# timbroed/HRFuser

Measured on AMD Instinct MI355X. Metric: train images/sec HRFuser-T r640 3-modal @1/2/4/8 MI355X; fwd ms/img, higher is better.
Workload: dtype f32; 1 GPU; t_nus_bn backbone train step (fwd+bwd+grad exchange+AdamW at lr 0), 2 img/GPU, 2x3x384x640 camera + 2 modalities, BN, single GPU; global_batch=2, parallelism=dp1, launch=hipGraph replay

## Files before the change

hrfuser_amd/_lib.py:

```python
import ctypes
import os
import re

import torch

_HERE = os.path.dirname(os.path.abspath(__file__))
HEADER = os.path.join(os.path.dirname(_HERE), 'include', 'hrfuser_hip.h')
DEBUG_HEADER = os.path.join(os.path.dirname(_HERE), 'include', 'hrfuser_hip_debug.h')
LIB_PATH = os.environ.get('HRF_LIB_PATH') or os.path.join(_HERE, 'libhrfuser_hip.so')

def _header_int(name, default):
    m = re.search(r'#define\s+' + name + r'\s+(\d+)', open(HEADER).read())
    return int(m.group(1)) if m else default


STAT_COPIES = _header_int('HRF_STAT_COPIES', 16)
FIN_MAXC = _header_int('HRF_FIN_MAXC', 576)
C3X_MAXC = _header_int('HRF_C3X_MAXC', 256)

def struct_from_header(tag, path=HEADER):
    src = re.sub(r'/\*.*?\*/', '', open(path).read(), flags=re.S)
    m = re.search(r'typedef\s+struct\s+' + tag + r'\s*\{(.*?)\}\s*' + tag + r'_t\s*;', src, flags=re.S)
    if not m:
        raise KeyError(tag)
    fields = []
    for decl in m.group(1).split(';'):
        decl = ' '.join(decl.split())
        if not decl:
            continue
        arr = re.search(r'(\w+)\[(\w+)\]$', decl)
        if arr:
            ext = int(arr.group(2)) if arr.group(2).isdigit() else _header_int(arr.group(2), 0)
            base = decl.split(' ', 1)[0]
            el = ctypes.c_void_p if '*' in decl else {'int': ctypes.c_int, 'long': ctypes.c_long, 'float': ctypes.c_float, 'double': ctypes.c_double}[base]
            fields.append((arr.group(1), el * ext))
            continue
        if '*' in decl:
            ct, names = ctypes.c_void_p, [re.findall(r'(\w+)$', decl)[0]]
        else:
            base, rest = decl.split(' ', 1)
            ct = {'int': ctypes.c_int, 'long': ctypes.c_long, 'float': ctypes.c_float, 'double': ctypes.c_double}[base]
            names = [n.strip() for n in rest.split(',')]
        fields += [(n, ct) for n in names]
    return type(tag, (ctypes.Structure,), {'_fields_': fields})


BnFin = struct_from_header('hrf_bn_fin')
BnBFin = struct_from_header('hrf_bn_bfin')
AttnBlock = struct_from_header('hrf_attn_block')
AttnProj = struct_from_header('hrf_attn_proj')
FfnEval = struct_from_header('hrf_ffn_eval')
BottleneckEval = struct_from_header('hrf_bottleneck_eval')
Conv3xPackJob = struct_from_header('hrf_conv3x_pack_job')
RoiLevels = struct_from_header('hrf_roi_levels')
P2p = struct_from_header('hrf_p2p')


def _ptr(t):
    return None if t is None else t.data_ptr()


_RAW_RETURN = ('hrf_conv3_wgrad_wide_scratch', 'hrf_conv_bwd_weight_scratch', 'hrf_conv3x_pack_size', 'hrf_conv3x_supported', 'hrf_conv_bwd_data_weight_supported', 'hrf_conv_fwd_split_scratch', 'hrf_wgrad_group_report', 'hrf_attn_block_supported', 'hrf_attn_block_bwd_supported', 'hrf_window_attn_proj_supported', 'hrf_group_count',
               'hrf_ffn_eval_supported', 'hrf_bottleneck_eval_supported', 'hrf_roi_align_supported', 'hrf_get_deterministic', 'hrf_det_bins_bytes', 'hrf_conv3_bf16x3_supported', 'hrf_grad_sumsq_parts')
_ERR = {1: 'HRF_ERR_ARG (bad argument)', 2: 'HRF_ERR_LAUNCH (kernel launch failed)'}


class HRFuserHipError(RuntimeError):
    pass


def parse_header(path=HEADER):
    src = open(path).read()
    src = re.sub(r'/\*.*?\*/', '', src, flags=re.S)
    protos = {}
    for m in re.finditer(r'\b(?:int|long)\s+(hrf_\w+)\s*\(([^)]*)\)\s*;', src):
        args = []
        for a in m.group(2).split(','):
            a = ' '.join(a.split())
            if not a or a == 'void':
                continue
            name = re.findall(r'(\w+)$', a)[0]
            if '*' in a:
                ct = ctypes.c_void_p
            elif a.startswith('float'):
                ct = ctypes.c_float
            elif a.startswith('double'):
                ct = ctypes.c_double
            elif a.startswith('long'):
                ct = ctypes.c_long
            else:
                ct = ctypes.c_int
            args.append((ct, name))
        protos[m.group(1)] = args
    return protos


class Lib:

    def __init__(self, path, require_cuda=True):
        if not os.path.exists(path):
            raise HRFuserHipError(
                f'{path} not found: the HRFuser HIP extension is not built. Run '
                '`python -m hrfuser_amd.build_ext` (needs hipcc). There is no CPU fallback.')
        self.path = path
        self.require_cuda = require_cuda
        self._dll = ctypes.CDLL(path)
        self.protos = parse_header()
        self.protos.update(parse_header(DEBUG_HEADER))
        self._fns = {}
        for name, args in self.protos.items():
            fn = getattr(self._dll, name)
            fn.restype = ctypes.c_long if name in ('hrf_conv3_wgrad_wide_scratch', 'hrf_conv_bwd_weight_scratch', 'hrf_conv3x_pack_size', 'hrf_conv_fwd_split_scratch', 'hrf_wgrad_group_report', 'hrf_group_count', 'hrf_det_bins_bytes', 'hrf_grad_sumsq_parts') else ctypes.c_int
            fn.argtypes = [ct for ct, _ in args]
            self._fns[name] = self._wrap(name, fn, args)
        if os.environ.get('HRF_DETERMINISTIC', '0') == '1':
            self.hrf_set_deterministic(1)

    def _wrap(self, name, fn, args):
        kinds = [ct for ct, _ in args]
        nargs = len(kinds)
        require_cuda = self.require_cuda

        def call(*a):
            if len(a) != nargs:
                raise TypeError(f'{name} expects {nargs} args, got {len(a)}')
            conv = []
            for v, ct in zip(a, kinds):
                if ct is ctypes.c_void_p:
                    if v is None:
                        conv.append(None)
                    elif isinstance(v, (ctypes.Structure, ctypes.Array)):
                        conv.append(ctypes.addressof(v))
                    elif isinstance(v, torch.Tensor):
                        if require_cuda and not v.is_cuda:
                            raise HRFuserHipError(f'{name}: tensor on {v.device}; the HIP path has no CPU fallback')
                        conv.append(v.data_ptr())
                    else:
                        conv.append(int(v))
                else:
                    conv.append(v)
            rc = fn(*conv)
            if name in _RAW_RETURN:
                return rc
            if rc != 0:
                raise HRFuserHipError(f'{name} failed: {_ERR.get(rc, rc)}')
# ... 35 lines not shown
```

hrfuser_amd/backbone.py:

```python
import os
import warnings

import torch
import torch.nn as nn

from . import _lib
from . import runtime as R
from .registry import BACKBONES

WIN = 7


def build_bn(norm_cfg, c):
    cfg = dict(norm_cfg or dict(type='BN'))
    kind = cfg.pop('type')
    if kind not in ('BN', 'SyncBN', 'GN'):
        raise KeyError(f'unsupported norm_cfg type {kind}')
    requires_grad = cfg.pop('requires_grad', True)
    if kind == 'GN':
        if 'num_groups' not in cfg:
            raise AssertionError('norm_cfg of type GN needs num_groups')
        bn = nn.GroupNorm(cfg['num_groups'], c, eps=cfg.get('eps', 1e-5))
    else:
        bn = nn.BatchNorm2d(c, eps=cfg.get('eps', 1e-5), momentum=cfg.get('momentum', 0.1))
# ... 425 lines not shown
        if eng is None:
            eng = Engine(self)
            self.__dict__['_hrf_engine'] = eng
        return eng

    def _lib_handle(self):
        return _lib.lib()

    def _bn_slot(self, bn):
        return self._engine().slots[id(bn)]

    def _bn_eval_affine(self, bn):
        return self._engine().bn_eval_affine(bn)

    use_lanes = True

    def _lane_pool(self, grow=False):
        pool = self.__dict__.setdefault('_hrf_lanes', [])
        if grow:
            lane = R.Lane(torch.cuda.Stream(priority=int(os.environ.get('HRF_LANE_PRIORITY', '0'))))
            pool.append(lane)
            return lane
        return pool

    def _lane_group(self, lane, base_group):
        groups = self.__dict__.setdefault('_hrf_lane_groups', {})
        g = groups.get(id(lane))
        if g is None:
            import torch.distributed as dist
            g = groups[id(lane)] = dist.new_group(ranks=dist.get_process_group_ranks(base_group))
        return g

    def _side_pool(self):
        pool = self.__dict__.get('_hrf_side')
        if pool is None:
            n = int(os.environ.get('HRF_SIDE_LANES', '6') or 6)
            try:
                low = max(torch.cuda.Stream.priority_range())
            except Exception:
                low = 0
            if os.environ.get('HRF_SIDE_PRIORITY', '1') == '0':
                low = 0
            pool = [R.Lane(torch.cuda.Stream(priority=low)) for _ in range(max(1, n))]
            self.__dict__['_hrf_side'] = pool
        return pool

    def set_sync_group(self, group, world):
        self.sync_group, self.sync_world = group, world
        if group is not None:
            R.check_sync_schedule(group, world)

    def set_deterministic(self, on=True):
        L = self._lib_handle()
        if bool(L.hrf_get_deterministic()) != bool(on):
            self._engine().det_epoch += 1
        L.hrf_set_deterministic(1 if on else 0)
        self._engine().det_sync()
        if hasattr(self, 'reset_graphs'):
            self.reset_graphs()

    def set_bottleneck_eval(self, on=True):
        self.__dict__['_hrf_bneck_eval'] = bool(on)
        if hasattr(self, 'reset_graphs'):
            self.reset_graphs()

    def params_updated(self):
        """Kept for callers that signal a weight update; nothing is cached across steps any more."""


class Bottleneck(nn.Module):
    expansion = 4

    def __init__(self, inplanes, planes, norm_cfg, downsample=None):
        super().__init__()
        self._nn = [norm_name(norm_cfg, k) for k in (1, 2, 3)]
        self.conv1 = nn.Conv2d(inplanes, planes, 1, bias=False)
        self.add_module(self._nn[0], build_bn(norm_cfg, planes))
        self.conv2 = nn.Conv2d(planes, planes, 3, 1, 1, bias=False)
        self.add_module(self._nn[1], build_bn(norm_cfg, planes))
        self.conv3 = nn.Conv2d(planes, planes * 4, 1, bias=False)
        self.add_module(self._nn[2], build_bn(norm_cfg, planes * 4))
        self.downsample = downsample

    def run(self, ctx, x):
        if R.bottleneck_eval_ok(ctx, self, x):
            return R.bottleneck_eval(ctx, x, self)
        n1, n2, n3 = (getattr(self, k) for k in self._nn)
        y = R.conv_bn(ctx, x, self.conv1, n1, R.TF_RELU)
        y = R.conv_bn(ctx, y, self.conv2, n2, R.TF_RELU)
        y = R.conv_bn(ctx, y, self.conv3, n3, R.TF_AFFINE)
        if self.downsample is not None:
            idt = R.conv_bn(ctx, x, self.downsample[0], self.downsample[1], R.TF_AFFINE)
            return R.materialize(ctx, y, R.ACT_RELU, lazy2=idt)
        return R.materialize(ctx, y, R.ACT_RELU, res=x)


class BasicBlock(nn.Module):
    expansion = 1

    def __init__(self, inplanes, planes, norm_cfg, downsample=None):
        super().__init__()
        if downsample is not None or inplanes != planes:
            raise NotImplementedError('BasicBlock with a downsample path is unused by the HRNet branches')
        self._nn = [norm_name(norm_cfg, k) for k in (1, 2)]
        self.conv1 = nn.Conv2d(inplanes, planes, 3, 1, 1, bias=False)
        self.add_module(self._nn[0], build_bn(norm_cfg, planes))
        self.conv2 = nn.Conv2d(planes, planes, 3, 1, 1, bias=False)
        self.add_module(self._nn[1], build_bn(norm_cfg, planes))
        self.downsample = None

    def run(self, ctx, x):
        y = R.conv_bn(ctx, x, self.conv1, getattr(self, self._nn[0]), R.TF_RELU)
        y = R.conv_bn(ctx, y, self.conv2, getattr(self, self._nn[1]), R.TF_AFFINE)
        return R.materialize(ctx, y, R.ACT_RELU, res=x)


class CrossFFN(nn.Module):

    def __init__(self, in_channels, hidden_channels=None, out_channels=None, norm_cfg=dict(type='SyncBN'), **kw):
        super().__init__()
        out_channels = out_channels or in_channels
        hidden_channels = hidden_channels or in_channels
        self.layers = nn.Sequential(
            nn.Conv2d(in_channels, hidden_channels, 1), build_bn(norm_cfg, hidden_channels), nn.GELU(),
            nn.Conv2d(hidden_channels, hidden_channels, 3, 1, 1, groups=hidden_channels),
            build_bn(norm_cfg, hidden_channels), nn.GELU(),
            nn.Conv2d(hidden_channels, out_channels, 1), build_bn(norm_cfg, out_channels), nn.GELU())

    def run(self, ctx, ln_in):
        l = self.layers
        return self.run_tail(ctx, R.conv_bn(ctx, ln_in, l[0], l[1], R.TF_GELU))

    def run_tail(self, ctx, h1):
        l = self.layers
        h = R.dwconv_bn(ctx, h1, l[3], l[4], R.TF_GELU)
        return R.conv_bn(ctx, h, l[6], l[7], R.TF_GELU)


class WindowMSA(nn.Module):
    def __init__(self, embed_dims, num_heads, window_size=(WIN, WIN), **kw):
        super().__init__()
        if tuple(window_size) != (WIN, WIN):
            raise NotImplementedError('the HIP attention core is specialised for 7x7 windows')
        self.embed_dims, self.num_heads = embed_dims, num_heads
        self.relative_position_bias_table = nn.Parameter(torch.zeros((2 * WIN - 1) ** 2, num_heads))
        self.register_buffer('relative_position_index', _rel_index())
        self.qkv = nn.Linear(embed_dims, embed_dims * 3)
        self.out_proj = nn.Linear(embed_dims, embed_dims)


class LocalWindowSelfAttention(nn.Module):

    def __init__(self, embed_dims, num_heads, window_size=WIN, with_pad_mask=False, **kw):
        super().__init__()
        if with_pad_mask:
            raise NotImplementedError('with_pad_mask=True is unused by every reference config')
        ws = (window_size, window_size) if isinstance(window_size, int) else tuple(window_size)
        self.attn = WindowMSA(embed_dims, num_heads, ws)

    def run(self, ctx, x, ln, cache=None, drop=None):
        a = self.attn
        B, H, W, C = x.t.shape
        lin = R.ln_input(ctx, x, ln, cache)
        if R.attn_proj_ok(ctx, C, a.num_heads):
            o = R.window_attention_proj(ctx, lin, lin, (a.qkv,), a.relative_position_bias_table, a.num_heads)
            return R.linear_residual(ctx, o, a.out_proj, x, drop=drop)
        qkv = R.Plain(R._new((B * H * W, 3 * C), x.t.device))
        R.linear_into(ctx, lin, a.qkv, qkv, 0)
        bq = a.qkv.bias
        o = R.window_attention(ctx, qkv, 0, qkv, C, qkv, 2 * C, bq[C:2 * C], bq[2 * C:], bq, C, bq, 2 * C,
                               a.relative_position_bias_table, a.num_heads, (B, H, W, C))
        return R.linear_residual(ctx, o, a.out_proj, x, drop=drop)


_DEBUG_PAD_CACHE = {}


# ... 310 lines not shown
                        row.append(nn.Sequential(nn.Conv2d(ch[j], ch[i], 1, bias=False), build_bn(norm_cfg, ch[i]),
                                                 nn.Upsample(scale_factor=2 ** (j - i), mode='nearest')))
                    elif j == i:
                        row.append(None)
                    else:
                        steps = []
                        for k in range(i - j):
                            last = k == i - j - 1
                            cout = ch[i] if last else ch[j]
                            mods = [nn.Conv2d(ch[j], cout, 3, 2, 1, bias=False), build_bn(norm_cfg, cout)]
                            if not last:
                                mods.append(nn.ReLU(inplace=False))
                            steps.append(nn.Sequential(*mods))
                        row.append(nn.Sequential(*steps))
                rows.append(nn.ModuleList(row))
            self.fuse_layers = nn.ModuleList(rows)

    def run(self, ctx, xs):
        nb = self.num_branches
        xs = list(xs)
        lanes = ctx.fork(nb, keep_first=ctx.keep_first)

        def branch(i):
            xs[i] = R.force(ctx, xs[i])
            for blk in self.branches[i]:
                xs[i] = blk.run(ctx, xs[i])
        ctx.parallel(lanes, [lambda i=i: branch(i) for i in range(nb)])
        ctx.join(lanes)
        if nb == 1:
            return [xs[0]]
        nrows = len(self.fuse_layers)
        terms = [[None] * nb for _ in range(nrows)]
        lanes = ctx.fork(nb, keep_first=ctx.keep_first)

        def source(j):
            for i, row in enumerate(self.fuse_layers):
                if j == i:
                    terms[i][j] = ('id', xs[j])
                elif j > i:
                    Hi, Wi, Hj, Wj = xs[i].t.shape[1], xs[i].t.shape[2], xs[j].t.shape[1], xs[j].t.shape[2]
                    if Hi != Hj << (j - i) or Wi != Wj << (j - i):
                        raise NotImplementedError('HRModule exchange on grids that do not nest (input not a multiple of 32)')
                    terms[i][j] = ('near', R.conv_bn(ctx, xs[j], row[j][0], row[j][1], R.TF_AFFINE))
                else:
                    cur = xs[j]
                    for step in row[j]:
                        cur = R.conv_bn(ctx, cur, step[0], step[1], R.TF_RELU if len(step) == 3 else R.TF_AFFINE)
                    terms[i][j] = ('same', cur)
        ctx.parallel(lanes, [lambda j=j: source(j) for j in range(nb)])
        ctx.join(lanes)
        return [R.fuse_sum(ctx, tuple(xs[i].t.shape), terms[i]) for i in range(nrows)]


def _make_transition(pre, cur, norm_cfg):
    layers = []
    for i, c in enumerate(cur):
        if i < len(pre):
            layers.append(_conv_bn_seq(pre[i], c, 3, 1, norm_cfg, relu=True) if c != pre[i] else None)
        else:
            steps = []
            for j in range(i + 1 - len(pre)):
                cout = c if j == i - len(pre) else pre[-1]
                steps.append(_conv_bn_seq(pre[-1], cout, 3, 2, norm_cfg, relu=True))
            layers.append(nn.Sequential(*steps))
    return nn.ModuleList(layers)


def _run_conv_chain(ctx, x, seqs):
    cur = x
    for seq in seqs:
        cur = R.conv_bn(ctx, cur, seq[0], seq[1], R.TF_RELU)
    return R.materialize(ctx, cur, R.ACT_RELU)


def _make_res_layer(inplanes, planes, blocks, norm_cfg):
    ds = None
    if inplanes != planes * 4:
        ds = nn.Sequential(nn.Conv2d(inplanes, planes * 4, 1, bias=False), build_bn(norm_cfg, planes * 4))
    layers = [Bottleneck(inplanes, planes, norm_cfg, ds)]
    layers += [Bottleneck(planes * 4, planes, norm_cfg) for _ in range(1, blocks)]
    return nn.Sequential(*layers)


def resolve_init_cfg(pretrained, init_cfg):
    assert not (init_cfg and pretrained), 'init_cfg and pretrained cannot be specified at the same time'
    if isinstance(pretrained, str):
        warnings.warn('DeprecationWarning: pretrained is deprecated, please use "init_cfg" instead')
        return dict(type='Pretrained', checkpoint=pretrained)
    if pretrained is not None:
        raise TypeError('pretrained must be a str or None')
    return init_cfg


def load_pretrained(module, init_cfg):
    path = init_cfg['checkpoint']
    if not os.path.isfile(path):
        raise FileNotFoundError(f'init_cfg Pretrained: {path} is not a local file (there is no downloader here)')
    ckpt = torch.load(path, map_location='cpu')
    sd = ckpt.get('state_dict', ckpt) if isinstance(ckpt, dict) else ckpt
    prefix = init_cfg.get('prefix')
    out = {}
    for k, v in sd.items():
        if k.startswith('module.'):
            k = k[7:]
        if prefix:
            p = prefix if prefix.endswith('.') else prefix + '.'
            if not k.startswith(p):
                continue
            k = k[len(p):]
        out[k] = v
    res = module.load_state_dict(out, strict=False)
    if res.missing_keys or res.unexpected_keys:
        warnings.warn(f'Pretrained init from {path}: {len(res.missing_keys)} missing, '
                      f'{len(res.unexpected_keys)} unexpected keys')
    return res


def default_or_pretrained_init(module):
    cfg = getattr(module, 'init_cfg', None)
    if cfg:
        if isinstance(cfg, dict) and cfg.get('type') == 'Pretrained':
            return load_pretrained(module, cfg)
        raise NotImplementedError(f'init_cfg {cfg!r}: only None (Kaiming / Constant default) and type=Pretrained are built')
    for m in module.modules():
        if isinstance(m, nn.Conv2d):
            nn.init.kaiming_normal_(m.weight, mode='fan_out', nonlinearity='relu')
            if m.bias is not None:
                nn.init.constant_(m.bias, 0)
        elif isinstance(m, (nn.modules.batchnorm._BatchNorm, nn.GroupNorm)):
            nn.init.constant_(m.weight, 1)
            nn.init.constant_(m.bias, 0)


class _BackboneFn(torch.autograd.Function):

    @staticmethod
    def forward(fctx, module, anchor, *inputs):
        record = anchor is not None
        ctx, outs, srcs = module._execute(inputs, record)
        fctx.hrf = (ctx, outs, srcs)
        fctx.set_materialize_grads(False)
        return tuple(o.t.permute(0, 3, 1, 2) for o in outs)

    @staticmethod
    def backward(fctx, *gouts):
        ctx, outs, srcs = fctx.hrf
        for o, g in zip(outs, gouts):
            if g is None:
                o.grad = torch.zeros_like(o.t)
            else:
                o.grad = g.permute(0, 2, 3, 1).contiguous()
                if o.grad.data_ptr() == g.data_ptr():
                    o.grad = o.grad.clone()
        ctx.run_backward()
        grads = tuple(fctx_module_input_grad(s) for s in srcs)
        fctx.hrf = None
        _poll_exchange(ctx.owner)
        return (None, None) + grads


def _poll_exchange(module):
    px = module._engine().__dict__.get('_p2p')
    if px is not None and px[2] is not None:
        px[2].poll()


# ... 314 lines not shown
            fcfg = extra['ModFusionD']
            self.fusion_d_cfg = fcfg
            ch = list(fcfg['num_channels'])
            self.transition_d = nn.ModuleList(_make_transition(sch, ch, ncfg) for _ in range(M))
            self.fusion_d = self._make_multimodal_fusion(fcfg, ch)
        self.init_weights()

    def _make_stage(self, cfg, in_channels, multiscale_output=True):
        block = self.blocks_dict[cfg['block']]
        if block is not HRFormerBlock:
            raise NotImplementedError('stages 2-4 / LidarStage B-C must use block HRFORMER')
        n = cfg['num_modules']
        nb0 = cfg['num_blocks'][0]
        dpr = cfg.get('drop_path_rates', [0.0] * (n * nb0))
        mods = []
        for i in range(n):
            ms = multiscale_output or i != n - 1
            mods.append(HRFomerModule(cfg['num_branches'], block, cfg['num_blocks'], in_channels,
                                      cfg['num_channels'], cfg['num_heads'], cfg['window_sizes'], cfg['mlp_ratios'],
                                      ms, drop_paths=dpr[nb0 * i:nb0 * (i + 1)],
                                      with_rpe=self.extra.get('with_rpe', True),
                                      with_pad_mask=self.extra.get('with_pad_mask', False),
                                      norm_cfg=self.norm_cfg, transformer_norm_cfg=self.transformer_norm_cfg,
                                      with_cp=self.with_cp))
            in_channels = mods[-1].in_channels
        return nn.Sequential(*mods), in_channels

    def _make_multimodal_fusion(self, cfg, num_inchannels):
        if cfg['block'] not in ('CA', 'MWCA'):
            raise Exception('Not valid fusion block')
        block = self.blocks_dict[cfg['block']]
        return nn.ModuleList(
            block(num_inchannels[i], cfg['num_channels'][i], num_heads=cfg['num_heads'][i],
                  window_size=cfg['window_sizes'][i], mlp_ratio=cfg['mlp_ratios'][i], drop_path=cfg['drop_path'],
                  norm_cfg=self.norm_cfg, transformer_norm_cfg=self.transformer_norm_cfg,
                  num_fused_modalities=self.num_fused_modalities, proj_drop_rate=cfg['proj_drop_rate'])
            for i in range(cfg['num_branches']))

    def init_weights(self):
        default_or_pretrained_init(self)

    def train(self, mode=True):
        super().train(mode)
        if mode and self.norm_eval:
            for m in self.modules():
                if isinstance(m, nn.modules.batchnorm._BatchNorm):
                    m.eval()
        return self

    def unused_parameter_names(self):
        return ('transition1.0.1.weight', 'transition1.0.1.bias')

    def forward(self, x, x_mod):
        if not self.num_fused_modalities == len(x_mod):
            raise Exception('num_fused_modalities does not fit the given input length')
        for m in x_mod:
            if m.shape[0] != x.shape[0] or m.shape[2:] != x.shape[2:]:
                raise AssertionError('camera and modality inputs must share batch and spatial size')
        return self._call_engine((x,) + tuple(x_mod))

    def refresh_inputs(self, inputs):
        bufs = self.__dict__.setdefault('_nhwc_in', {})
        for i, t in enumerate(inputs):
            Bn, C, H, W = t.shape
            if t.is_contiguous(memory_format=torch.channels_last) and not t.is_contiguous():
                bufs[i] = t.permute(0, 2, 3, 1)
                continue
            b = bufs.get(i)
            if b is None or b.shape != (Bn, H, W, C) or b.device != t.device or not b.is_contiguous():
                b = bufs[i] = torch.empty(Bn, H, W, C, device=t.device, dtype=torch.float32)
            b.copy_(t.permute(0, 2, 3, 1))
        return bufs

    def _wrap_inputs(self, inputs):
        bufs = {}
        if self.training and inputs[0].is_cuda:
            bufs = self.refresh_inputs(inputs)
        return [R.RawInput(t, bool(t.requires_grad), bufs.get(i)) for i, t in enumerate(inputs)]

    def _stem(self, ctx, src, c1, b1, c2, b2, layer):
        y = R.conv_bn(ctx, src, c1, b1, R.TF_RELU)
        y = R.conv_bn(ctx, y, c2, b2, R.TF_RELU)
        x = R.materialize(ctx, y, R.ACT_RELU)
        for blk in layer:
            x = blk.run(ctx, x)
        return x

    def _fuse_stage(self, ctx, cam_in, trans_cam, trans_mod, fusion, nb, mods, first, tag=''):
        M = self.num_fused_modalities
        cams = [None] * nb
        ms = [[None] * M for _ in range(nb)]
        lanes = ctx.bundle_lanes(1 + M, 'trans')

        def cam_trans():
            for i in range(nb):
                if first:
                    t0 = trans_cam[i][0]
                    cams[i] = self._bare_conv(ctx, cam_in, t0) if isinstance(t0, nn.Conv2d) \
                        else _run_conv_chain(ctx, cam_in, [t0])
                elif trans_cam[i] is not None:
                    tr = trans_cam[i]
                    same = isinstance(tr[0], nn.Conv2d)
                    cams[i] = _run_conv_chain(ctx, cam_in[i] if same else cam_in[-1], [tr] if same else list(tr))
                else:
                    cams[i] = cam_in[i]

        def mod_trans(k):
            for i in range(nb):
                tr = trans_mod[k][i]
                ms[i][k] = mods[k] if tr is None else \
                    _run_conv_chain(ctx, mods[k], [tr] if isinstance(tr[0], nn.Conv2d) else list(tr))
        ctx.parallel(lanes, [cam_trans] + [lambda k=k: mod_trans(k) for k in range(M)])
        ctx.join(lanes)
        ctx.mark('transitions_' + tag)
        xs = [R.Pending(tuple(cams[i].t.shape), lambda c, i=i: fusion[i].run(c, cams[i], ms[i])) for i in range(nb)]
        m0 = [R.split_grad(ctx, ms[0][k]) for k in range(M)]
        if not _PENDING_FUSION:
            xs = R.force_all(ctx, xs)
            ctx.mark('fusion_' + tag)
        return xs, m0

    def _bare_conv(self, ctx, x, conv):
        B, H, W, C = x.t.shape
        out = R.Plain(R._new((B * H * W, conv.weight.shape[0]), x.t.device))
        L, s = ctx.L, ctx.stream
        w = conv.weight
        Cout = w.shape[0]
        strides = (H * W * C, W * C, C, 1)
        L.hrf_conv_fwd(x.t, *strides, B, H, W, C, w, None, 3, 1, Cout, out.t, Cout, 0, None, None, 0,
                       R.TF_NONE, None, None, None, None, None, None, 0.0, s)
        act = R.Act(out.t.view(B, H, W, Cout))

        def bwd():
            R._conv_backward(ctx, x, w, None, 3, 1, Cout, act.grad, Cout, 0, None, None)
        ctx.push(bwd)
        return act

    @staticmethod
    def _run_stage(ctx, stage, xs):
        mods = list(stage)
        for k, mod in enumerate(mods):
            if isinstance(mod, HRFomerModule) and mod.num_branches == 1 and k + 1 < len(mods) and \
                    isinstance(mods[k + 1], HRFomerModule) and mods[k + 1].num_branches == 1:
                xs = mod.run(ctx, xs, defer_out=True)
            else:
                xs = mod.run(ctx, xs)
        return R.force_all(ctx, xs)

    def _run(self, ctx, srcs):
        M = self.num_fused_modalities
        lanes = ctx.bundle_lanes(1 + M, 'stems')
        mods = [None] * M
        cam = [None]

        def cam_stem():
            cam[0] = self._stem(ctx, srcs[0], self.conv1, getattr(self, self._stem_nn[0]), self.conv2, getattr(self, self._stem_nn[1]), self.layer1)

        def mod_stem(k):
            mods[k] = self._stem(ctx, srcs[1 + k], self.conv_a[k], self.norm_a[k], self.conv_b[k], self.norm_b[k],
                                 self.layer_a[k])
        ctx.parallel(lanes, [cam_stem] + [lambda k=k: mod_stem(k) for k in range(M)])
        ctx.join(lanes)
        ctx.mark('stems')
        x = cam[0]
        xs, m0 = self._fuse_stage(ctx, x, self.transition1, self.transition_a, self.fusion_a,
                                  self.stage2_cfg['num_branches'], mods, True, 'a')
        ys, mods = self._stages(ctx, self.stage2, xs, self.stage_b, m0)
        ctx.mark('stage2+stage_b')
        xs, m0 = self._fuse_stage(ctx, ys, self.transition2, self.transition_b, self.fusion_b,
# ... 187 lines not shown
```

hrfuser_amd/csrc/conv_engine.hip:

```cpp
#include <algorithm>
#include <cstdlib>
#include <vector>
#include "hrf_common.h"
#include "hrf_group.h"
#include "hrf_lin.h"
#include "../../include/hrfuser_hip.h"

#include "hrf_wgrad.h"

namespace {

constexpr int BM = 64;
constexpr int BK = 64;
constexpr int LDK = 65;
constexpr float SENT = -1.0e30f;

static int g_knob[12] = {0, 0, 0, 0, 0, 0, 0, 0, 0, 0, 0, 0};

__device__ __forceinline__ float act_at_read(int tf, float u) {
  return tf == HRF_TF_AFFINE_RELU ? fmaxf(u, 0.f) : (tf == HRF_TF_AFFINE_GELU ? hrf_gelu(u) : u);
}

struct ConvFwdArgs {
  const float* x; const float* w; const float* bias;
// ... 890 lines not shown
  const int pad = KH / 2;
  a.bfin = hrf_bn_bfin_t{};
  if (!hrf_det_fin_ok(bfin)) return HRF_ERR_ARG;
  if (bfin != nullptr) a.bfin = *bfin;
  stats = hrf_det_tag(stats);
  a.dy = dy; a.ldD = ldD; a.doff = doff; a.yraw = yraw; a.cA = cA; a.cB = cB; a.cC = cC; a.w = w;
  a.dx = dx; a.sB = sB; a.sY = sY; a.sX = sX; a.sC = sC; a.accumulate = accumulate; a.epi = epi;
  a.xraw = xraw; a.ldXr = ldXr; a.tf_scale = tf_scale; a.tf_shift = tf_shift; a.act = act; a.stats = stats;
  a.B = B; a.H = H; a.W = W; a.Cin = Cin;
  a.Ho = (H + 2 * pad - KH) / stride + 1; a.Wo = (W + 2 * pad - KH) / stride + 1;
  a.Cout = Cout; a.stride = stride; a.pad = pad;
  a.M = B * H * W; a.K = KH * KH * Cout;
  if (a.M <= 0) return HRF_OK;
  if (KH == 1 && stride == 1 && sC == 1 && sY == W * sX && sB == H * sY && g_knob[4] == 0) {
    LinBwdDataArgs l;
    l.dy = dy; l.ldD = ldD; l.doff = doff; l.yraw = yraw; l.cA = cA; l.cB = cB; l.cC = cC; l.w = w;
    l.dx = dx; l.ldDx = sX; l.accumulate = accumulate; l.epi = epi; l.xraw = xraw; l.ldXr = ldXr;
    l.tf_scale = tf_scale; l.tf_shift = tf_shift; l.act = act; l.stats = stats; l.bfin = a.bfin;
    l.M = a.M; l.K = Cout; l.N = Cin;
    const int rc2 = hrf_lin2_bwd_data_launch(l, stream);
    if (rc2 >= 0) return rc2;
    const int rc = hrf_lin_bwd_data_launch(l, stream);
    if (rc >= 0) return rc;
  }
  if (KH == 3 && stride == 1 && Cout >= (g_knob[5] > 0 ? g_knob[5] : 16) && sC == 1 && sY == W * sX && sB == H * sY && g_knob[6] == 0) {
    Conv3Args c{};
    c.in = dy + doff; c.ldIn = ldD; c.in2 = cA != nullptr ? yraw + doff : nullptr; c.t0 = cA; c.t1 = cB; c.t2 = cC;
    c.w = w; c.wCin = Cin; c.out = dx; c.ldOut = sX; c.accumulate = accumulate; c.epi = epi; c.xraw = xraw; c.ldXr = ldXr;
    c.esc = tf_scale; c.esh = tf_shift; c.act = act; c.stats = stats; c.bfin = a.bfin;
    c.B = B; c.H = H; c.W = W; c.Cin = Cout; c.Cout = Cin;
    return hrf_conv3_bwd_data_launch(c, stream);
  }
  if (KH == 3 && stride == 2 && Cout >= (g_knob[5] > 0 ? g_knob[5] : 16) && sC == 1 && sY == W * sX && sB == H * sY && g_knob[6] == 0) {
    Conv3Args c{};
    c.in = dy + doff; c.ldIn = ldD; c.in2 = cA != nullptr ? yraw + doff : nullptr; c.t0 = cA; c.t1 = cB; c.t2 = cC;
    c.w = w; c.wCin = Cin; c.out = dx; c.ldOut = sX; c.accumulate = accumulate; c.epi = epi; c.xraw = xraw; c.ldXr = ldXr;
    c.esc = tf_scale; c.esh = tf_shift; c.act = act; c.stats = stats; c.bfin = a.bfin;
    c.B = B; c.H = H; c.W = W; c.Cin = Cout; c.Cout = Cin; c.Hs = a.Ho; c.Ws = a.Wo;
    return hrf_conv3s2_bwd_data_launch(c, stream);
  }
  const int nt = pick_nt(Cin);
  if (KH == 1) {
    if (cA != nullptr) { HRF_BD_NT(1, true) } else { HRF_BD_NT(1, false) }
  } else {
    if (cA != nullptr) { HRF_BD_NT(3, true) } else { HRF_BD_NT(3, false) }
  }
  return hrf_check_launch();
}

extern "C" int hrf_conv_bwd_data_weight_supported(int Cin, int Cout, long rows, int epi, int bnb) {
  if (Cin <= 0 || Cout <= 0 || rows <= 0 || (epi != 0 && epi != 1) || g_knob[4] != 0) return 0;
  if (rows > (1L << 30)) return 0;
  if (hrf_lin2_bwd_data_wide(rows, Cout, Cin)) return 0;
  return hrf_lin_bwd_data_wg_ok((int)rows, Cout, Cin, bnb != 0) ? 1 : 0;
}

extern "C" int hrf_conv_bwd_data_weight(const float* dy, int ldD, int doff, const float* yraw,
                                        const float* cA, const float* cB, const float* cC, const hrf_bn_bfin_t* bfin,
                                        const float* w, int KH, int stride, int Cout,
                                        int B, int H, int W, int Cin,
                                        float* dx, int sB, int sY, int sX, int sC, int accumulate,
                                        int epi, const float* xraw, int ldXr, const float* tf_scale,
                                        const float* tf_shift, int act, double* stats,
                                        const float* x, int ldX, float* dw, float* dbias, long copy_stride, void* stream) {
  HRF_GROUP_CALL();
  if (KH != 1 || stride != 1 || !(sC == 1 && sX == Cin && sY == W * sX && sB == H * sY)) return HRF_ERR_ARG;
  if (bfin != nullptr && (cA == nullptr || bfin->C != Cout || Cout > HRF_FIN_MAXC || bfin->gstats == nullptr)) return HRF_ERR_ARG;
  if (dy == nullptr || w == nullptr || dx == nullptr || dw == nullptr || copy_stride < 0) return HRF_ERR_ARG;
  if (epi == 1 ? (xraw == nullptr || tf_scale == nullptr || tf_shift == nullptr || ldXr < Cin) : (x == nullptr || ldX < Cin)) return HRF_ERR_ARG;
  const long rows = (long)B * H * W;
  if (rows <= 0 || !hrf_conv_bwd_data_weight_supported(Cin, Cout, rows, epi, cA != nullptr ? 1 : 0)) return HRF_ERR_ARG;
  if (!hrf_det_fin_ok(bfin)) return HRF_ERR_ARG;
  bool det_ok = true;
  dw = hrf_det_grad(dw, det_ok); dbias = hrf_det_grad(dbias, det_ok);
  if (!det_ok) return HRF_ERR_ARG;
  LinBwdDataArgs l;
  l.bfin = hrf_bn_bfin_t{};
  if (bfin != nullptr) l.bfin = *bfin;
  l.dy = dy; l.ldD = ldD; l.doff = doff; l.yraw = yraw; l.cA = cA; l.cB = cB; l.cC = cC; l.w = w;
  l.dx = dx; l.ldDx = sX; l.accumulate = accumulate; l.epi = epi; l.xraw = xraw; l.ldXr = ldXr;
  l.tf_scale = tf_scale; l.tf_shift = tf_shift; l.act = act; l.stats = hrf_det_tag(stats);
  l.M = (int)rows; l.K = Cout; l.N = Cin;
  l.x = x; l.ldX = ldX; l.dw = dw; l.dbias = dbias; l.copy_stride = copy_stride;
  const int rc = hrf_lin_bwd_data_launch(l, stream);
  return rc >= 0 ? rc : HRF_ERR_ARG;
}

extern "C" int hrf_conv3x_supported(int Cin, int Cout, int KH, int stride, int dir) {
  if (KH != 3 || Cin <= 0 || Cout <= 0) return 0;
  if (dir == 0) return (stride == 1 || stride == 2) && Cout > 32 ? 1 : 0;
  if (stride == 2) return Cin > 32 && Cout <= 64 ? 1 : 0;
  return stride == 1 && Cin > 32 ? 1 : 0;
}

extern "C" int hrf_conv_fwd_packed(const float* x, int sB, int sY, int sX, int sC, int B, int H, int W, int Cin,
                                   const float* w, const float* bias, int KH, int stride, int Cout,
                                   float* y, int ldY, int yoff, const float* res, const float* res2, int ldR,
                                   int tf_mode, const float* tf_scale, const float* tf_shift,
                                   const float* tf_rowstat, double* stats, const hrf_bn_fin_t* tf_fin, float* ln_rowstat,
                                   float ln_eps, const float* wp, void* stream) {
  HRF_GROUP_CALL();
  (void)w; (void)tf_rowstat;
  if (wp == nullptr || !hrf_conv3x_supported(Cin, Cout, KH, stride, 0)) return HRF_ERR_ARG;
  if (!(sC == 1 && sY == W * sX && sB == H * sY) || tf_mode < 0 || tf_mode > HRF_TF_AFFINE_GELU) return HRF_ERR_ARG;
  if (ln_rowstat != nullptr && (ldY != Cout || yoff != 0)) return HRF_ERR_ARG;
  if (tf_mode != HRF_TF_NONE && Cin > HRF_C3X_MAXC) return HRF_ERR_ARG;
  if (tf_fin != nullptr && (tf_mode < HRF_TF_AFFINE || tf_fin->C != Cin || tf_fin->stats == nullptr)) return HRF_ERR_ARG;
  C3xArgs c{};
  c.in = x; c.ldIn = sX; c.t0 = tf_scale; c.t1 = tf_shift; c.tf_mode = tf_mode; c.wp = wp;
  c.Np = (Cout + 63) & ~63; c.Kp = (Cin + 31) & ~31; c.bias = bias;
  c.out = y; c.ldOut = ldY; c.ooff = yoff; c.res = res; c.res2 = res2; c.ldR = ldR; c.stats = hrf_det_tag(stats);
  c.B = B; c.H = H; c.W = W; c.Cin = Cin; c.Cout = Cout;
  if (!hrf_det_fin_ok(tf_fin)) return HRF_ERR_ARG;
  if (tf_fin != nullptr) c.fin = *tf_fin;
  int rc;
  if (stride == 2) {
    c.Hs = H; c.Ws = W; c.H = (H + 2 - KH) / 2 + 1; c.W = (W + 2 - KH) / 2 + 1;
    rc = hrf_conv3xs2_fwd_launch(c, stream);
  } else {
    rc = hrf_conv3x_fwd_launch(c, stream);
  }
  if (rc == HRF_OK && ln_rowstat != nullptr) return hrf_ln_stats(y, (long)B * c.H * c.W, Cout, ln_eps, ln_rowstat, stream);
  return rc;
}

extern "C" int hrf_conv_bwd_data_packed(const float* dy, int ldD, int doff, const float* yraw,
                                        const float* cA, const float* cB, const float* cC, const hrf_bn_bfin_t* bfin,
                                        const float* w, int KH, int stride, int Cout,
                                        int B, int H, int W, int Cin,
                                        float* dx, int sB, int sY, int sX, int sC, int accumulate,
                                        int epi, const float* xraw, int ldXr, const float* tf_scale,
                                        const float* tf_shift, int act, double* stats, const float* wp, void* stream) {
  HRF_GROUP_CALL();
  (void)w;
  if (wp == nullptr || !hrf_conv3x_supported(Cin, Cout, KH, stride, 1)) return HRF_ERR_ARG;
  if (!(sC == 1 && sY == W * sX && sB == H * sY)) return HRF_ERR_ARG;
  if (cA != nullptr && Cout > HRF_C3X_MAXC) return HRF_ERR_ARG;
  if (bfin != nullptr && (cA == nullptr || bfin->C != Cout || bfin->gstats == nullptr)) return HRF_ERR_ARG;
  C3xArgs c{};
  c.in = dy + doff; c.ldIn = ldD; c.in2 = cA != nullptr ? yraw + doff : nullptr; c.t0 = cA; c.t1 = cB; c.t2 = cC;
  c.wp = wp; c.Np = (Cin + 63) & ~63; c.Kp = (Cout + 31) & ~31;
  c.out = dx; c.ldOut = sX; c.accumulate = accumulate; c.epi = epi; c.xraw = xraw; c.ldXr = ldXr;
  c.esc = tf_scale; c.esh = tf_shift; c.act = act; c.stats = hrf_det_tag(stats);
  if (!hrf_det_fin_ok(bfin)) return HRF_ERR_ARG;
  if (bfin != nullptr) c.bfin = *bfin;
  c.B = B; c.H = H; c.W = W; c.Cin = Cout; c.Cout = Cin;
  if (stride == 1) return hrf_conv3x_bwd_data_launch(c, stream);
  c.Hs = (H + 2 - KH) / stride + 1; c.Ws = (W + 2 - KH) / stride + 1;
  return hrf_conv3xs2_bwd_data_launch(c, stream);
}

extern "C" __attribute__((visibility("hidden"))) int hrf_pw_knob(int key, int value);
extern "C" __attribute__((visibility("hidden"))) int hrf_conv3w_knob(int key, int value);
extern "C" __attribute__((visibility("hidden"))) int hrf_lin2_knob(int key, int value);
extern "C" __attribute__((visibility("hidden"))) int hrf_w3x_knob(int key, int value);
extern "C" __attribute__((visibility("hidden"))) int hrf_dw_knob(int key, int value);
extern "C" __attribute__((visibility("hidden"))) int hrf_ab_knob(int key, int value);
extern "C" int hrf_debug_knob(int key, int value) {
  if (key >= 36 && key < 40) return hrf_ab_knob(key - 36, value);
  if (key >= 40 && key < 44) return hrf_dw_knob(key - 40, value);
  if (key >= 32 && key < 36) return hrf_w3x_knob(key - 32, value);
  if (key >= 28 && key < 32) return hrf_lin2_knob(key - 28, value);
  if (key >= 16 && key < 20) return hrf_pw_knob(key - 16, value);
  if (key >= 24 && key < 28) return hrf_conv3w_knob(key - 24, value);
  if (key < 0 || key >= 12) return HRF_ERR_ARG;
  g_knob[key] = value;
// ... 269 lines not shown
```

hrfuser_amd/csrc/hrf_lin.h:

```cpp
#pragma once
#include "../../include/hrfuser_hip.h"

struct LinFwdArgs {
  const float* x; int ldX;
  const float* w; const float* bias;
  float* y; int ldY; int yoff;
  const float* res; const float* res2; int ldR;
  int tf_mode; const float* tf_scale; const float* tf_shift; const float* tf_rowstat;
  double* stats;
  float* ln_out; float ln_eps;
  hrf_bn_fin_t fin;
  int M, K, N;
};

struct LinBwdDataArgs {
  const float* dy; int ldD; int doff; const float* yraw;
  const float* cA; const float* cB; const float* cC;
  const float* w;
  float* dx; int ldDx; int accumulate;
  int epi; const float* xraw; int ldXr; const float* tf_scale; const float* tf_shift; int act;
  double* stats;
  hrf_bn_bfin_t bfin;
  int M, K, N;
  const float* x = nullptr; int ldX = 0;
  float* dw = nullptr; float* dbias = nullptr; long copy_stride = 0;
};

int hrf_lin_fwd_launch(const LinFwdArgs& a, void* stream);
bool hrf_lin_fwd_emits_ln(const LinFwdArgs& a);
int hrf_lin_bwd_data_launch(const LinBwdDataArgs& a, void* stream);
bool hrf_lin_bwd_data_wg_ok(int M, int K, int N, bool bnb);
int hrf_lin2_fwd_launch(const LinFwdArgs& a, void* stream);
bool hrf_lin2_fwd_emits_ln(const LinFwdArgs& a);
int hrf_lin2_bwd_data_launch(const LinBwdDataArgs& a, void* stream);
bool hrf_lin2_bwd_data_wide(long M, int K, int N);

struct Conv3Args {
  const float* in; int ldIn;
  const float* in2;
  const float* t0; const float* t1; const float* t2;
  int tf_mode;
  const float* w; int wCin;
  const float* bias;
  float* out; int ldOut; int ooff;
  const float* res; const float* res2; int ldR;
  int accumulate, epi; const float* xraw; int ldXr; const float* esc; const float* esh; int act;
  double* stats;
  hrf_bn_fin_t fin;
  hrf_bn_bfin_t bfin;
  int B, H, W, Cin, Cout;
  int Hs, Ws;
  int tilesX, tilesY;
};
int hrf_conv3_fwd_launch(const Conv3Args& a, void* stream);
int hrf_conv3_bwd_data_launch(const Conv3Args& a, void* stream);
int hrf_conv3s2_bwd_data_launch(const Conv3Args& a, void* stream);

struct C3xArgs {
  const float* in; int ldIn;
  const float* in2;
  const float* t0; const float* t1; const float* t2;
  int tf_mode;
  const float* wp; int Np, Kp;
  const float* bias;
  float* out; int ldOut; int ooff;
  const float* res; const float* res2; int ldR;
  int accumulate, epi; const float* xraw; int ldXr; const float* esc; const float* esh; int act;
  double* stats;
  hrf_bn_fin_t fin;
  hrf_bn_bfin_t bfin;
  int B, H, W, Cin, Cout;
  int Hs, Ws;
  int tilesX, tilesY, ntiles, per_xcd;
  int cols_per_block;
};

int hrf_conv3x_fwd_launch(const C3xArgs& a, void* stream);
int hrf_conv3x_bwd_data_launch(const C3xArgs& a, void* stream);
int hrf_conv3xs2_fwd_launch(const C3xArgs& a, void* stream);
int hrf_conv3xs2_bwd_data_launch(const C3xArgs& a, void* stream);
```

hrfuser_amd/csrc/lin2_engine.hip:

```cpp
#include <type_traits>
#include "hrf_common.h"
#include "hrf_lin.h"
#include "hrf_group.h"
#include "../../include/hrfuser_hip.h"

namespace {

constexpr int GK = 16, GLP = GK + 4, NW = 4, NTHR = 64 * NW, GROWS = 16 * NW;

template <int CG_, int CT_, int PD_>
struct Tile {
  static constexpr int CG = CG_, CT = CT_, PD = PD_;
  static constexpr int NB = CG * CT * 16, RT = CG, RG = NW / CG;
  static constexpr int SLOT = (GROWS + NB) * GLP;
  static constexpr int NWV = (NB * 4 + NTHR - 1) / NTHR;
  static constexpr int Q = CT * 4, PE = CT * 16 + 4, NRG = NTHR / Q, NR = (GROWS + NRG - 1) / NRG;
  static constexpr int RED = NRG * 2 * CT * 16;
  static_assert(GROWS * PE <= 2 * SLOT, "the transposed accumulator tile must fit the operand ring");
};
typedef Tile<1, 5, 4> TileA;
typedef Tile<2, 5, 4> TileB;
typedef Tile<2, 8, 2> TileC;
typedef Tile<2, 10, 2> TileD;

#ifdef HRF_EMUL
#define L2_SCHED_FENCE() ((void)0)
#define L2_OPAQUE(v) ((void)0)
#else
#define L2_OPAQUE(v) asm volatile("" : "+v"(v))
#define L2_SCHED_FENCE() __builtin_amdgcn_sched_barrier(0)
#endif
#define L2_INLINE __attribute__((always_inline))

__device__ float g_zero4l[4] = {0.f, 0.f, 0.f, 0.f};
#if defined(HRF_L2_TIMING) && !defined(HRF_EMUL)
__device__ long long g_l2_t[64];
#define L2_T(k) do { if (blockIdx.x == 100 && blockIdx.y == 0 && threadIdx.x == 0) g_l2_t[k] = wall_clock64(); } while (0)
#else
#define L2_T(k)
#endif
static int g_l2_knob[4] = {0, 0, 0, 0};

__device__ __forceinline__ hrf_f4 l2_ld4(const float* p) {
#ifdef HRF_EMUL
  return hrf_ld4(p);
#else
  return *reinterpret_cast<const hrf_f4*>(p);
#endif
}
__device__ __forceinline__ void l2_st4(float* p, hrf_f4 v) {
#ifdef HRF_EMUL
  hrf_st4(p, v);
#else
  *reinterpret_cast<hrf_f4*>(p) = v;
#endif
}
__device__ __forceinline__ hrf_f4 gl_ld4(const float* p, int nvalid) {
  if (nvalid >= 4) return hrf_ld4(p);
  hrf_f4 r;
#pragma unroll
  for (int e = 0; e < 4; ++e) r[e] = *(e < nvalid ? p + e : g_zero4l);
  return r;
}

__device__ __forceinline__ hrf_f4 ld4_ragged(const float* row, int idx, int len) {
  const int ic = idx > len - 4 ? len - 4 : idx;
  const int d = idx - ic;
  const hrf_f4 v = hrf_ld4(row + ic);
  hrf_f4 o;
  o[0] = d == 0 ? v[0] : (d == 1 ? v[1] : (d == 2 ? v[2] : (d == 3 ? v[3] : 0.f)));
  o[1] = d == 0 ? v[1] : (d == 1 ? v[2] : (d == 2 ? v[3] : 0.f));
  o[2] = d == 0 ? v[2] : (d == 1 ? v[3] : 0.f);
  o[3] = d == 0 ? v[3] : 0.f;
  return o;
}

template <class T>
__device__ __forceinline__ void acc_to_lds(float* sE, const hrf_f4 (*acc)[T::CT], int rg, int lane) {
  const int i = lane & 15, q = lane >> 4;
#pragma unroll
  for (int rr = 0; rr < T::RT; ++rr)
#pragma unroll
    for (int tt = 0; tt < T::CT; ++tt) l2_st4(sE + ((rg * T::RT + rr) * 16 + i) * T::PE + tt * 16 + 4 * q, acc[rr][tt]);
}
template <class T>
__device__ __forceinline__ void moments_out(float* sRed, double* stats, int N, int chbase, int c4, int rgp, bool active,
                                            const float* s1, const float* s2) {
  constexpr int CW = T::CT * 16;
  if (active) {
#pragma unroll
    for (int r = 0; r < 4; ++r) {
      sRed[(rgp * 2 + 0) * CW + 4 * c4 + r] = s1[r];
      sRed[(rgp * 2 + 1) * CW + 4 * c4 + r] = s2[r];
    }
  }
  __syncthreads();
  for (int e = threadIdx.x; e < 2 * CW; e += NTHR) {
    const int which = e / CW, c = e - which * CW;
    if (chbase + c < N) {
      float s = 0.f;
#pragma unroll
      for (int g = 0; g < T::NRG; ++g) s += sRed[(g * 2 + which) * CW + c];
      hrf_stat_add(stats, 2 * N, which * N + chbase + c, (double)s);
    }
  }
}

template <int V> using IC = std::integral_constant<int, V>;

template <class T, int TF>
__global__ __launch_bounds__(NTHR, 2) void lin2_fwd_kernel(HrfGroup<LinFwdArgs> grp) {
  const LinFwdArgs& a = grp.sel();
  constexpr int CG = T::CG, CT = T::CT, PD = T::PD, NB = T::NB, RT = T::RT, SLOT = T::SLOT, NWV = T::NWV;
  constexpr bool TBLS = TF != HRF_TF_NONE;
  HRF_DYN_SMEM(float, smem);
  const int KT = (a.K + GK - 1) & ~(GK - 1);
  float* sTab = smem + 2 * SLOT;
  float* sRed = sTab + (TBLS ? 2 * KT : 0);
  const int tid = threadIdx.x, lane = tid & 63;
  const int wave = __builtin_amdgcn_readfirstlane(tid >> 6);
  const int i = lane & 15, q = lane >> 4;
  const int chg = wave % CG, rg = wave / CG;
  const long m0 = (long)blockIdx.x * GROWS;
  const int n0 = blockIdx.y * NB;
  L2_T(0);

  if (TBLS) {
    if (TF != HRF_TF_LN && a.fin.stats != nullptr) {
      hrf_bn_fin_onload(a.fin, sTab, sTab + KT, tid, NTHR, blockIdx.x == 0 && blockIdx.y == 0);
    } else {
      for (int k = tid; k < a.K; k += NTHR) { sTab[k] = a.tf_scale[k]; sTab[KT + k] = a.tf_shift[k]; }
    }
    for (int k = a.K + tid; k < KT; k += NTHR) { sTab[k] = 0.f; sTab[KT + k] = 0.f; }
  }

  hrf_f4 acc[RT][CT];
#pragma unroll
  for (int rr = 0; rr < RT; ++rr)
#pragma unroll
    for (int tt = 0; tt < CT; ++tt) acc[rr][tt] = hrf_f4{0.f, 0.f, 0.f, 0.f};

  const long xr = m0 + (tid >> 2) < a.M ? m0 + (tid >> 2) : a.M - 1;
  const int xdst = (tid >> 2) * GLP + 4 * (tid & 3);
  float mean = 0.f, rstd = 1.f;
  if (TF == HRF_TF_LN) { mean = a.tf_rowstat[2 * xr]; rstd = a.tf_rowstat[2 * xr + 1]; }
  const unsigned xoff = (unsigned)(xr * a.ldX);
  const int wn0 = tid >> 2, wq = tid & 3;
  unsigned woff[NWV];
#pragma unroll
  for (int e = 0; e < NWV; ++e) {
    const int n = n0 + wn0 + 64 * e;
    woff[e] = (unsigned)(n < a.N ? n : 0) * (unsigned)a.K;
  }
  const int wdst0 = (GROWS + wn0) * GLP + 4 * wq;
  hrf_f4 xpre[PD], wpre[PD][NWV];
  auto load_tile = [&](auto SETC, int s) L2_INLINE {
    constexpr int SET = decltype(SETC)::value;
    const int kb = s * GK + 4 * (tid & 3);
    if ((s + 1) * GK <= a.K) {
      xpre[SET] = hrf_ld4(a.x + (size_t)(xoff + kb));
#pragma unroll
      for (int e = 0; e < NWV; ++e) wpre[SET][e] = hrf_ld4(a.w + (size_t)(woff[e] + kb));
    } else {
      xpre[SET] = ld4_ragged(a.x + (size_t)xoff, kb, a.K);
#pragma unroll
      for (int e = 0; e < NWV; ++e) wpre[SET][e] = ld4_ragged(a.w + (size_t)woff[e], kb, a.K);
    }
  };
  auto store_tile = [&](auto SETC, int s) L2_INLINE {
    constexpr int SET = decltype(SETC)::value;
    float* d = smem + (s & 1) * SLOT;
    const int kb = s * GK + 4 * (tid & 3);
    hrf_f4 v = xpre[SET];
    if (TBLS) {
      const hrf_f4 sc = l2_ld4(sTab + kb), sh = l2_ld4(sTab + KT + kb);
#pragma unroll
      for (int r = 0; r < 4; ++r) {
        float u = TF == HRF_TF_LN ? fmaf((v[r] - mean) * rstd, sc[r], sh[r]) : fmaf(v[r], sc[r], sh[r]);
        v[r] = TF == HRF_TF_AFFINE_RELU ? fmaxf(u, 0.f) : (TF == HRF_TF_AFFINE_GELU ? hrf_gelu(u) : u);
      }
    }
    l2_st4(d + xdst, v);
#pragma unroll
    for (int e = 0; e < NWV; ++e)
      if ((e + 1) * NTHR <= NB * 4 || tid + e * NTHR < NB * 4) l2_st4(d + wdst0 + e * 64 * GLP, wpre[SET][e]);
  };
// ... 50 lines not shown
    if (s + 1 + PD < S) load_tile(IC<J1>{}, s + 1 + PD);
    read_frags(s & 1);
    L2_SCHED_FENCE();
    mma(ALL);
    L2_SCHED_FENCE();
    __syncthreads();
    L2_T(3 + (s < 40 ? s : 40));
  };
  auto kloop = [&](auto ALL) L2_INLINE {
    for (int s = 0; s < S; s += PD) {
      step(ALL, IC<0>{}, s);
      if (s + 1 < S) step(ALL, IC<1 % PD>{}, s + 1);
      if (PD > 2) {
        if (s + 2 < S) step(ALL, IC<2 % PD>{}, s + 2);
        if (s + 3 < S) step(ALL, IC<3 % PD>{}, s + 3);
      }
    }
  };
  if (all_on) kloop(std::true_type{}); else kloop(std::false_type{});

  {
    constexpr int Q = T::Q, PE = T::PE, NRG = T::NRG, NR = T::NR;
    float* sE = smem;
    const int c4 = tid % Q, rgp = tid / Q;
    const bool active = rgp < NRG;
#pragma unroll 1
    for (int pass = 0; pass < CG; ++pass) {
      const int chbase = n0 + pass * CT * 16, ch = chbase + 4 * c4;
      const int nval = active ? a.N - ch : 0;
      hrf_f4 bv = hrf_f4{0.f, 0.f, 0.f, 0.f};
      if (a.bias != nullptr) bv = gl_ld4(a.bias + ch, nval);
      hrf_f4 r1[NR], r2[NR];
#pragma unroll
      for (int j = 0; j < NR; ++j) { r1[j] = hrf_f4{0.f, 0.f, 0.f, 0.f}; r2[j] = r1[j]; }
      if (a.res != nullptr) {
#pragma unroll
        for (int j = 0; j < NR; ++j) {
          const long m = m0 + rgp + j * NRG;
          const bool rv = rgp + j * NRG < GROWS && m < a.M;
          r1[j] = gl_ld4(a.res + (rv ? m : 0) * a.ldR + ch, rv ? nval : 0);
        }
      }
      if (a.res2 != nullptr) {
#pragma unroll
        for (int j = 0; j < NR; ++j) {
          const long m = m0 + rgp + j * NRG;
          const bool rv = rgp + j * NRG < GROWS && m < a.M;
          r2[j] = gl_ld4(a.res2 + (rv ? m : 0) * a.ldR + ch, rv ? nval : 0);
        }
      }
      L2_T(44 + 4 * pass);
      if (pass > 0) __syncthreads();
      if (chg == pass) acc_to_lds<T>(sE, acc, rg, lane);
      __syncthreads();
      L2_T(45 + 4 * pass);
      float s1[4] = {0.f, 0.f, 0.f, 0.f}, s2[4] = {0.f, 0.f, 0.f, 0.f};
#pragma unroll
      for (int j = 0; j < NR; ++j) {
        const int row = rgp + j * NRG;
        const long m = m0 + row;
        if (row < GROWS && m < a.M && nval > 0) {
          hrf_f4 v = l2_ld4(sE + row * PE + 4 * c4);
#pragma unroll
          for (int r = 0; r < 4; ++r) {
            v[r] = r < nval ? v[r] + bv[r] + r1[j][r] + r2[j][r] : 0.f;
            s1[r] += v[r]; s2[r] = fmaf(v[r], v[r], s2[r]);
          }
          float* o = a.y + m * a.ldY + a.yoff + ch;
          if (nval >= 4) hrf_st4(o, v);
          else {
#pragma unroll
            for (int r = 0; r < 4; ++r)
              if (r < nval) o[r] = v[r];
          }
        }
      }
      L2_T(46 + 4 * pass);
      if (a.stats != nullptr) moments_out<T>(sRed, a.stats, a.N, chbase, c4, rgp, active, s1, s2);
      L2_T(47 + 4 * pass);
    }
  }
}

template <class T, bool BNB>
__global__ __launch_bounds__(NTHR, 2) void lin2_bwd_data_kernel(HrfGroup<LinBwdDataArgs> grp) {
  const LinBwdDataArgs& a = grp.sel();
  constexpr int CG = T::CG, CT = T::CT, PD = T::PD, NB = T::NB, RT = T::RT, SLOT = T::SLOT, NWV = T::NWV;
  HRF_DYN_SMEM(float, smem);
  const int KT = (a.K + GK - 1) & ~(GK - 1);
  float* sTab = smem + 2 * SLOT;
  float* sRed = sTab + (BNB ? 3 * KT : 0);
  const int tid = threadIdx.x, lane = tid & 63;
  const int wave = __builtin_amdgcn_readfirstlane(tid >> 6);
  const int i = lane & 15, q = lane >> 4;
  const int chg = wave % CG, rg = wave / CG;
  const long m0 = (long)blockIdx.x * GROWS;
  const int n0 = blockIdx.y * NB;
  L2_T(0);

  if (BNB) {
    if (a.bfin.gstats != nullptr) {
      hrf_bn_bfin_onload(a.bfin, sTab, sTab + KT, sTab + 2 * KT, tid, NTHR, blockIdx.x == 0 && blockIdx.y == 0);
    } else {
      for (int k = tid; k < a.K; k += NTHR) { sTab[k] = a.cA[k]; sTab[KT + k] = a.cB[k]; sTab[2 * KT + k] = a.cC[k]; }
    }
    for (int k = a.K + tid; k < KT; k += NTHR) { sTab[k] = 0.f; sTab[KT + k] = 0.f; sTab[2 * KT + k] = 0.f; }
  }

  hrf_f4 acc[RT][CT];
#pragma unroll
  for (int rr = 0; rr < RT; ++rr)
#pragma unroll
    for (int tt = 0; tt < CT; ++tt) acc[rr][tt] = hrf_f4{0.f, 0.f, 0.f, 0.f};

  const long xr = m0 + (tid >> 2) < a.M ? m0 + (tid >> 2) : a.M - 1;
  const unsigned doff = (unsigned)(xr * a.ldD + a.doff);
  const int xdst = (tid >> 2) * GLP + 4 * (tid & 3);
  const int wkk = tid & 15, wn0 = 4 * (tid >> 4);
  hrf_f4 dpre[PD], ypre[PD], wpre[PD][NWV];
  auto load_tile = [&](auto SETC, int s) L2_INLINE {
    constexpr int SET = decltype(SETC)::value;
    const int kb = s * GK + 4 * (tid & 3);
    if ((s + 1) * GK <= a.K) {
      dpre[SET] = hrf_ld4(a.dy + (size_t)(doff + kb));
      if (BNB) ypre[SET] = hrf_ld4(a.yraw + (size_t)(doff + kb));
    } else {
      dpre[SET] = ld4_ragged(a.dy + (size_t)doff, kb, a.K);
      if (BNB) ypre[SET] = ld4_ragged(a.yraw + (size_t)doff, kb, a.K);
    }
    const int k = s * GK + wkk;
    const float* wrow = a.w + (size_t)((unsigned)(k < a.K ? k : a.K - 1) * (unsigned)a.N);
    int nn = n0 + wn0;
    L2_OPAQUE(nn);
#pragma unroll
    for (int e = 0; e < NWV; ++e) wpre[SET][e] = ld4_ragged(wrow, nn + 64 * e, a.N);
  };
  auto store_tile = [&](auto SETC, int s) L2_INLINE {
    constexpr int SET = decltype(SETC)::value;
    float* d = smem + (s & 1) * SLOT;
    const int kb = s * GK + 4 * (tid & 3);
    hrf_f4 v = dpre[SET];
    if (BNB) {
      const hrf_f4 ca = l2_ld4(sTab + kb), cb = l2_ld4(sTab + KT + kb), cc = l2_ld4(sTab + 2 * KT + kb);
#pragma unroll
      for (int r = 0; r < 4; ++r) v[r] = fmaf(ca[r], v[r], fmaf(cb[r], ypre[SET][r], cc[r]));
    }
    l2_st4(d + xdst, v);
    const float km = s * GK + wkk < a.K ? 1.f : 0.f;
#pragma unroll
    for (int e = 0; e < NWV; ++e)
      if ((e + 1) * NTHR <= NB * 4 || tid + e * NTHR < NB * 4) {
#pragma unroll
        for (int r = 0; r < 4; ++r) d[(GROWS + wn0 + 64 * e + r) * GLP + wkk] = wpre[SET][e][r] * km;
      }
  };
  hrf_f4 fa[RT], fb[CT];
  const float* abase = smem + (rg * 16 * RT + i) * GLP + 4 * q;
  const float* bbase = smem + (GROWS + chg * CT * 16 + i) * GLP + 4 * q;
  auto read_frags = [&](int slot) L2_INLINE {
#pragma unroll
    for (int rr = 0; rr < RT; ++rr) fa[rr] = l2_ld4(abase + slot * SLOT + rr * 16 * GLP);
#pragma unroll
    for (int tt = 0; tt < CT; ++tt) fb[tt] = l2_ld4(bbase + slot * SLOT + tt * 16 * GLP);
  };
  bool tile_on[CT];
#pragma unroll
  for (int tt = 0; tt < CT; ++tt) tile_on[tt] = n0 + (chg * CT + tt) * 16 < a.N;
  const bool all_on = tile_on[CT - 1];
  auto mma = [&](auto ALL) L2_INLINE {
    if (decltype(ALL)::value) {
#pragma unroll
      for (int tt = 0; tt < CT; ++tt)
#pragma unroll
        for (int m = 0; m < 4; ++m)
#pragma unroll
          for (int rr = 0; rr < RT; ++rr) acc[rr][tt] = hrf_mfma16(fb[tt][m], fa[rr][m], acc[rr][tt]);
    } else {
#pragma unroll
      for (int tt = 0; tt < CT - 1; ++tt) {
        if (!tile_on[tt]) break;
#pragma unroll
        for (int m = 0; m < 4; ++m)
#pragma unroll
          for (int rr = 0; rr < RT; ++rr) acc[rr][tt] = hrf_mfma16(fb[tt][m], fa[rr][m], acc[rr][tt]);
      }
    }
  };

  const int S = (a.K + GK - 1) / GK;
  if (BNB) __syncthreads();
  L2_T(1);
  load_tile(IC<0>{}, 0);
  if (S > 1) load_tile(IC<1 % PD>{}, 1);
  if (PD > 2) {
    if (S > 2) load_tile(IC<2 % PD>{}, 2);
    if (S > 3) load_tile(IC<3 % PD>{}, 3);
  }
  store_tile(IC<0>{}, 0);
  if (S > PD) load_tile(IC<0>{}, PD);
  __syncthreads();
  L2_T(2);
  auto step = [&](auto ALL, auto JC, int s) L2_INLINE {
    constexpr int J1 = (decltype(JC)::value + 1) % PD;
    L2_SCHED_FENCE();
    if (s + 1 < S) store_tile(IC<J1>{}, s + 1);
    if (s + 1 + PD < S) load_tile(IC<J1>{}, s + 1 + PD);
    read_frags(s & 1);
    L2_SCHED_FENCE();
    mma(ALL);
    L2_SCHED_FENCE();
    __syncthreads();
    L2_T(3 + (s < 40 ? s : 40));
  };
  auto kloop = [&](auto ALL) L2_INLINE {
    for (int s = 0; s < S; s += PD) {
      step(ALL, IC<0>{}, s);
      if (s + 1 < S) step(ALL, IC<1 % PD>{}, s + 1);
      if (PD > 2) {
        if (s + 2 < S) step(ALL, IC<2 % PD>{}, s + 2);
        if (s + 3 < S) step(ALL, IC<3 % PD>{}, s + 3);
      }
    }
  };
  if (all_on) kloop(std::true_type{}); else kloop(std::false_type{});

  {
    constexpr int Q = T::Q, PE = T::PE, NRG = T::NRG, NR = T::NR;
    float* sE = smem;
    const int c4 = tid % Q, rgp = tid / Q;
    const bool active = rgp < NRG;
    const bool mom = a.epi == 1 && a.stats != nullptr;
#pragma unroll 1
    for (int pass = 0; pass < CG; ++pass) {
      const int chbase = n0 + pass * CT * 16, ch = chbase + 4 * c4;
      const int nval = active ? a.N - ch : 0;
      hrf_f4 sc = hrf_f4{0.f, 0.f, 0.f, 0.f}, sh = sc;
      if (a.epi == 1) { sc = gl_ld4(a.tf_scale + ch, nval); sh = gl_ld4(a.tf_shift + ch, nval); }
      hrf_f4 xv[NR];
#pragma unroll
      for (int j = 0; j < NR; ++j) xv[j] = hrf_f4{0.f, 0.f, 0.f, 0.f};
      if (a.epi == 1 || a.accumulate) {
        const float* src = a.epi == 1 ? a.xraw : a.dx;
        const long ld = a.epi == 1 ? a.ldXr : a.ldDx;
#pragma unroll
        for (int j = 0; j < NR; ++j) {
          const long m = m0 + rgp + j * NRG;
          const bool rv = rgp + j * NRG < GROWS && m < a.M;
          xv[j] = gl_ld4(src + (rv ? m : 0) * ld + ch, rv ? nval : 0);
        }
      }
      L2_T(44 + 4 * pass);
      if (pass > 0) __syncthreads();
      if (chg == pass) acc_to_lds<T>(sE, acc, rg, lane);
      __syncthreads();
      L2_T(45 + 4 * pass);
      float s1[4] = {0.f, 0.f, 0.f, 0.f}, s2[4] = {0.f, 0.f, 0.f, 0.f};
      auto rows = [&](auto ACT) L2_INLINE {
        constexpr int AC = decltype(ACT)::value;
#pragma unroll
        for (int j = 0; j < NR; ++j) {
          const int row = rgp + j * NRG;
          const long m = m0 + row;
          if (row < GROWS && m < a.M && nval > 0) {
            hrf_f4 v = l2_ld4(sE + row * PE + 4 * c4);
#pragma unroll
            for (int r = 0; r < 4; ++r) {
              if (AC == 0) v[r] += xv[j][r];
              else if (AC == 1) v[r] = fmaf(xv[j][r], sc[r], sh[r]) > 0.f ? v[r] : 0.f;
              else if (AC == 2) v[r] *= hrf_gelu_grad(fmaf(xv[j][r], sc[r], sh[r]));
              v[r] = r < nval ? v[r] : 0.f;
              s1[r] += v[r]; s2[r] = fmaf(v[r], xv[j][r], s2[r]);
            }
            float* o = a.dx + m * a.ldDx + ch;
            if (nval >= 4) hrf_st4(o, v);
            else {
#pragma unroll
              for (int r = 0; r < 4; ++r)
                if (r < nval) o[r] = v[r];
            }
          }
        }
      };
      if (a.epi != 1) rows(IC<0>{});
      else if (a.act == HRF_ACT_RELU) rows(IC<1>{});
      else if (a.act == HRF_ACT_GELU) rows(IC<2>{});
      else rows(IC<3>{});
      L2_T(46 + 4 * pass);
      if (mom) moments_out<T>(sRed, a.stats, a.N, chbase, c4, rgp, active, s1, s2);
      L2_T(47 + 4 * pass);
    }
  }
}

inline int tile_nb(int id) { return id == 1 ? 80 : (id == 2 ? 160 : (id == 3 ? 256 : 320)); }
inline int pick_tile(int N) {
  if (g_l2_knob[1] >= 1 && g_l2_knob[1] <= 4) return g_l2_knob[1];
  if (N <= 80) return 1;
  if (N <= 160) return 2;
  if (N <= 256) return 3;
  if (N <= 320) return 4;
  const int p4 = ((N + 319) / 320) * 320, p3 = ((N + 255) / 256) * 256;
  return p3 < p4 ? 3 : 4;
}
inline size_t smem_bytes(int id, int ntab, int K, int red) {
  const int KT = (K + GK - 1) & ~(GK - 1);
  return ((size_t)2 * (GROWS + tile_nb(id)) * GLP + (size_t)ntab * KT + red) * sizeof(float);
}
inline bool wide_enough(long M, int K, int N) {
  if (g_l2_knob[0] == 2) return false;
  if (K < 16 || N < 16 || M <= 0) return false;
  if (g_l2_knob[0] == 1) return true;
  const int id = pick_tile(N);
  const long blocks = ((M + GROWS - 1) / GROWS) * ((N + tile_nb(id) - 1) / tile_nb(id));
  const long minb = g_l2_knob[2] > 0 ? g_l2_knob[2] : ((K <= 160 && N >= 320) ? 200 : 400);
  return (K < N ? K : N) >= 64 && blocks >= minb;
}

template <class KERN>
int set_smem(KERN kern, size_t smem) {
#ifndef HRF_EMUL
  if (hipFuncSetAttribute(reinterpret_cast<const void*>(kern), hipFuncAttributeMaxDynamicSharedMemorySize, (int)smem) != hipSuccess)
    return HRF_ERR_LAUNCH;
#endif
  return HRF_OK;
}
constexpr size_t SMEM_MAX = 160 * 1024;

template <class T, int TF>
int launch_fwd(const LinFwdArgs& a, int id, void* stream) {
  const size_t smem = smem_bytes(id, TF != HRF_TF_NONE ? 2 : 0, a.K, T::RED);
  if (smem > SMEM_MAX) return -1;
  static size_t granted = 0;
  if (smem > granted) { if (set_smem(&lin2_fwd_kernel<T, TF>, smem) != HRF_OK) return HRF_ERR_LAUNCH; granted = smem; }
  const dim3 grid(hrf_cdiv(a.M, GROWS), hrf_cdiv(a.N, T::NB));
  return HRF_LAUNCH_G((lin2_fwd_kernel<T, TF>), grid, dim3(NTHR), (unsigned)smem, stream, a);
}
template <class T>
int launch_fwd_tf(const LinFwdArgs& a, int id, void* stream) {
  switch (a.tf_mode) {
    case HRF_TF_NONE: return launch_fwd<T, HRF_TF_NONE>(a, id, stream);
    case HRF_TF_AFFINE: return launch_fwd<T, HRF_TF_AFFINE>(a, id, stream);
    case HRF_TF_AFFINE_RELU: return launch_fwd<T, HRF_TF_AFFINE_RELU>(a, id, stream);
    case HRF_TF_AFFINE_GELU: return launch_fwd<T, HRF_TF_AFFINE_GELU>(a, id, stream);
    case HRF_TF_LN: return launch_fwd<T, HRF_TF_LN>(a, id, stream);
    default: return -1;
  }
}
template <class T, bool BNB>
int launch_bwd(const LinBwdDataArgs& a, int id, void* stream) {
  const size_t smem = smem_bytes(id, BNB ? 3 : 0, a.K, T::RED);
  if (smem > SMEM_MAX) return -1;
  static size_t granted = 0;
  if (smem > granted) { if (set_smem(&lin2_bwd_data_kernel<T, BNB>, smem) != HRF_OK) return HRF_ERR_LAUNCH; granted = smem; }
  const dim3 grid(hrf_cdiv(a.M, GROWS), hrf_cdiv(a.N, T::NB));
  return HRF_LAUNCH_G((lin2_bwd_data_kernel<T, BNB>), grid, dim3(NTHR), (unsigned)smem, stream, a);
}
template <class T>
int launch_bwd_b(const LinBwdDataArgs& a, int id, void* stream) {
  return a.cA != nullptr ? launch_bwd<T, true>(a, id, stream) : launch_bwd<T, false>(a, id, stream);
}

}

int hrf_lin2_fwd_launch(const LinFwdArgs& a, void* stream) {
  if (!wide_enough(a.M, a.K, a.N)) return -1;
  if (a.ln_out != nullptr && g_l2_knob[0] != 1) return -1;
  if ((long)a.M * a.ldX >= (1L << 32)) return -1;
  if (a.tf_mode != HRF_TF_NONE && a.tf_mode != HRF_TF_LN && a.fin.stats != nullptr && a.K > HRF_FIN_MAXC) return -1;
  const int id = pick_tile(a.N);
  switch (id) {
    case 1: return launch_fwd_tf<TileA>(a, id, stream);
    case 2: return launch_fwd_tf<TileB>(a, id, stream);
    case 3: return launch_fwd_tf<TileC>(a, id, stream);
    default: return launch_fwd_tf<TileD>(a, id, stream);
  }
}
bool hrf_lin2_fwd_emits_ln(const LinFwdArgs&) { return false; }
bool hrf_lin2_bwd_data_wide(long M, int K, int N) { return wide_enough(M, K, N); }
int hrf_lin2_bwd_data_launch(const LinBwdDataArgs& a, void* stream) {
  if (!wide_enough(a.M, a.K, a.N)) return -1;
  if (a.cA != nullptr && a.bfin.gstats != nullptr && a.K > HRF_FIN_MAXC) return -1;
  if ((long)a.M * a.ldD + a.doff >= (1L << 32)) return -1;
  const int id = pick_tile(a.N);
  switch (id) {
    case 1: return launch_bwd_b<TileA>(a, id, stream);
    case 2: return launch_bwd_b<TileB>(a, id, stream);
    case 3: return launch_bwd_b<TileC>(a, id, stream);
    default: return launch_bwd_b<TileD>(a, id, stream);
  }
}
#if defined(HRF_L2_TIMING) && !defined(HRF_EMUL)
extern "C" int hrf_lin2_stamps(long long* out) {
  return hipMemcpyFromSymbol(out, HIP_SYMBOL(g_l2_t), sizeof(long long) * 64) == hipSuccess ? HRF_OK : HRF_ERR_LAUNCH;
}
#endif
extern "C" __attribute__((visibility("hidden"))) int hrf_lin2_knob(int key, int value) {
  if (key < 0 || key >= 4) return HRF_ERR_ARG;
  g_l2_knob[key] = value;
  return HRF_OK;
}
```

hrfuser_amd/csrc/lin_engine.hip:

```cpp
#include "hrf_common.h"
#include "hrf_lin.h"
#include "hrf_group.h"
#include "../../include/hrfuser_hip.h"

namespace {

#ifndef HRF_LIN_BWD_EPI_MAX_NT
#define HRF_LIN_BWD_EPI_MAX_NT 5
#endif
constexpr int LIN_BWD_EPI_MAX_NT = HRF_LIN_BWD_EPI_MAX_NT;
#ifndef HRF_LIN_FWD_MAX_NT
#define HRF_LIN_FWD_MAX_NT 5
#endif
constexpr int LIN_FWD_MAX_NT = HRF_LIN_FWD_MAX_NT;
constexpr int LIN_SB = 3, LIN_SB_WIDE = 2, LIN_SB_WIDE_K = 64;

__device__ float g_zero4[4] = {0.f, 0.f, 0.f, 0.f};

template <bool V4>
__device__ __forceinline__ hrf_f4 ld_group(const float* p, long off, int nvalid) {
  if (V4) return hrf_ld4(nvalid > 0 ? p + off : g_zero4);
  hrf_f4 r;
#pragma unroll
  for (int e = 0; e < 4; ++e) r[e] = *(e < nvalid ? p + off + e : g_zero4);
  return r;
}

__device__ __forceinline__ hrf_f4 ld_sel(bool full, const float* p, long off, int nvalid) {
  if (full) return ld_group<true>(p, off, nvalid);
  return ld_group<false>(p, off, nvalid);
}

template <bool V4>
__device__ __forceinline__ void st_group(float* p, hrf_f4 v, int nvalid) {
  if (V4) {
    if (nvalid > 0) hrf_st4(p, v);
  } else {
#pragma unroll
    for (int e = 0; e < 4; ++e)
      if (e < nvalid) p[e] = v[e];
  }
}

template <int NT>
__device__ __forceinline__ void wave_moments(float* sStat, int wave, int j, int q, bool pixv, int n0w, int N,
                                             const hrf_f4* v, const hrf_f4* w) {
#pragma unroll
  for (int t = 0; t < NT; ++t) {
    const int nval = N - (n0w + 16 * t + 4 * q);
    float s1[4], s2[4];
#pragma unroll
    for (int r = 0; r < 4; ++r) {
      const float m = (pixv && r < nval) ? 1.f : 0.f;
      s1[r] = hrf_row16_sum(v[t][r] * m);
      s2[r] = hrf_row16_sum(v[t][r] * w[t][r] * m);
    }
    if (j == 0) {
#pragma unroll
      for (int r = 0; r < 4; ++r) {
        sStat[(wave * 2 + 0) * (NT * 16) + 16 * t + 4 * q + r] = s1[r];
        sStat[(wave * 2 + 1) * (NT * 16) + 16 * t + 4 * q + r] = s2[r];
      }
    }
  }
}

template <int NT>
__device__ __forceinline__ void flush_moments(const float* sStat, double* stats, int n0w, int N) {
  for (int i = threadIdx.x; i < 2 * NT * 16; i += 256) {
    const int which = i / (NT * 16), cidx = i - which * (NT * 16);
    const int ch = n0w + cidx;
    if (ch < N) {
      const float s = sStat[(0 * 2 + which) * (NT * 16) + cidx] + sStat[(1 * 2 + which) * (NT * 16) + cidx] +
                      sStat[(2 * 2 + which) * (NT * 16) + cidx] + sStat[(3 * 2 + which) * (NT * 16) + cidx];
      hrf_stat_add(stats, 2 * N, which * N + ch, (double)s);
    }
  }
}

template <int NT, int TF, int SB, bool SK, bool ONE = false>
__global__ __launch_bounds__(256) void lin_fwd_kernel(HrfGroup<LinFwdArgs> grp) {
  const LinFwdArgs& a = grp.sel();
  __shared__ float sStat[4 * 2 * NT * 16];
  __shared__ __attribute__((aligned(16))) float sRed[SK ? 3 * NT * 256 : 4];
  __shared__ __attribute__((aligned(16))) float sFin[(TF >= HRF_TF_AFFINE && TF <= HRF_TF_AFFINE_GELU) ? 2 * HRF_FIN_MAXC : 4];
  const int tid = threadIdx.x, lane = tid & 63, wave = tid >> 6;
  const int j = lane & 15, q = lane >> 4;
  const int n0w = blockIdx.y * (NT * 16);
  const int pix = SK ? blockIdx.x * 16 + j : blockIdx.x * 64 + wave * 16 + j;
  const bool pixin = pix < a.M;
  const bool pixv = pixin && (!SK || wave == 0);
  const long pc = pixin ? pix : a.M - 1;
  const float* scp = a.tf_scale;
  const float* shp = a.tf_shift;
  if (TF >= HRF_TF_AFFINE && TF <= HRF_TF_AFFINE_GELU) {
    if (a.fin.stats != nullptr) {
      hrf_bn_fin_onload(a.fin, sFin, sFin + HRF_FIN_MAXC, tid, 256, blockIdx.x == 0 && blockIdx.y == 0);
      __syncthreads();
      scp = sFin; shp = sFin + HRF_FIN_MAXC;
    }
  }

  hrf_f4 acc[NT];
#pragma unroll
  for (int t = 0; t < NT; ++t) {
    const int chb = n0w + 16 * t + 4 * q, nval = a.N - chb;
    const bool nfull = n0w + 16 * (t + 1) <= a.N;
    const bool own = !SK || wave == 0;
    acc[t] = ld_sel(nfull, a.bias, chb, (own && a.bias != nullptr) ? nval : 0);
    const hrf_f4 r1 = ld_sel(nfull, a.res, pc * a.ldR + chb, (own && a.res != nullptr) ? nval : 0);
    const hrf_f4 r2 = ld_sel(nfull, a.res2, pc * a.ldR + chb, (own && a.res2 != nullptr) ? nval : 0);
#pragma unroll
    for (int r = 0; r < 4; ++r) acc[t][r] += r1[r] + r2[r];
  }
  float mean = 0.f, rstd = 1.f;
  if (TF == HRF_TF_LN) { mean = a.tf_rowstat[2 * pc]; rstd = a.tf_rowstat[2 * pc + 1]; }

  const int nslab = (a.K + 15) >> 4;
  const int kper = SK ? (nslab + 3) >> 2 : nslab;
  const int k0 = SK ? wave * kper : 0, k1 = SK ? min(nslab, k0 + kper) : nslab;
  const long xrow = pc * a.ldX;
#pragma unroll 1
  for (int kb = k0; kb < (ONE ? k0 + 1 : k1); kb += SB) {
    hrf_f4 xa[SB], sc[SB], sh[SB], wv[SB][NT];
#pragma unroll
    for (int s = 0; s < SB; ++s) {
      const int kbase = 16 * (kb + s) + 4 * q, kval = (!SK || kb + s < k1) ? a.K - kbase : 0;
      const bool kfull = 16 * (kb + s + 1) <= a.K;
      xa[s] = ld_sel(kfull, a.x, xrow + kbase, kval);
      if (TF != HRF_TF_NONE) { sc[s] = ld_sel(kfull, scp, kbase, kval); sh[s] = ld_sel(kfull, shp, kbase, kval); }
#pragma unroll
      for (int t = 0; t < NT; ++t) {
        const int n = n0w + 16 * t + j;
        wv[s][t] = ld_sel(kfull, a.w, (long)n * a.K + kbase, n < a.N ? kval : 0);
      }
    }
#pragma unroll
    for (int s = 0; s < SB; ++s) {
#pragma unroll
      for (int r = 0; r < 4; ++r) {
        float v = xa[s][r];
        if (TF == HRF_TF_LN) v = fmaf((v - mean) * rstd, sc[s][r], sh[s][r]);
        else if (TF != HRF_TF_NONE) v = fmaf(v, sc[s][r], sh[s][r]);
        v = TF == HRF_TF_AFFINE_RELU ? fmaxf(v, 0.f) : (TF == HRF_TF_AFFINE_GELU ? hrf_gelu(v) : v);
#pragma unroll
        for (int t = 0; t < NT; ++t) acc[t] = hrf_mfma16(wv[s][t][r], v, acc[t]);
      }
    }
  }
  if (SK) {
    if (wave != 0) {
#pragma unroll
      for (int t = 0; t < NT; ++t) hrf_st4(sRed + (((wave - 1) * NT + t) * 64 + lane) * 4, acc[t]);
    }
    __syncthreads();
    if (wave == 0) {
#pragma unroll
      for (int w = 0; w < 3; ++w)
#pragma unroll
        for (int t = 0; t < NT; ++t) {
          const hrf_f4 v = hrf_ld4(sRed + ((w * NT + t) * 64 + lane) * 4);
#pragma unroll
          for (int r = 0; r < 4; ++r) acc[t][r] += v[r];
        }
    }
  }

#pragma unroll
  for (int t = 0; t < NT; ++t) {
    const int chb = n0w + 16 * t + 4 * q;
    if (n0w + 16 * (t + 1) <= a.N) st_group<true>(a.y + (long)pc * a.ldY + a.yoff + chb, acc[t], pixv ? a.N - chb : 0);
    else st_group<false>(a.y + (long)pc * a.ldY + a.yoff + chb, acc[t], pixv ? a.N - chb : 0);
  }
  if (a.ln_out != nullptr && gridDim.y == 1) {
    float sm = 0.f;
#pragma unroll
    for (int t = 0; t < NT; ++t)
#pragma unroll
      for (int r = 0; r < 4; ++r) sm += (16 * t + 4 * q + r < a.N) ? acc[t][r] : 0.f;
    sm += __shfl_xor(sm, 16); sm += __shfl_xor(sm, 32);
    const float mu = sm / (float)a.N;
    float sq = 0.f;
#pragma unroll
    for (int t = 0; t < NT; ++t)
#pragma unroll
      for (int r = 0; r < 4; ++r) { const float dd = (16 * t + 4 * q + r < a.N) ? acc[t][r] - mu : 0.f; sq = fmaf(dd, dd, sq); }
    sq += __shfl_xor(sq, 16); sq += __shfl_xor(sq, 32);
    if (q == 0 && pixv) { a.ln_out[2 * (long)pix] = mu; a.ln_out[2 * (long)pix + 1] = 1.0f / sqrtf(sq / (float)a.N + a.ln_eps); }
  }
  if (a.stats != nullptr) {
    wave_moments<NT>(sStat, wave, j, q, pixv, n0w, a.N, acc, acc);
    __syncthreads();
    flush_moments<NT>(sStat, a.stats, n0w, a.N);
  }
}

constexpr int LIN_WG_LD = 20;
template <int NT, bool BNB, int SB, bool SK, bool ONE = false, bool WG = false>
__global__ __launch_bounds__(256) void lin_bwd_data_kernel(HrfGroup<LinBwdDataArgs> grp) {
  const LinBwdDataArgs& a = grp.sel();
  __shared__ float sStat[4 * 2 * NT * 16];
  __shared__ __attribute__((aligned(16))) float sRed[SK ? 3 * NT * 256 : 4];
  __shared__ __attribute__((aligned(16))) float sFin[BNB ? 3 * HRF_FIN_MAXC : 4];
  __shared__ __attribute__((aligned(16))) float sTr[WG ? 4 * 16 * LIN_WG_LD : 4];
  __shared__ __attribute__((aligned(16))) float sMrg[(WG && !SK) ? 2 * (4 * NT * 256 + 64) : 4];
  const int tid = threadIdx.x, lane = tid & 63, wave = tid >> 6;
  const int j = lane & 15, q = lane >> 4;
  const int n0w = blockIdx.y * (NT * 16);
  const int pix = SK ? blockIdx.x * 16 + j : blockIdx.x * 64 + wave * 16 + j;
  const bool pixin = pix < a.M;
  const bool pixv = pixin && (!SK || wave == 0);
  const long pc = pixin ? pix : a.M - 1;
  const float* cAp = a.cA;
  const float* cBp = a.cB;
  const float* cCp = a.cC;
  if (BNB) {
    if (a.bfin.gstats != nullptr) {
      hrf_bn_bfin_onload(a.bfin, sFin, sFin + HRF_FIN_MAXC, sFin + 2 * HRF_FIN_MAXC, tid, 256, blockIdx.x == 0 && blockIdx.y == 0);
      __syncthreads();
      cAp = sFin; cBp = sFin + HRF_FIN_MAXC; cCp = sFin + 2 * HRF_FIN_MAXC;
    }
  }

  hrf_f4 acc[NT], xr[NT];
#pragma unroll
  for (int t = 0; t < NT; ++t) {
    const int chb = n0w + 16 * t + 4 * q, nval = a.N - chb;
    const bool nfull = n0w + 16 * (t + 1) <= a.N;
    xr[t] = ld_sel(nfull, a.xraw, pc * a.ldXr + chb, a.epi == 1 ? nval : 0);
    acc[t] = ld_sel(nfull, a.dx, pc * a.ldDx + chb, (a.epi != 1 && a.accumulate && (!SK || wave == 0)) ? nval : 0);
  }

  hrf_f4 xb[WG ? NT : 1];
  float* const sT = sTr + (WG ? wave * 16 * LIN_WG_LD : 0);
  const long wcp = WG ? (long)(blockIdx.x % HRF_STAT_COPIES) * a.copy_stride : 0;
  int mbuf = 0;
  if (WG) {
    hrf_f4 xv[NT];
#pragma unroll
    for (int t = 0; t < NT; ++t) {
      const int chb = n0w + 16 * t + 4 * q, nval = a.N - chb;
      const bool nfull = n0w + 16 * (t + 1) <= a.N;
      if (a.epi == 1) {
        const hrf_f4 esc = ld_sel(nfull, a.tf_scale, chb, nval), esh = ld_sel(nfull, a.tf_shift, chb, nval);
#pragma unroll
        for (int r = 0; r < 4; ++r) xv[t][r] = fmaf(xr[t][r], esc[r], esh[r]);
      } else {
        xv[t] = ld_sel(nfull, a.x, pc * a.ldX + chb, nval);
      }
    }
    if (a.epi == 1) {
      hrf_with_act(a.act, [&](auto kind) HRF_KIND_INLINE {
        constexpr int ACT = decltype(kind)::value;
#pragma unroll
        for (int t = 0; t < NT; ++t)
#pragma unroll
          for (int r = 0; r < 4; ++r) xv[t][r] = hrf_act(ACT, xv[t][r]);
      });
    }
#pragma unroll
    for (int t = 0; t < NT; ++t) {
#pragma unroll
      for (int r = 0; r < 4; ++r) {
        const bool cv = n0w + 16 * t + 4 * q + r < a.N;
        sT[(4 * q + r) * LIN_WG_LD + j] = (pixin && cv) ? xv[t][r] : 0.f;
      }
      HRF_WAVE_SYNC();
      xb[t] = hrf_ld4(sT + j * LIN_WG_LD + 4 * q);
      HRF_WAVE_SYNC();
    }
  }

  const int nslab = (a.K + 15) >> 4;
  const int kper = SK ? (nslab + 3) >> 2 : nslab;
  const int k0 = SK ? wave * kper : 0, k1 = SK ? min(nslab, k0 + kper) : nslab;
  const long drow = pc * a.ldD + a.doff;
#pragma unroll 1
  for (int kb = k0; kb < (ONE ? k0 + 1 : k1); kb += SB) {
    hrf_f4 dv[SB], yv[SB], ca[SB], cb[SB], cc[SB], wv[SB][NT];
#pragma unroll
    for (int s = 0; s < SB; ++s) {
      const int kbase = 16 * (kb + s) + 4 * q, kval = (!SK || kb + s < k1) ? a.K - kbase : 0;
      const bool kfull = 16 * (kb + s + 1) <= a.K;
      dv[s] = ld_sel(kfull, a.dy, drow + kbase, kval);
      if (BNB) {
        yv[s] = ld_sel(kfull, a.yraw, drow + kbase, kval);
        ca[s] = ld_sel(kfull, cAp, kbase, kval); cb[s] = ld_sel(kfull, cBp, kbase, kval); cc[s] = ld_sel(kfull, cCp, kbase, kval);
      }
#pragma unroll
      for (int t = 0; t < NT; ++t) {
        const int ci = n0w + 16 * t + j;
#pragma unroll
        for (int r = 0; r < 4; ++r)
          wv[s][t][r] = *((r < kval && ci < a.N) ? a.w + (long)(kbase + r) * a.N + ci : g_zero4);
      }
    }
#pragma unroll
    for (int s = 0; s < SB; ++s) {
#pragma unroll
      for (int r = 0; r < 4; ++r) {
        const float d = BNB ? fmaf(ca[s][r], dv[s][r], fmaf(cb[s][r], yv[s][r], cc[s][r])) : dv[s][r];
#pragma unroll
        for (int t = 0; t < NT; ++t) acc[t] = hrf_mfma16(wv[s][t][r], d, acc[t]);
      }
    }
    if (WG) {
#pragma unroll
      for (int s = 0; s < SB; ++s) {
        const int slab = kb + s;
        if (slab < k1) {
          float bs[4];
#pragma unroll
          for (int r = 0; r < 4; ++r) {
            const float d = BNB ? fmaf(ca[s][r], dv[s][r], fmaf(cb[s][r], yv[s][r], cc[s][r])) : dv[s][r];
            const float dm = (pixin && 16 * slab + 4 * q + r < a.K) ? d : 0.f;
            sT[(4 * q + r) * LIN_WG_LD + j] = dm;
            bs[r] = hrf_row16_sum(dm);
          }
          HRF_WAVE_SYNC();
          const hrf_f4 da = hrf_ld4(sT + j * LIN_WG_LD + 4 * q);
          HRF_WAVE_SYNC();
          hrf_f4 wacc[NT];
#pragma unroll
          for (int t = 0; t < NT; ++t) wacc[t] = hrf_f4{0.f, 0.f, 0.f, 0.f};
#pragma unroll
          for (int m = 0; m < 4; ++m)
#pragma unroll
            for (int t = 0; t < NT; ++t) wacc[t] = hrf_mfma16(da[m], xb[t][m], wacc[t]);
          if (SK) {
#pragma unroll
            for (int t = 0; t < NT; ++t)
#pragma unroll
              for (int r = 0; r < 4; ++r) {
                const int k = 16 * slab + 4 * q + r, ci = n0w + 16 * t + j;
                if (k < a.K && ci < a.N) hrf_grad_add(a.dw, wcp, (long)k * a.N + ci, wacc[t][r]);
              }
            if (a.dbias != nullptr && blockIdx.y == 0 && j == 0) {
#pragma unroll
              for (int r = 0; r < 4; ++r)
                if (16 * slab + 4 * q + r < a.K) hrf_grad_add(a.dbias, wcp, 16 * slab + 4 * q + r, bs[r]);
            }
          } else {
            float* const sM = sMrg + mbuf * (4 * NT * 256 + 64);
#pragma unroll
            for (int t = 0; t < NT; ++t)
#pragma unroll
              for (int r = 0; r < 4; ++r) sM[wave * (NT * 256) + (t * 4 + r) * 64 + lane] = wacc[t][r];
            if (j == 0) {
#pragma unroll
              for (int r = 0; r < 4; ++r) sM[4 * NT * 256 + wave * 16 + 4 * q + r] = bs[r];
            }
            __syncthreads();
#pragma unroll
            for (int t = 0; t < NT; ++t) {
              const int idx = t * 256 + tid;
              const float v = (sM[idx] + sM[NT * 256 + idx]) + (sM[2 * NT * 256 + idx] + sM[3 * NT * 256 + idx]);
              const int k = 16 * slab + 4 * q + wave, ci = n0w + 16 * t + j;
              if (k < a.K && ci < a.N) hrf_grad_add(a.dw, wcp, (long)k * a.N + ci, v);
            }
            if (a.dbias != nullptr && blockIdx.y == 0 && tid < 16 && 16 * slab + tid < a.K) {
              const float* b = sM + 4 * NT * 256;
              hrf_grad_add(a.dbias, wcp, 16 * slab + tid, (b[tid] + b[16 + tid]) + (b[32 + tid] + b[48 + tid]));
            }
            mbuf ^= 1;
          }
        }
      }
    }
  }
  if (SK) {
    if (wave != 0) {
#pragma unroll
      for (int t = 0; t < NT; ++t) hrf_st4(sRed + (((wave - 1) * NT + t) * 64 + lane) * 4, acc[t]);
    }
    __syncthreads();
    if (wave == 0) {
#pragma unroll
      for (int w = 0; w < 3; ++w)
#pragma unroll
        for (int t = 0; t < NT; ++t) {
          const hrf_f4 v = hrf_ld4(sRed + ((w * NT + t) * 64 + lane) * 4);
#pragma unroll
          for (int r = 0; r < 4; ++r) acc[t][r] += v[r];
        }
    }
  }

  if (a.epi == 1) {
    hrf_f4 esc[NT], esh[NT];
#pragma unroll
    for (int t = 0; t < NT; ++t) {
      const int chb = n0w + 16 * t + 4 * q, nval = a.N - chb;
      const bool nfull = n0w + 16 * (t + 1) <= a.N;
      esc[t] = ld_sel(nfull, a.tf_scale, chb, nval); esh[t] = ld_sel(nfull, a.tf_shift, chb, nval);
    }
    hrf_with_act(a.act, [&](auto kind) HRF_KIND_INLINE {
      constexpr int ACT = decltype(kind)::value;
#pragma unroll
      for (int t = 0; t < NT; ++t)
#pragma unroll
        for (int r = 0; r < 4; ++r) acc[t][r] *= hrf_act_grad(ACT, fmaf(xr[t][r], esc[t][r], esh[t][r]));
    });
  }
#pragma unroll
  for (int t = 0; t < NT; ++t) {
    const int chb = n0w + 16 * t + 4 * q;
    if (n0w + 16 * (t + 1) <= a.N) st_group<true>(a.dx + (long)pc * a.ldDx + chb, acc[t], pixv ? a.N - chb : 0);
    else st_group<false>(a.dx + (long)pc * a.ldDx + chb, acc[t], pixv ? a.N - chb : 0);
  }
  if (a.epi == 1 && a.stats != nullptr) {
    wave_moments<NT>(sStat, wave, j, q, pixv, n0w, a.N, acc, xr);
    __syncthreads();
    flush_moments<NT>(sStat, a.stats, n0w, a.N);
  }
}

inline int pick_ntw(int M, int T) {
  const long ptiles = (M + 15) / 16;
#ifndef HRF_LIN_WAVES
#define HRF_LIN_WAVES 768
#endif
  long groups = (HRF_LIN_WAVES + ptiles - 1) / ptiles;
  if (groups > T) groups = T;
  const long gmin = (T + 8) / 9;
  if (groups < gmin) groups = gmin;
  const int need = (int)((T + groups - 1) / groups);
  return need <= 1 ? 1 : (need <= 2 ? 2 : (need <= 3 ? 3 : (need <= 5 ? 5 : 9)));
}

}

#ifndef HRF_LIN_SK_MAX_M
#define HRF_LIN_SK_MAX_M 4096
#endif
#ifndef HRF_LIN_SK_MIN_SLABS
#define HRF_LIN_SK_MIN_SLABS 8
#endif
constexpr int LIN_SK_MAX_M = HRF_LIN_SK_MAX_M, LIN_SK_MIN_SLABS = HRF_LIN_SK_MIN_SLABS;
#ifndef HRF_LIN_LN_ROW_MAX_M
#define HRF_LIN_LN_ROW_MAX_M 8192
#endif
constexpr int LIN_LN_ROW_MAX_M = HRF_LIN_LN_ROW_MAX_M;
inline bool lin_use_sk(int M, int K) { return M <= LIN_SK_MAX_M && ((K + 15) >> 4) >= LIN_SK_MIN_SLABS; }
inline void lin_fwd_plan(const LinFwdArgs& a, int& ntw, bool& sk) {
  const int T = (a.N + 15) / 16;
  sk = lin_use_sk(a.M, a.K);
  ntw = pick_ntw(sk ? 4 * a.M : a.M, T);
  if (ntw > LIN_FWD_MAX_NT) ntw = LIN_FWD_MAX_NT;
  if (a.ln_out != nullptr && T <= 9 && a.M <= LIN_LN_ROW_MAX_M) ntw = T <= 1 ? 1 : (T <= 2 ? 2 : (T <= 3 ? 3 : (T <= 5 ? 5 : 9)));
}

#define HRF_LF_LAUNCH(NT_, TF_, SB_, SK_) HRF_LAUNCH_G((lin_fwd_kernel<NT_, TF_, SB_, SK_>), grid, dim3(256), 0, stream, a)
#define HRF_LF_ONE(NT_, TF_)                                                                                                   \
  { if (a.K <= 16) { HRF_LAUNCH_G((lin_fwd_kernel<NT_, TF_, 1, false, true>), grid, dim3(256), 0, stream, a); }                  \
    else if (a.K <= 32) { HRF_LAUNCH_G((lin_fwd_kernel<NT_, TF_, 2, false, true>), grid, dim3(256), 0, stream, a); }             \
    else { HRF_LAUNCH_G((lin_fwd_kernel<NT_, TF_, 3, false, true>), grid, dim3(256), 0, stream, a); } }
#define HRF_LF_WIDE(NT_, TF_, SK_) { if (a.K <= LIN_SB_WIDE_K) { HRF_LF_LAUNCH(NT_, TF_, LIN_SB, SK_); } else { HRF_LF_LAUNCH(NT_, TF_, LIN_SB_WIDE, SK_); } }
#define HRF_LF_NT(TF_, SK_)                              \
  if (!SK_ && a.K <= 48) {                               \
    switch (ntw) {                                       \
      case 1: HRF_LF_ONE(1, TF_) break;                  \
      case 2: HRF_LF_ONE(2, TF_) break;                  \
      case 3: HRF_LF_ONE(3, TF_) break;                  \
      case 5: HRF_LF_ONE(5, TF_) break;                  \
      default: HRF_LF_WIDE(9, TF_, SK_) break;           \
    }                                                    \
  } else                                                 \
  switch (ntw) {                                         \
    case 1: HRF_LF_LAUNCH(1, TF_, LIN_SB, SK_); break;   \
    case 2: HRF_LF_LAUNCH(2, TF_, LIN_SB, SK_); break;   \
// ... 1 lines not shown
    case 5: HRF_LF_WIDE(5, TF_, SK_) break;              \
    default: HRF_LF_WIDE(9, TF_, SK_) break;             \
  }
#define HRF_LF_V4(TF_) { if (sk) { HRF_LF_NT(TF_, true) } else { HRF_LF_NT(TF_, false) } }

bool hrf_lin_fwd_emits_ln(const LinFwdArgs& a) {
  if (a.K < 4 || a.N < 4 || a.M <= 0) return false;
  int ntw; bool sk;
  lin_fwd_plan(a, ntw, sk);
  return hrf_cdiv((a.N + 15) / 16, ntw) == 1;
}

int hrf_lin_fwd_launch(const LinFwdArgs& a, void* stream) {
  if (a.K < 4 || a.N < 4 || a.M <= 0) return -1;
  const int T = (a.N + 15) / 16;
  int ntw; bool sk;
  lin_fwd_plan(a, ntw, sk);
  const dim3 grid(hrf_cdiv(a.M, sk ? 16 : 64), hrf_cdiv(T, ntw));
  switch (a.tf_mode) {
    case HRF_TF_NONE: HRF_LF_V4(HRF_TF_NONE) break;
    case HRF_TF_AFFINE: HRF_LF_V4(HRF_TF_AFFINE) break;
    case HRF_TF_AFFINE_RELU: HRF_LF_V4(HRF_TF_AFFINE_RELU) break;
    case HRF_TF_AFFINE_GELU: HRF_LF_V4(HRF_TF_AFFINE_GELU) break;
    case HRF_TF_LN: HRF_LF_V4(HRF_TF_LN) break;
    default: return -1;
  }
  return hrf_check_launch();
}

#define HRF_LB_LAUNCH(NT_, BNB_, SB_, SK_) HRF_LAUNCH_G((lin_bwd_data_kernel<NT_, BNB_, SB_, SK_>), grid, dim3(256), 0, stream, a)
#define HRF_LB_ONE(NT_, BNB_)                                                                                                   \
  { if (a.K <= 16) { HRF_LAUNCH_G((lin_bwd_data_kernel<NT_, BNB_, 1, false, true>), grid, dim3(256), 0, stream, a); }             \
    else if (a.K <= 32) { HRF_LAUNCH_G((lin_bwd_data_kernel<NT_, BNB_, 2, false, true>), grid, dim3(256), 0, stream, a); }        \
    else { HRF_LAUNCH_G((lin_bwd_data_kernel<NT_, BNB_, 3, false, true>), grid, dim3(256), 0, stream, a); } }
#define HRF_LB_WIDE(NT_, BNB_, SK_) { if (a.K <= LIN_SB_WIDE_K) { HRF_LB_LAUNCH(NT_, BNB_, LIN_SB, SK_); } else { HRF_LB_LAUNCH(NT_, BNB_, LIN_SB_WIDE, SK_); } }
#define HRF_LB_NT(BNB_, SK_)                             \
  if (!SK_ && a.K <= 48) {                               \
    switch (ntw) {                                       \
      case 1: HRF_LB_ONE(1, BNB_) break;                 \
      case 2: HRF_LB_ONE(2, BNB_) break;                 \
      case 3: HRF_LB_ONE(3, BNB_) break;                 \
      case 5: HRF_LB_ONE(5, BNB_) break;                 \
      default: HRF_LB_ONE(5, BNB_) break;                \
    }                                                    \
  } else                                                 \
  switch (ntw) {                                         \
    case 1: HRF_LB_LAUNCH(1, BNB_, LIN_SB, SK_); break;  \
    case 2: HRF_LB_LAUNCH(2, BNB_, LIN_SB, SK_); break;  \
    case 3: HRF_LB_LAUNCH(3, BNB_, LIN_SB, SK_); break;  \
    default: HRF_LB_WIDE(5, BNB_, SK_) break;            \
  }
#define HRF_LB_V4(BNB_) { if (sk) { HRF_LB_NT(BNB_, true) } else { HRF_LB_NT(BNB_, false) } }

#define HRF_LBW(NT_, BNB_, SB_, SK_, ONE_) HRF_LAUNCH_G((lin_bwd_data_kernel<NT_, BNB_, SB_, SK_, ONE_, true>), grid, dim3(256), 0, stream, a)
#define HRF_LBW_ONE(NT_)                                           \
  { if (a.K <= 16) { HRF_LBW(NT_, true, 1, false, true); }         \
    else if (a.K <= 32) { HRF_LBW(NT_, true, 2, false, true); }    \
    else { HRF_LBW(NT_, true, 3, false, true); } }
#define HRF_LBW_WIDE(SK_) { if (a.K <= LIN_SB_WIDE_K) { HRF_LBW(5, false, LIN_SB, SK_, false); } else { HRF_LBW(5, false, LIN_SB_WIDE, SK_, false); } }
#define HRF_LBW_NT(SK_)                                    \
  switch (ntw) {                                           \
    case 1: HRF_LBW(1, false, LIN_SB, SK_, false); break;  \
    case 2: HRF_LBW(2, false, LIN_SB, SK_, false); break;  \
    case 3: HRF_LBW(3, false, LIN_SB, SK_, false); break;  \
    default: HRF_LBW_WIDE(SK_) break;                      \
  }
constexpr int LIN_WG_MAX_K = 160;
bool hrf_lin_bwd_data_wg_ok(int M, int K, int N, bool bnb) {
  if (K < 4 || N < 4 || M <= 0 || K > LIN_WG_MAX_K) return false;
  return K <= 48 ? bnb : !bnb;
}
static int lin_bwd_data_wg_launch(const LinBwdDataArgs& a, int ntw, bool sk, dim3 grid, void* stream) {
  if (a.K <= 48) {
    switch (ntw) {
      case 1: HRF_LBW_ONE(1) break;
      case 2: HRF_LBW_ONE(2) break;
      case 3: HRF_LBW_ONE(3) break;
      default: HRF_LBW_ONE(5) break;
    }
  } else if (sk) { HRF_LBW_NT(true) } else { HRF_LBW_NT(false) }
  return hrf_check_launch();
}

int hrf_lin_bwd_data_launch(const LinBwdDataArgs& a, void* stream) {
  if (a.K < 4 || a.N < 4 || a.M <= 0) return -1;
  if (a.dw != nullptr && !hrf_lin_bwd_data_wg_ok(a.M, a.K, a.N, a.cA != nullptr)) return -1;
  const int T = (a.N + 15) / 16;
  const bool sk = T <= 9 && lin_use_sk(a.M, a.K);
  int ntw = pick_ntw(sk ? 4 * a.M : a.M, T);
  if (ntw > LIN_BWD_EPI_MAX_NT) ntw = LIN_BWD_EPI_MAX_NT;
  const dim3 grid(hrf_cdiv(a.M, sk ? 16 : 64), hrf_cdiv(T, ntw));
  if (a.dw != nullptr) return lin_bwd_data_wg_launch(a, ntw, sk, grid, stream);
  if (a.cA != nullptr) { HRF_LB_V4(true) } else { HRF_LB_V4(false) }
  return hrf_check_launch();
}
```

hrfuser_amd/profiling.py:

```python
import ctypes
import math
import os
import time

import torch

from . import _lib
from .runtime import gc_paused as _gc_paused


def _pick_nt(C):
    T = (C + 15) // 16
    best, cost = 2, 1 << 30
    for nt in (2, 3, 4):
        c = ((T + nt - 1) // nt) * nt
        if c <= cost:
            cost, best = c, nt
    return best


def _out_hw(H, W, KH, s):
    p = KH // 2
    return (H + 2 * p - KH) // s + 1, (W + 2 * p - KH) // s + 1


def work_model(name, a):
    f4 = 4.0
    if name in ('hrf_conv_fwd', 'hrf_conv_fwd_split', 'hrf_conv_fwd_packed'):
        Ho, Wo = _out_hw(a['H'], a['W'], a['KH'], a['stride'])
        M, K = a['B'] * Ho * Wo, a['KH'] ** 2 * a['Cin']
        by = f4 * (a['B'] * a['H'] * a['W'] * a['Cin'] + a['Cout'] * K + M * a['Cout'] * (1 + (a['res'] is not None) + (a['res2'] is not None)))
        if name == 'hrf_conv_fwd_packed':
            return 'conv3x_kernel<0, 2>', 2.0 * M * a['Cout'] * K, by
        if a['KH'] == 1 and a['stride'] == 1 and a['sC'] == 1 and a['Cin'] >= 4 and a['Cout'] >= 4:
            return 'lin_fwd_kernel', 2.0 * M * a['Cout'] * K, by
        return f"conv_fwd_kernel<{_pick_nt(a['Cout'])},{a['KH']},{a['tf_mode']}>", 2.0 * M * a['Cout'] * K, by
    if name in ('hrf_conv_bwd_data', 'hrf_conv_bwd_data_packed'):
        Ho, Wo = _out_hw(a['H'], a['W'], a['KH'], a['stride'])
        M, K = a['B'] * a['H'] * a['W'], a['KH'] ** 2 * a['Cout']
        by = f4 * (a['B'] * Ho * Wo * a['Cout'] * (2 if a['cA'] is not None else 1) + a['Cin'] * K
                   + M * a['Cin'] * (2 if a['epi'] else 1 + bool(a['accumulate'])))
        fl = 2.0 * a['B'] * Ho * Wo * a['Cin'] * K
        if name == 'hrf_conv_bwd_data_packed':
            return f"conv3x_kernel<{a['stride']}, 2>", fl, by
        if a['KH'] == 1 and a['stride'] == 1 and a['sC'] == 1 and a['Cin'] >= 4 and a['Cout'] >= 4:
            return 'lin_bwd_data_kernel', fl, by
        return f"conv_bwd_data_kernel<{_pick_nt(a['Cin'])},{a['KH']},{int(a['cA'] is not None)}>", fl, by
    if name == 'hrf_conv_bwd_data_weight':
        M = a['B'] * a['H'] * a['W']
        by = f4 * (M * a['Cout'] * (2 if a['cA'] is not None else 1) + 2 * a['Cin'] * a['Cout']
                   + M * a['Cin'] * (2 if a['epi'] else 2 + bool(a['accumulate'])))
        return 'lin_bwd_data_kernel', 4.0 * M * a['Cin'] * a['Cout'], by
    if name == 'hrf_conv_bwd_weight_s':
        Ho, Wo = _out_hw(a['H'], a['W'], a['KH'], a['stride'])
        Mp, Np = a['B'] * Ho * Wo, a['KH'] ** 2 * a['Cin']
        by = f4 * (Mp * a['Cout'] * (2 if a['cA'] is not None else 1) + a['B'] * a['H'] * a['W'] * a['Cin'] + a['Cout'] * Np)
        return f"wgrad3x_kernel<{a['stride']}>", 2.0 * Mp * a['Cout'] * Np, by
    if name == 'hrf_conv_bwd_weight':
        Ho, Wo = _out_hw(a['H'], a['W'], a['KH'], a['stride'])
        Mp, Np = a['B'] * Ho * Wo, a['KH'] ** 2 * a['Cin']
        by = f4 * (Mp * a['Cout'] * (2 if a['cA'] is not None else 1) + a['B'] * a['H'] * a['W'] * a['Cin'] + a['Cout'] * Np)
        dense = a['sC'] == 1 and (a['KH'] == 3 or a['stride'] == 1)
        return ('wgrad_dense_kernel' if dense else 'conv_bwd_wgt_kernel'), 2.0 * Mp * a['Cout'] * Np, by
    if name in ('hrf_dwconv_fwd', 'hrf_dwconv_bwd_weight'):
        Ho, Wo = _out_hw(a['H'], a['W'], 3, a['stride'])
        n_in, n_out = a['B'] * a['H'] * a['W'] * a['C'], a['B'] * Ho * Wo * a['C']
        if name == 'hrf_dwconv_fwd':
            return f"dw_fwd_kernel<{a['stride']}>", 18.0 * n_out, f4 * (n_in + n_out)
        return f"dw_bwd_wgt_kernel<{a['stride']}>", 20.0 * n_out, f4 * (n_in + n_out * (2 if a['cA'] is not None else 1))
    if name == 'hrf_dwconv_bwd_data':
        Ho, Wo = _out_hw(a['H'], a['W'], 3, a['stride'])
        n_in, n_out = a['B'] * a['H'] * a['W'] * a['C'], a['B'] * Ho * Wo * a['C']
        return (f"dw_bwd_data_kernel<{a['stride']}>", 18.0 * n_in,
                f4 * (n_out * (2 if a['cA'] is not None else 1) + n_in * (2 if a['epi'] else 1)))
    if name == 'hrf_dwconv_bwd_data_weight':
        n = a['B'] * a['H'] * a['W'] * a['C']
        return 'dw_bwd_data_kernel<1,wg>', 38.0 * n, f4 * (n * (2 if a['cA'] is not None else 1) + 2 * n)
    if name in ('hrf_window_attn_fwd', 'hrf_window_attn_bwd'):
        nwin = a['B'] * math.ceil(a['H'] / 7) * math.ceil(a['W'] / 7)
        D = a['C'] // a['heads']
        P = a['B'] * a['H'] * a['W']
        unit = 2.0 * 49 * 49 * D * nwin * a['heads']
        if name == 'hrf_window_attn_fwd':
            return f"attn_fwd_kernel<{D}>", 2 * unit, f4 * P * a['C'] * 4
        return f"attn_bwd_kernel<{D}>", 5 * unit, f4 * P * a['C'] * 7
    if name == 'hrf_window_attn_proj_fwd':
        C, heads = a['C'], a['heads']
        rows = float(a['B']) * a['H'] * a['W']
        nwin = a['B'] * math.ceil(a['H'] / 7) * math.ceil(a['W'] / 7)
        fl = 2.0 * rows * C * C * 3 + 2 * 2.0 * 49 * 49 * (C // heads) * nwin * heads
        by = f4 * (rows * C * (2 + bool(a.get('cross')) + 3 * bool(a.get('store'))) + 3 * C * C)
        return f'attn_proj_fwd_kernel<{C // heads}>', fl, by
    if name in ('hrf_attn_block_fwd', 'hrf_attn_block_bwd'):
        C, heads = a['C'], a['heads']
        rows = float(a['B']) * a['H'] * a['W']
        nwin = a['B'] * math.ceil(a['H'] / 7) * math.ceil(a['W'] / 7)
        cross, ffn = bool(a['cross']), bool(a['w1'])
        attn = 2 * 2.0 * 49 * 49 * (C // heads) * nwin * heads
        fwd = 2.0 * rows * C * C * 4 + attn + (2.0 * rows * C * 4 * C if ffn else 0.0)
        wts = 4.0 * (4 * C * C + (4 * C * C if ffn else 0))
        if name == 'hrf_attn_block_fwd':
            by = f4 * rows * C * (2 + 2 * cross + (4 if ffn else 0)) + wts
            return f'attn_block_fwd_kernel<{C}, {heads}, {_lib.attn_fwd_form(C)}>', fwd, by
        slot = 4 * C * C + (4 * C * C if ffn else 0)
        by = f4 * (rows * C * (4 + 3 * cross + (8 if ffn else 0)) + nwin * (slot + heads * 49 * 49)) + wts
        return f'attn_block_bwd_kernel<{C}, {heads}>', 3.0 * fwd, by
    if name == 'hrf_bottleneck_eval':
        M, Cin, pl, ds = float(a['B']) * a['H'] * a['W'], a['Cin'], a['planes'], bool(a['has_downsample'])
        wts = Cin * pl + 9 * pl * pl + 4 * pl * pl + (4 * pl * Cin if ds else 0)
        return f'bneck_eval_kernel<{"true" if ds else "false"}>', 2.0 * M * wts, f4 * (M * Cin + M * 4 * pl + wts)
    if name == 'hrf_rpb_grad':
        return 'rpb_grad_kernel', 0.0, f4 * a['nwin'] * a['heads'] * 49 * 49
    if name in ('hrf_roi_align_fwd', 'hrf_roi_align_bwd'):
        K, C = float(a['K']), a['C']
        fp = K * min(23.0 * 23.0, float(a.get('HW0', 23 * 23))) * C
        fl = 2.0 * K * 49 * C * 4 * 4
        return ('roi_align_fwd_kernel' if name.endswith('fwd') else 'roi_align_bwd_kernel'), fl, f4 * (fp + K * 49 * C)
    if name == 'hrf_conv3_packed_bf16x3':
        M = float(a['B']) * a['H'] * a['W']
        return ('conv3w_bf16x3_kernel', 2.0 * 9 * M * a['K'] * a['N'],
                f4 * (M * a['K'] + 9.0 * a['K'] * a['N'] + M * a['N'] * (1 + bool(a['accumulate']))))
    rc = None
    if 'rows' in a and 'C' in a:
        rc = float(a['rows']) * a['C']
    if name == 'hrf_affine_act_res':
        return 'affine_act_res_kernel', 4 * rc, f4 * rc * (2 + (a['res'] is not None) + (a['y2'] is not None))
    if name == 'hrf_act_bwd':
        n = 2 + (a['out'] is not None) + (a['y1'] is not None and a['st1'] is not None or a['mode'] == 1) \
            + (a['y2'] is not None) + (a['y3'] is not None)
        return 'act_bwd_kernel', 6 * rc, f4 * rc * n
    if name == 'hrf_scale_add':
        return 'scale_add_kernel', 3 * rc, f4 * rc * (2 + (a['mask'] is not None) + (a['res'] is not None) + (a['res2'] is not None))
    if name == 'hrf_ln_stats':
        return 'ln_stats_kernel', 4 * rc, f4 * rc
    if name == 'hrf_ln_bwd':
# ... 630 lines not shown
```

hrfuser_amd/runtime.py:

```python
import ctypes
import os

import torch

try:
    import greenlet as _greenlet
except Exception:
    _greenlet = None

from . import _lib

_DW_FUSED_WG = os.environ.get('HRF_DW_FUSED_WG', '1') != '0'
_FIN_ONLOAD = os.environ.get('HRF_FIN_ONLOAD', '1') != '0'
_XHUB = os.environ.get('HRF_XHUB', '0') != '0'
_LANE_COMMS = os.environ.get('HRF_SYNC_LANE_COMMS', '0') == '1'


def _p2p_mode_id():
    from . import p2p
    return {'off': 0, 'on': 1, 'auto': 2}[p2p.mode()]


def set_lane_comms(on):
    global _LANE_COMMS
    _LANE_COMMS = bool(on)


def lane_comms():
    return _LANE_COMMS


def sync_schedule_fingerprint():
    lockstep = os.environ.get('HRF_LOCKSTEP', '1') != '0'
    batch = os.environ.get('HRF_SYNC_BATCH', '1') != '0'
    eff = 1 if (_greenlet is not None and lockstep and batch and not _LANE_COMMS) else 0
    return [1 if _greenlet is not None else 0, 1 if batch else 0, 1 if _XHUB else 0, 1 if _LANE_COMMS else 0,
            1 if _FIN_ONLOAD else 0, _lib.STAT_COPIES, 1 if lockstep else 0, eff, _p2p_mode_id()]


def check_sync_schedule(group, world):
    if _greenlet is None and os.environ.get('HRF_SYNC_BATCH', '1') != '0' and not _LANE_COMMS and _p2p_mode_id() != 1:
        raise _lib.HRFuserHipError(
            'SyncBN: the batched exchange schedule needs the `greenlet` module, which is not importable here.  Install it, '
            'or set HRF_SYNC_BATCH=0 on EVERY rank to run one collective per BatchNorm (about 3x the collectives).')
    if group is None or world <= 1:
        return
    import torch.distributed as dist
    dev = torch.device('cuda', torch.cuda.current_device()) if dist.get_backend(group) == 'nccl' else torch.device('cpu')
    fp = torch.tensor(sync_schedule_fingerprint(), dtype=torch.int64, device=dev)
    lo, hi = fp.clone(), fp.clone()
    dist.all_reduce(lo, op=dist.ReduceOp.MIN, group=group)
    dist.all_reduce(hi, op=dist.ReduceOp.MAX, group=group)
    if not bool((lo == hi).all()):
        raise _lib.HRFuserHipError(
            f'SyncBN: the ranks disagree on the exchange schedule (greenlet, HRF_SYNC_BATCH, HRF_XHUB, HRF_SYNC_LANE_COMMS, '
            f'HRF_FIN_ONLOAD, HRF_STAT_COPIES, HRF_LOCKSTEP, effective batching, HRF_SYNC_P2P): min {lo.tolist()} max {hi.tolist()}, this rank {fp.tolist()}')
FIN_MAXC = _lib.FIN_MAXC
LN_EPS = 1e-6
_MAX_LANES = int(os.environ.get('HRF_MAX_LANES', '0'))
_FORK_ANCHOR = os.environ.get('HRF_FORK_ANCHOR', '0') == '1'


def force_collectives():
    return os.environ.get('HRF_FORCE_COLLECTIVES', '0') == '1'


TF_NONE, TF_AFFINE, TF_RELU, TF_GELU, TF_LN = 0, 1, 2, 3, 4
ACT_NONE, ACT_RELU, ACT_GELU = 0, 1, 2
_TF2ACT = {TF_NONE: ACT_NONE, TF_AFFINE: ACT_NONE, TF_RELU: ACT_RELU, TF_GELU: ACT_GELU}


def gpu_add_(dst, g):
    _lib.lib().hrf_scale_add(g, None, 1.0, None, 1, dst, None, dst, g.numel(), 1, _lib.stream_ptr())
    return dst


def gpu_clone(g):
    out = _new_like(g)
    _lib.lib().hrf_scale_add(g, None, 1.0, None, 1, None, None, out, g.numel(), 1, _lib.stream_ptr())
    return out


def gpu_zero_(t):
    _lib.lib().hrf_memset(t, 0, t.numel() * t.element_size(), _lib.stream_ptr())
    return t


class Act:
    __slots__ = ('t', 'grad', 'needs_grad', 'rowstat')

    def __init__(self, t, needs_grad=True):
        self.t = t
        self.grad = None
        self.needs_grad = needs_grad
        self.rowstat = None

    @property
    def shape(self):
        return self.t.shape

    def grad_target(self):
        if self.grad is None:
            self.grad = _new_like(self.t)
            return self.grad, 0
        return self.grad, 1

    def add_grad(self, g):
        if self.grad is None:
            self.grad = g
        else:
            gpu_add_(self.grad, g)


class BNState:
    __slots__ = ('bn', 'C', 'raw', 'count', 'scale', 'shift', 'mean', 'invstd', 'stats', 'gstats',
                 'coef', 'du', 'train', 'pending', 'lane', 'bx_done', 'packed', 'bpacked', 'count_ptr', 'fin_lane',
                 'gn_raw', 'gn_stat')


class Lazy:
    __slots__ = ('st', 'mode')

    def __init__(self, st, mode):
        self.st = st
        self.mode = mode

    @property
    def raw(self):
        return self.st.raw

    @property
    def shape(self):
        return self.st.raw.shape


class LNIn:
    __slots__ = ('act', 'rowstat', 'ln')

    def __init__(self, act, rowstat, ln):
        self.act, self.rowstat, self.ln = act, rowstat, ln

    @property
    def shape(self):
        return self.act.t.shape


class LazyTail:
    __slots__ = ('res', 'lazy', 'rowscale', 'out')

    def __init__(self, res, lazy, rowscale=None):
        self.res, self.lazy, self.rowscale, self.out = res, lazy, rowscale, None

    @property
    def shape(self):
        return self.res.t.shape

    def force(self, ctx):
        if self.out is None:
            self.out = materialize(ctx, self.lazy, ACT_GELU, res=self.res, act_first=True, rowscale=self.rowscale)
        return self.out


class Pending:
    __slots__ = ('dims', 'fn', 'out')

    def __init__(self, dims, fn):
        self.dims, self.fn, self.out = tuple(dims), fn, None

    @property
    def shape(self):
        return self.dims

    def force(self, ctx):
        if self.out is None:
            self.out = self.fn(ctx)
            self.fn = None
        return self.out


def LazyFuse(dims, terms):
    return Pending(dims, lambda ctx: fuse_sum(ctx, tuple(dims), terms))


def split_grad(ctx, act):
    alias = Act(act.t, act.needs_grad)
    alias.rowstat = act.rowstat

    def bwd():
        if alias.grad is not None and act.needs_grad:
            act.add_grad(alias.grad)
    ctx.push(bwd)
    return alias


def force(ctx, x):
    return x.force(ctx) if isinstance(x, (LazyTail, Pending)) else x


def force_all(ctx, xs):
    pend = [i for i, x in enumerate(xs) if isinstance(x, Pending) and x.out is None]
    xs = list(xs)
    if len(pend) > 1:
        lanes = ctx.fork(len(pend))

        def one(i):
            xs[i] = force(ctx, xs[i])
        ctx.parallel(lanes, [lambda i=i: one(i) for i in pend])
        ctx.join(lanes)
    return [force(ctx, x) for x in xs]


_TAIL_ONLOAD = os.environ.get('HRF_TAIL_ONLOAD', '1') != '0'


def tail_onload():
    return _TAIL_ONLOAD


class RawInput:
    __slots__ = ('t', 'grad', 'needs_grad', 'nhwc', 'cols')

    def __init__(self, t, needs_grad, nhwc=None):
        self.t, self.grad, self.needs_grad = t, None, needs_grad
        self.nhwc = nhwc
        self.cols = None

    @property
    def shape(self):
        B, C, H, W = self.t.shape
        return (B, H, W, C)


class StageStamps:

    def __init__(self, device, cap=256):
        self.buf = torch.zeros(cap, dtype=torch.int64, device=device)
        self.marks = []

    def reset(self):
        self.marks = []

    def take(self, ctx, direction, name, stream=None):
        i = len(self.marks)
        if i >= self.buf.numel():
            return
        self.marks.append((direction, name))
        ctx.lib.hrf_stamp(self.buf.data_ptr() + 8 * i, ctx.stream if stream is None else stream)

    def read(self):
        t = self.buf[:len(self.marks)].cpu().tolist()
        return [(d, n, (v - t[0]) / 100.0) for (d, n), v in zip(self.marks, t)]


class Lane:
    __slots__ = ('stream', 'ptr')

    def __init__(self, stream):
        self.stream = stream
        self.ptr = stream.cuda_stream if stream is not None else 0


class Strand:
    __slots__ = ('lane', 'tape', 'glet', 'pending', 'wait', 'parent', 'kids_alive', 'cur')

    def __init__(self, lane, parent=None):
        self.lane, self.parent = lane, parent
        self.tape = []
        self.glet = None
        self.pending = None
        self.wait = None
        self.kids_alive = 0
        self.cur = lane


_GROUPABLE = frozenset((
    'hrf_conv_fwd', 'hrf_conv_bwd_data', 'hrf_conv_fwd_packed', 'hrf_conv_bwd_data_packed', 'hrf_dwconv_fwd', 'hrf_dwconv_bwd_data',
    'hrf_dwconv_bwd_data_weight', 'hrf_conv_bwd_data_weight',
    'hrf_attn_block_fwd', 'hrf_attn_block_bwd', 'hrf_affine_act_res', 'hrf_act_bwd', 'hrf_scale_add', 'hrf_ln_stats',
    'hrf_ln_bwd', 'hrf_window_attn_fwd', 'hrf_window_attn_bwd', 'hrf_window_attn_proj_fwd', 'hrf_fuse_sum', 'hrf_bilinear_up_bwd'))
_NO_PARK = frozenset(_lib._RAW_RETURN) | frozenset((
    'hrf_wgrad_group_begin', 'hrf_wgrad_group_end', 'hrf_group_begin', 'hrf_group_end', 'hrf_debug_knob'))


class _LibProxy:

    def __init__(self, ctx, lib):
        self.__dict__['_ctx'] = ctx
        self.__dict__['_lib'] = lib

    def __getattr__(self, name):
        fn = getattr(self.__dict__['_lib'], name)
        if name in _NO_PARK:
            self.__dict__[name] = fn
            return fn
        ctx = self.__dict__['_ctx']

        def call(*a):
            s = ctx._parkable()
            if s is None:
                return fn(*a)
            s.pending = (name, fn, a)
            s.wait = 'call'
            ctx._yield(s)
        self.__dict__[name] = call
        return call


class gc_paused:

    def __enter__(self):
        import gc
        self.was = gc.isenabled()
        gc.disable()
        return self

    def __exit__(self, *exc):
        if self.was:
            import gc
            gc.enable()
        return False


class Ctx:

    def __init__(self, owner, training, record):
        self.lib = owner._lib_handle()
        self.L = _LibProxy(self, self.lib)
        self.det = bool(self.lib.hrf_get_deterministic())
        self.training = training
        self.record = record
        self.owner = owner
        self.group = owner.sync_group if training else None
        self.world = owner.sync_world if (training and owner.sync_group is not None) else 1
        self.multi = bool(torch.cuda.is_available() and getattr(owner, 'use_lanes', True)
                          and os.environ.get('HRF_LANES', '1') != '0')
        self.main = Lane(torch.cuda.current_stream() if torch.cuda.is_available() else None)
        self.cur = self.main
        self.stream = self.main.ptr
        self.root = Strand(self.main)
        self.strand = self.root
        self._free = list(owner._lane_pool()) if self.multi else []
        self._side_i = 0
        self._side_used = {}
        self._deferred = []
        self.probe = [] if owner.__dict__.get('_relu_probe') else None
        self.n_collectives = 0
        self.xhist = {}
        self.coll = self.group is not None and (self.world > 1 or force_collectives())
        self.p2p = owner._engine().p2p_context(self.group, self.world) if self.coll else None
        self.n_p2p = 0
        self.exchange = None
        self.n_grad_collectives = 0
        self.pending = []
        self.bpending = []
        glet = _greenlet if os.environ.get('HRF_LOCKSTEP', '1') != '0' else None
        self.sync_batch = self.coll and glet is not None and os.environ.get('HRF_SYNC_BATCH', '1') != '0' and not _LANE_COMMS \
            and self.p2p is None
        self.merge = glet is not None and os.environ.get('HRF_GROUP', '1') != '0' and hasattr(self.lib, 'hrf_group_begin') \
            and self.lib.hrf_group_count(3) > 1
        self._glet = glet if (self.merge or self.sync_batch or os.environ.get('HRF_LOCKSTEP') == '1') else None
# ... 351 lines not shown
    def side_launch(self, fn, cost=1.0, key=None, target=None):
        mode = os.environ.get('HRF_WGRAD', 'defer')
        bucketed = self.exchange is not None and mode == 'defer'
        if (not self.multi and not bucketed) or mode == 'inline':
            fn()
            return
        if mode in ('defer', 'flush') or bucketed:
            self._deferred.append((float(cost), fn, key, target))
            return
        pool = self.owner._side_pool()
        lane = pool[self._side_i % len(pool)]
        self._side_i += 1
        lane.stream.wait_stream(self.cur.stream)
        self._side_used[id(lane)] = lane
        with _LaneScope(self, lane):
            fn()

    def _flush_deferred(self):
        fns = [it[1] for it in self._deferred]
        self._deferred = []
        pool = self.owner._side_pool()
        k = min(len(pool), int(os.environ.get('HRF_WGRAD_FLUSH_LANES', os.environ.get('HRF_WGRAD_LANES', '4'))))
        group = os.environ.get('HRF_WGRAD_GROUP', '1') != '0'
        for j in range(k):
            lane = pool[(self._side_i + j) % len(pool)]
            lane.stream.wait_stream(self.main.stream)
            self._side_used[id(lane)] = lane
            with _LaneScope(self, lane):
                if group:
                    self.L.hrf_wgrad_group_begin()
                try:
                    for fn in fns[j::k]:
                        fn()
                finally:
                    if group:
                        self.L.hrf_wgrad_group_end(self.stream)
        self._side_i += k

    def _run_tape(self, strand):
        tape = strand.tape
        flush_n = self._flush_n if strand is self.root else 0
        while tape:
            e = tape.pop()
            if e[0] == 'J':
                for k in e[2]:
                    if self.multi and k.stream is not None:
                        k.stream.wait_stream(e[1].stream)
                if self.multi and e[2] and e[2][0].stream is not None:
                    self._fork_anchor(e[1], force=len(e) > 3 and e[3])
                    self._lane_stamp('fork', e[1], e[2])
            elif e[0] == 'F':
                if self.multi and e[2] and e[2][0].stream is not None:
                    self._lane_stamp('join', e[1], e[2])
                for k in e[2]:
                    if self.multi and k.stream is not None:
                        e[1].stream.wait_stream(k.stream)
                if flush_n and e[1] is self.main and len(self._deferred) >= flush_n:
                    self._flush_deferred()
            elif e[0] == 'P':
                kids = e[2]
                self.parallel([k.lane for k in kids], [lambda k=k: self._run_tape(k) for k in kids], kids=kids)
            else:
                fn, lane, sync = e
                if sync is not None and self.coll and sync.train and not sync.bx_done:
                    self.sync_wait_bwd(sync, lane)
                with _LaneScope(self, lane):
                    fn()

    def run_backward(self):
        eng = self.owner._engine()
        if getattr(self, 'gen', None) is not None and self.gen != getattr(eng, 'gen', self.gen):
            raise _lib.HRFuserHipError(
                'backward of a forward pass that is no longer the latest one of this module: every forward re-uses the '
                'BatchNorm statistics slots and step buffers of its engine, so `net(x1); net(x2); loss.backward()` would '
                'back-propagate x1 with the statistics of x2.  Run backward before the next forward of the same module '
                '(or use two module instances).')
        if self.det != bool(self.lib.hrf_get_deterministic()):
            raise _lib.HRFuserHipError('backward of a forward pass that ran in the other deterministic mode: the moment slots '
                                       'of the forward hold ' + ('integer bins' if self.det else 'doubles') + ' the backward '
                                       'kernels would misread (set_deterministic between forward and backward)')
        if self.det:
            eng.det_begin()
        self.lin_fused = lin_fused_sites()
        use_keep_list(self.owner._engine().keep)
        self.owner._engine().fs_prepare()
        self._flush_n = int(os.environ.get('HRF_WGRAD_FLUSH', '48')) if (self.multi and os.environ.get('HRF_WGRAD', 'defer') == 'flush') else 0
        entry = torch.cuda.current_stream() if self.multi else None
        if self.multi:
            self.main.stream.wait_stream(entry)
        self.strand = self.root
        self._run_tape(self.root)
        if self._deferred and os.environ.get('HRF_DEBUG_SKIP_WGRAD') == '1':
            self._deferred = []
        eng0 = self.owner._engine()
        if eng0.rpb_pending():
            if self._deferred:
                self._deferred.append((eng0.fs_rpb_bytes, lambda: eng0.rpb_grad_now(self.L, self.stream), None, None))
            else:
                eng0.rpb_grad_now(self.L, self.stream)
        if self._deferred and eng0.fs_used and os.environ.get('HRF_FOLD_LEAF', '1') != '0':
            self._deferred.append((4.0 * eng0.fs_bytes(), lambda: eng0.fold_slots_now(self.L, self.stream), None, None))
        comm = None
        if self._deferred:
            items, self._deferred = self._deferred, []
            k = int(os.environ.get('HRF_WGRAD_LANES', '4'))
            group = os.environ.get('HRF_WGRAD_GROUP', '1') != '0'
            self.strand = self.root
            for r, (its, ready) in enumerate(self._exchange_rounds(items)):
                lanes = self.fork(k)
                parts = _balance(its, k) if os.environ.get('HRF_WGRAD_BALANCE', '1') != '0' else \
                    [[it[1] for it in its[j::k]] for j in range(k)]
                for j in range(k):
                    with _LaneScope(self, lanes[j]):
                        if group:
                            self.L.hrf_wgrad_group_begin()
                        try:
                            for fn in parts[j]:
                                fn()
                        finally:
                            if group:
                                self.L.hrf_wgrad_group_end(self.stream)
                self.join(lanes)
                xs = self.owner.__dict__.get('_exchange_stamps')
                if xs is not None:
                    xs.take(self, 'leaves_done', f'group {r}', stream=self.main.ptr)
                if self.exchange is not None:
                    if r == 0:
                        if self.multi and self._side_used:
                            for lane in self._side_used.values():
                                self.main.stream.wait_stream(lane.stream)
                            self._side_used = {}
                        with _LaneScope(self, self.main):
                            eng0.fold_grads(self.L, self.main.ptr)
                    comm = self._exchange_issue(ready, comm)
            self.root.tape.clear()
        if self.multi:
            for lane in self._side_used.values():
                self.main.stream.wait_stream(lane.stream)
            self._side_used = {}
        with _LaneScope(self, self.main):
            self.owner._engine().fold_grads(self.L, self.main.ptr)
            st = self.owner.__dict__.get('_stage_stamps')
            if st is not None:
                st.take(self, 'bwd', 'weight_gradients')
        if self.exchange is not None:
            if self.n_grad_collectives == 0:
                comm = self._exchange_issue(list(self.exchange[0]), comm)
            if comm is not None and comm.stream is not None:
                self.main.stream.wait_stream(comm.stream)
                self._free.append(comm)
        if self.multi:
            torch.cuda.set_stream(entry)
            entry.wait_stream(self.main.stream)

    def _exchange_rounds(self, items):
        if self.exchange is None:
            return [(items, [])]
        buckets, _, rounds = self.exchange
        rounds = max(1, min(int(rounds), len(buckets)))
        per = (len(buckets) + rounds - 1) // rounds
        groups = [buckets[g * per:(g + 1) * per] for g in range(rounds)]
        groups = [g for g in groups if g]
        offs = self.owner._engine()._poffs
        out = [([], list(g)) for g in groups]
        for it in items:
            tgt = it[3] if len(it) > 3 else None
# ... 186 lines not shown
        if st.pending == 'fwd':
            _finalize_now(ctx, st)
        elif st.fin_lane is not None and st.fin_lane is not ctx.cur:
            _finalize_now(ctx, st, update_running=False)
            st.pending = 'written'
        else:
            st.pending = None
        return None
    bn = st.bn
    mom = bn.momentum if bn.momentum is not None else 0.1
    P = _lib._ptr
    stats, copies = (P(st.stats), 0) if st.packed is None else (st.packed[0].data_ptr() + 8 * st.packed[1], 1)
    fin = _lib.BnFin(stats, P(bn.weight), P(bn.bias), P(bn.running_mean), P(bn.running_var),
                     P(st.scale), P(st.shift), P(st.mean), P(st.invstd), st.count, float(bn.eps), float(mom),
                     1 if bn.track_running_stats else 0, 1 if st.pending == 'fwd' else 0, st.C, copies, st.count_ptr)
    st.pending = 'written'
    st.fin_lane = ctx.cur
    return fin


def _src_fin(ctx, src, limit=FIN_MAXC):
    return take_fin(ctx, src.st, limit) if isinstance(src, Lazy) else None


def bn_backward_coef(ctx, st, consumer_follows=True, limit=FIN_MAXC):
    slot = ctx.owner._bn_slot(st.bn)
    cA, cB, cC = slot['cA'], slot['cB'], slot['cC']
    st.coef = (cA, cB, cC)
    wg = st.bn.weight.grad if st.bn.weight.requires_grad else None
    bg = st.bn.bias.grad if st.bn.bias.requires_grad else None
    coll = st.train and _collectives(ctx)
    if coll and not st.bx_done:
        ctx.flush_bwd([st], [ctx.cur])
    if coll and st.bx_done:
        packed, local, off = st.bpacked
        P = _lib._ptr
        lptr = local.data_ptr() + 8 * off if local is not None else None
        bf = _lib.BnBFin(packed.data_ptr() + 8 * off, P(st.bn.weight), P(st.mean), P(st.invstd), P(wg), P(bg), P(cA), P(cB),
                         P(cC), st.count, 1, 1, st.C, 1, lptr, 1.0 / max(1, ctx.world), st.count_ptr)
        if _FIN_ONLOAD and consumer_follows and st.C <= limit:
            return st.coef, bf
        ctx.L.hrf_bn_bwd_finalize_packed(bf, 1, packed.data_ptr() + 8 * off, lptr, ctx.stream)
        return st.coef, None
    if _FIN_ONLOAD and consumer_follows and not coll and st.C <= limit and not ctx.det:
        P = _lib._ptr
        return st.coef, _lib.BnBFin(P(st.gstats), P(st.bn.weight), P(st.mean), P(st.invstd), P(wg), P(bg), P(cA), P(cB),
                                    P(cC), st.count, 1 if st.train else 0, 1, st.C)
    local = None
    if coll:
        local = _keep(st.gstats.clone())
        ctx.all_reduce(st.gstats)
    ctx.L.hrf_bn_bwd_finalize(st.gstats, local, st.bn.weight, st.mean, st.invstd, st.count, 1 if st.train else 0,
                              wg, bg, cA, cB, cC, st.C, ctx.stream)
    return st.coef, None


def _conv_out_hw(H, W, KH, stride):
    pad = KH // 2
    return (H + 2 * pad - KH) // stride + 1, (W + 2 * pad - KH) // stride + 1


_LIN_FUSED_WG_DEFAULT = 'proj'
_LIN_FUSED_MAX_ROWS_PLAIN = 2048


def lin_fused_sites(value=None):
    v = (os.environ.get('HRF_LIN_FUSED_WG', _LIN_FUSED_WG_DEFAULT) if value is None else value).strip().lower()
    if v not in ('0', 'proj', 'ffn', 'all'):
        raise ValueError(f"HRF_LIN_FUSED_WG={v!r}: one of 0, proj, ffn, all")
    return {'0': frozenset(), 'proj': frozenset(('proj',)), 'ffn': frozenset(('ffn',)), 'all': frozenset(('proj', 'ffn'))}[v]


def _lin_fused(ctx, site, Cin, Cout, rows, epi, bnb, copy_stride):
    sites = ctx.__dict__.get('lin_fused')
    if sites is None:
        sites = lin_fused_sites()
    if site not in sites or not hasattr(ctx.L, 'hrf_conv_bwd_data_weight'):
        return False
    if copy_stride == 0 and rows > _LIN_FUSED_MAX_ROWS_PLAIN:
        return False
    return bool(ctx.L.hrf_conv_bwd_data_weight_supported(Cin, Cout, rows, epi, 1 if bnb else 0))


_S2F_MINPIX = int(os.environ.get('HRF_C3X_S2F_MINPIX', '4096'))
_IM2COL = os.environ.get('HRF_IM2COL', '1') != '0'


def _packed(ctx, weight, direction, strides, B, H, W, Cin, coef_channels=0):
    if coef_channels > _lib.C3X_MAXC:
        return None
    eng = ctx.owner._engine()
    wp = eng.packed(weight, direction) if hasattr(eng, 'packed') else None
    if wp is None or tuple(strides) != (H * W * Cin, W * Cin, Cin, 1):
        return None
    return wp


def _conv_backward(ctx, src, weight, bias, KH, stride, Cout, dy, ldD, doff, yraw, st=None):
    L, s = ctx.L, ctx.stream
    x, strides, (B, H, W, Cin), tf, sc, sh, rowstat = _src_desc(src)
    needs = _needs_grad(src)
    wpb = (_packed(ctx, weight, 1, strides, B, H, W, Cin, Cout if st is not None else 0)
           if (KH == 3 and (stride == 1 or B * H * W >= 16384)) else None)

    def bwd_data(*args):
        if wpb is not None:
            L.hrf_conv_bwd_data_packed(*args[:-1], wpb, args[-1])
        else:
            L.hrf_conv_bwd_data(*args)
    bfin = None
    cA = cB = cC = None
    if st is not None:
        (cA, cB, cC), bfin = bn_backward_coef(ctx, st, consumer_follows=needs)
    if not needs:
        pass
    elif isinstance(src, Lazy):
        ps = src.st
        ps.du = _new_like(ps.raw)
        fused = False
        if KH == 1 and stride == 1 and weight.requires_grad and tuple(strides) == _nhwc_strides(B, H, W, Cin):
            eng = ctx.owner._engine()
            wacc, cs = eng.grad_acc(weight)
            bacc, bcs = eng.grad_acc(bias) if (bias is not None and bias.requires_grad) else (None, cs)
            fused = bcs == cs and _lin_fused(ctx, 'ffn', Cin, Cout, B * H * W, 1, cA is not None, cs)
        if fused:
            L.hrf_conv_bwd_data_weight(dy, ldD, doff, yraw, cA, cB, cC, bfin, weight, KH, stride, Cout, B, H, W, Cin,
                                       ps.du, *strides, 0, 1, ps.raw, Cin, ps.scale, ps.shift, _TF2ACT[src.mode],
                                       ps.gstats, None, 0, wacc, bacc, cs, s)
            return
        bwd_data(dy, ldD, doff, yraw, cA, cB, cC, bfin, weight, KH, stride, Cout, B, H, W, Cin,
                            ps.du, *strides, 0, 1, ps.raw, Cin, ps.scale, ps.shift, _TF2ACT[src.mode],
                            ps.gstats, s)
    elif isinstance(src, LNIn):
        da = _new_like(src.act.t)
        bwd_data(dy, ldD, doff, yraw, cA, cB, cC, bfin, weight, KH, stride, Cout, B, H, W, Cin,
                            da, *strides, 0, 0, None, 0, None, None, 0, None, s)
        g, acc = src.act.grad_target()
        eng = ctx.owner._engine()
        gacc, cs = eng.grad_acc(src.ln.weight)
        bacc, _ = eng.grad_acc(src.ln.bias)
        L.hrf_ln_bwd(da, src.act.t, src.rowstat, src.ln.weight, B * H * W, Cin, g, acc, gacc, bacc, cs, s)
    elif isinstance(src, Act):
        g, acc = src.grad_target()
        bwd_data(dy, ldD, doff, yraw, cA, cB, cC, bfin, weight, KH, stride, Cout, B, H, W, Cin,
                            g, *strides, acc, 0, None, 0, None, None, 0, None, s)
    else:
        if src.grad is None:
            src.grad = _new_like(src.t)
            acc = 0
        else:
            acc = 1
        bwd_data(dy, ldD, doff, yraw, cA, cB, cC, bfin, weight, KH, stride, Cout, B, H, W, Cin,
                            src.grad, *strides, acc, 0, None, 0, None, None, 0, None, s)
    if weight.requires_grad:
        bgrad = bias.grad if (bias is not None and bias.requires_grad) else None
        if bgrad is not None and ctx.det:
            bacc, bcs = ctx.owner._engine().grad_acc(bias)
            if bcs:
                bgrad = bacc
        xw, sw = x, strides
        if isinstance(src, RawInput) and KH == 3 and src.cols is not None:
            Ho, Wo = _conv_out_hw(H, W, KH, stride)
            K9 = 9 * Cin
            cols = src.cols
            cost = 4.0 * B * Ho * Wo * (K9 + Cout * (2 if cA is not None else 1))
            ctx.side_launch(lambda: L.hrf_conv_bwd_weight(
                dy, ldD, doff, yraw, cA, cB, cC, cols, *_nhwc_strides(B, Ho, Wo, K9), B, Ho, Wo, K9, 1, 1, Cout,
                TF_NONE, None, None, None, weight.grad, bgrad, ctx.stream), cost=cost,
                key=('conv_w', K9, Cout, 1, 1, TF_NONE, cA is not None), target=weight)
            return
        if isinstance(src, RawInput) and KH == 3:
            xw = src.nhwc if src.nhwc is not None else _keep(x.permute(0, 2, 3, 1).contiguous())
            sw = _nhwc_strides(B, H, W, Cin)
        Ho, Wo = _conv_out_hw(H, W, KH, stride)
        cost = 4.0 * B * (H * W * Cin + Ho * Wo * Cout * (2 if cA is not None else 1)) + 0.2 * B * Ho * Wo * Cout * Cin * KH * KH
        nsc = L.hrf_conv_bwd_weight_scratch(*sw, B, H, W, Cin, KH, stride, Cout, tf, 1 if bgrad is not None else 0) if KH == 3 else 0
        if nsc > 0:
            scratch = _new((nsc,), weight.device)
            ctx.side_launch(lambda: L.hrf_conv_bwd_weight_s(
                dy, ldD, doff, yraw, cA, cB, cC, xw, *sw, B, H, W, Cin, KH, stride, Cout,
                tf, sc, sh, rowstat, weight.grad, bgrad, scratch, ctx.stream), cost=cost,
                key=('conv_w3x', Cin, Cout, KH, stride, tf, cA is not None), target=weight)
            return
        ctx.side_launch(lambda: L.hrf_conv_bwd_weight(
            dy, ldD, doff, yraw, cA, cB, cC, xw, *sw, B, H, W, Cin, KH, stride, Cout,
            tf, sc, sh, rowstat, weight.grad, bgrad, ctx.stream), cost=cost,
            key=('conv_w', Cin, Cout, KH, stride, tf, cA is not None), target=weight)


def is_gn(norm):
    return isinstance(norm, torch.nn.GroupNorm)


_GN_CONST = {}


def _gn_unit_affine(C, device):
    key = (str(device), C)
    if key not in _GN_CONST:
        _GN_CONST[key] = (torch.ones(C, device=device), torch.zeros(C, device=device))
    return _GN_CONST[key]


def gn_forward(ctx, gn, raw):
    L, s = ctx.L, ctx.stream
    B, H, W, C = raw.shape
    G = gn.num_groups
    mom = _keep(torch.zeros(B * 2 * C, device=raw.device, dtype=torch.float64))
    L.hrf_gn_moments(raw, None, B, H * W, C, mom, s)
    y = _new_like(raw)
    stat = _new((B, G, 2), raw.device)
    L.hrf_gn_apply(raw, mom, gn.weight, gn.bias, float(gn.eps), B, H * W, C, G, y, stat, s)
    st = BNState()
    st.bn, st.C, st.raw, st.du, st.coef, st.pending, st.lane, st.bx_done = gn, C, y, None, None, None, None, True
    st.packed = st.bpacked = None
    st.count_ptr = None
    st.fin_lane = None
    st.train = False
    st.stats = None
    st.gstats = _keep(torch.zeros(_lib.STAT_COPIES * 2 * C, device=raw.device, dtype=torch.float64))
    st.scale, st.shift = _gn_unit_affine(C, raw.device)
    st.mean = st.invstd = None
    st.count = float(B * H * W)
    st.gn_raw, st.gn_stat = raw, stat
# ... 457 lines not shown
            st.du = None
    ctx.push(bwd, sync=st)
    return out, h1


def dwconv_bn(ctx, src, conv, bn, mode):
    L, s = ctx.L, ctx.stream
    x, _, (B, H, W, C), tf, sc, sh, _ = _src_desc(src)
    w, b = conv.weight, conv.bias
    stride = conv.stride[0]
    Ho, Wo = _conv_out_hw(H, W, 3, stride)
    y = _new((B, Ho, Wo, C), x.device)
    if is_gn(bn):
        L.hrf_dwconv_fwd(x, B, H, W, C, w, b, stride, tf, sc, sh, y, None, _src_fin(ctx, src, 1 << 30), s)
        gst = gn_forward(ctx, bn, y)
        gout = Lazy(gst, mode)
        if ctx.probe is not None and mode == TF_RELU:
            ctx.probe.append(('lazy', gst))

        def gbwd():
            draw = gn_backward(ctx, gst)
            if isinstance(src, Lazy):
                ps = src.st
                ps.du = _new_like(ps.raw)
                L.hrf_dwconv_bwd_data(draw, None, None, None, None, None, w, stride, B, H, W, C, ps.du, 0, 1, ps.raw,
                                      ps.scale, ps.shift, _TF2ACT[src.mode], ps.gstats, s)
            elif src.needs_grad:
                g, acc = src.grad_target()
                L.hrf_dwconv_bwd_data(draw, None, None, None, None, None, w, stride, B, H, W, C, g, acc, 0, None, None,
                                      None, 0, None, s)
            if w.requires_grad:
                eng = ctx.owner._engine()
                wacc, cs = eng.grad_acc(w)
                bacc = eng.grad_acc(b)[0] if b is not None else None
                ctx.side_launch(lambda: L.hrf_dwconv_bwd_weight(
                    draw, None, None, None, None, x, B, H, W, C, stride, tf, sc, sh, wacc, bacc, cs, ctx.stream),
                    cost=4.0 * B * H * W * C * (1.0 + 2.0 / (stride * stride)), key=('dw_w', stride))
            gst.du = None
        ctx.push(gbwd)
        return gout
    slot = ctx.owner._bn_slot(bn)
    train = ctx.training and bn.training
    stats = slot['stats'] if train else None
    L.hrf_dwconv_fwd(x, B, H, W, C, w, b, stride, tf, sc, sh, y, stats, _src_fin(ctx, src, 1 << 30), s)
    st = bn_forward(ctx, bn, y, stats)
    out = Lazy(st, mode)
    if ctx.probe is not None and mode == TF_RELU:
        ctx.probe.append(('lazy', st))

    def bwd():
        needs = isinstance(src, Lazy) or src.needs_grad
        (cA, cB, cC), bfin = bn_backward_coef(ctx, st, consumer_follows=needs, limit=1 << 30)
        fused_wg = False
        if isinstance(src, Lazy):
            ps = src.st
            ps.du = _new_like(ps.raw)
            fused_wg = stride == 1 and w.requires_grad and _DW_FUSED_WG
            if fused_wg:
                eng = ctx.owner._engine()
                wacc, cs = eng.grad_acc(w)
                bacc = eng.grad_acc(b)[0] if b is not None else None
                L.hrf_dwconv_bwd_data_weight(st.du, st.raw, cA, cB, cC, bfin, w, B, H, W, C, ps.du, ps.raw, ps.scale,
                                             ps.shift, _TF2ACT[src.mode], ps.gstats, wacc, bacc, cs, s)
            else:
                L.hrf_dwconv_bwd_data(st.du, st.raw, cA, cB, cC, bfin, w, stride, B, H, W, C, ps.du, 0, 1, ps.raw,
                                      ps.scale, ps.shift, _TF2ACT[src.mode], ps.gstats, s)
        elif src.needs_grad:
            g, acc = src.grad_target()
            L.hrf_dwconv_bwd_data(st.du, st.raw, cA, cB, cC, bfin, w, stride, B, H, W, C, g, acc, 0, None, None,
                                  None, 0, None, s)
        if w.requires_grad and not fused_wg:
            du_ = st.du
            eng = ctx.owner._engine()
            wacc, cs = eng.grad_acc(w)
            bacc = eng.grad_acc(b)[0] if b is not None else None
            ctx.side_launch(lambda: L.hrf_dwconv_bwd_weight(
                du_, st.raw, cA, cB, cC, x, B, H, W, C, stride, tf, sc, sh, wacc, bacc, cs, ctx.stream),
                cost=4.0 * B * H * W * C * (1.0 + 2.0 / (stride * stride)), key=('dw_w', stride))
        st.du = None
    ctx.push(bwd, sync=st)
    return out


def materialize(ctx, lazy, act, res=None, lazy2=None, act_first=False, rowscale=None):
    L, s = ctx.L, ctx.stream
    if not act_first and act not in (ACT_NONE, ACT_RELU):
        raise _lib.HRFuserHipError('materialize: an activation applied last must be ReLU or none (its backward uses the output mask)')
    st = lazy.st
    B, H, W, C = st.raw.shape
    rows = B * H * W
    out = Act(_new_like(st.raw))
    st2 = lazy2.st if lazy2 is not None else None
    rs_out = None
    if act_first:
        out.rowstat = (LN_EPS, _new((rows, 2), st.raw.device))
        rs_out = out.rowstat[1]
    L.hrf_affine_act_res(st.raw, st.scale, st.shift, st2.raw if st2 else None, st2.scale if st2 else None,
                         st2.shift if st2 else None, res.t if res is not None else None, rowscale, H * W,
                         act, 1 if act_first else 0, out.t, rows, C, rs_out, LN_EPS, take_fin(ctx, st), take_fin(ctx, st2), s)
    if ctx.probe is not None and act == ACT_RELU and not act_first:
        ctx.probe.append(('out', out.t))

    def bwd():
        g = _new_like(out.t)
        if act_first:
            assert act == ACT_GELU and st2 is None
            L.hrf_act_bwd(out.grad, None, st.raw, st.scale, st.shift, rowscale, H * W, 1, g, None, None,
                          st.gstats, None, None, rows, C, s)
            st.du = g
            if res is not None and res.needs_grad:
                res.add_grad(out.grad)
        else:
            mode = 0 if act == ACT_RELU else 2
            L.hrf_act_bwd(out.grad, out.t, st.raw, None, None, None, 1, mode, g, st2.raw if st2 else None, None,
                          st.gstats, st2.gstats if st2 else None, None, rows, C, s)
            st.du = g
            if st2 is not None:
                st2.du = g
            if res is not None and res.needs_grad:
                if res.grad is None:
                    res.grad = gpu_clone(g)
                else:
                    gpu_add_(res.grad, g)
    ctx.push(bwd)
    return out


def fuse_sum(ctx, dims, terms):
    L, s = ctx.L, ctx.stream
    B, H, W, C = dims
    dev = terms[0][1].t.device if isinstance(terms[0][1], Act) else terms[0][1].raw.device
    out = Act(_new((B, H, W, C), dev))
    args = []
    fins = (_lib.BnFin * 4)()
    any_fin = False
    for k, (kind, t) in enumerate(terms):
        if kind == 'id':
            args += [1, t.t, None, None, 0, 0]
            continue
        fin = take_fin(ctx, t.st, FIN_MAXC // 2)
        if fin is not None:
            fins[k] = fin
            any_fin = True
        if kind == 'same':
            args += [2, t.raw, t.st.scale, t.st.shift, 0, 0]
        else:
            args += [3 if kind == 'up' else 4, t.raw, t.st.scale, t.st.shift, t.raw.shape[1], t.raw.shape[2]]
    for _ in range(4 - len(terms)):
        args += [0, None, None, None, 0, 0]
    L.hrf_fuse_sum(*args, out.t, B, H, W, C, fins if any_fin else None, s)
    if ctx.probe is not None:
        ctx.probe.append(('out', out.t))

    def bwd():
        g = _new_like(out.t)
        same = [t for kind, t in terms if kind == 'same']
        assert len(same) <= 3
        ys = [t.raw for t in same] + [None] * (3 - len(same))
        sts = [t.st.gstats for t in same] + [None] * (3 - len(same))
        L.hrf_act_bwd(out.grad, out.t, ys[0], None, None, None, 1, 0, g, ys[1], ys[2], sts[0], sts[1], sts[2],
                      B * H * W, C, s)
        can_alias = len(same) == 0
        for kind, t in terms:
            if kind == 'id':
                if t.needs_grad:
                    if t.grad is None:
                        t.grad = g if can_alias else gpu_clone(g)
                        can_alias = False
                    else:
                        gpu_add_(t.grad, g)
            elif kind == 'same':
                t.st.du = g
            else:
                st = t.st
                st.du = _new_like(st.raw)
                adj = L.hrf_bilinear_up_bwd if kind == 'up' else L.hrf_nearest_up_bwd
                adj(g, C, 0, B, H, W, C, st.raw, st.raw.shape[1], st.raw.shape[2], st.du, st.gstats, s)
    ctx.push(bwd)
    return out


def collect_relu_masks(ctx):
    masks = []
    for kind, obj in ctx.probe:
        if kind == 'out':
            t = obj
        else:
            st = obj
            B, H, W, C = st.raw.shape
            t = torch.empty_like(st.raw)
            ctx.L.hrf_affine_act_res(st.raw, st.scale, st.shift, None, None, None, None, None, H * W, ACT_RELU, 0, t,
                                     B * H * W, C, None, 0.0, None, None, ctx.stream)
        masks.append((t > 0).permute(0, 3, 1, 2))
    return masks
```

include/hrfuser_hip.h:

```cpp
#ifndef HRFUSER_HIP_H_
#define HRFUSER_HIP_H_

#ifndef HRF_STAT_COPIES
#define HRF_STAT_COPIES 4
#endif

#define HRF_FIN_MAXC 576
#define HRF_C3X_MAXC 256
typedef struct hrf_bn_fin {
  const double* stats;
  const float* gamma; const float* beta; float* running_mean; float* running_var;
  float* scale; float* shift; float* mean; float* invstd;
  double count; float eps; float momentum; int update_running; int write; int C;
  int copies;
  const double* count_ptr;
} hrf_bn_fin_t;
typedef struct hrf_bn_bfin {
  const double* gstats;
  const float* gamma; const float* mean; const float* invstd;
  float* dgamma; float* dbeta; float* cA; float* cB; float* cC;
  double count; int train; int write; int C;
  int copies;
  const double* gstats_local;
  float pgrad_scale;
  const double* count_ptr;
} hrf_bn_bfin_t;

#ifdef __cplusplus
extern "C" {
#endif

int hrf_conv_fwd(const float* x, int sB, int sY, int sX, int sC, int B, int H, int W, int Cin,
                 const float* w, const float* bias, int KH, int stride, int Cout,
                 float* y, int ldY, int yoff, const float* res, const float* res2, int ldR,
                 int tf_mode, const float* tf_scale, const float* tf_shift,
                 const float* tf_rowstat, double* stats, const hrf_bn_fin_t* tf_fin, float* ln_rowstat, float ln_eps, void* stream);
long hrf_conv_fwd_split_scratch(int sB, int sY, int sX, int sC, int B, int H, int W, int Cin, int KH, int stride, int Cout,
                                int ldY, int yoff);
int hrf_conv_fwd_split(const float* x, int sB, int sY, int sX, int sC, int B, int H, int W, int Cin,
                       const float* w, const float* bias, int KH, int stride, int Cout,
                       float* y, int ldY, int yoff, const float* res, const float* res2, int ldR,
                       int tf_mode, const float* tf_scale, const float* tf_shift,
                       const float* tf_rowstat, double* stats, const hrf_bn_fin_t* tf_fin, float* ln_rowstat, float ln_eps,
                       float* scratch, void* stream);
int hrf_conv_bwd_data(const float* dy, int ldD, int doff, const float* yraw,
                      const float* cA, const float* cB, const float* cC, const hrf_bn_bfin_t* bfin,
                      const float* w, int KH, int stride, int Cout,
                      int B, int H, int W, int Cin,
                      float* dx, int sB, int sY, int sX, int sC, int accumulate,
                      int epi, const float* xraw, int ldXr, const float* tf_scale,
                      const float* tf_shift, int act, double* stats, void* stream);
int hrf_conv_bwd_data_weight_supported(int Cin, int Cout, long rows, int epi, int bnb);
int hrf_conv_bwd_data_weight(const float* dy, int ldD, int doff, const float* yraw,
                             const float* cA, const float* cB, const float* cC, const hrf_bn_bfin_t* bfin,
                             const float* w, int KH, int stride, int Cout,
                             int B, int H, int W, int Cin,
                             float* dx, int sB, int sY, int sX, int sC, int accumulate,
                             int epi, const float* xraw, int ldXr, const float* tf_scale,
                             const float* tf_shift, int act, double* stats,
                             const float* x, int ldX, float* dw, float* dbias, long copy_stride, void* stream);
int hrf_conv_bwd_weight(const float* dy, int ldD, int doff, const float* yraw,
                        const float* cA, const float* cB, const float* cC,
                        const float* x, int sB, int sY, int sX, int sC,
                        int B, int H, int W, int Cin, int KH, int stride, int Cout,
                        int tf_mode, const float* tf_scale, const float* tf_shift,
                        const float* tf_rowstat, float* dw, float* dbias, void* stream);

typedef struct hrf_conv3x_pack_job {
  const float* w; float* wp;
  int Cout, Cin, dir;
} hrf_conv3x_pack_job_t;
long hrf_conv3x_pack_size(int Cout, int Cin, int dir);
int hrf_conv3x_pack(const hrf_conv3x_pack_job_t* jobs, int n, void* stream);
int hrf_conv3x_supported(int Cin, int Cout, int KH, int stride, int dir);
int hrf_conv_fwd_packed(const float* x, int sB, int sY, int sX, int sC, int B, int H, int W, int Cin,
                        const float* w, const float* bias, int KH, int stride, int Cout,
                        float* y, int ldY, int yoff, const float* res, const float* res2, int ldR,
                        int tf_mode, const float* tf_scale, const float* tf_shift,
                        const float* tf_rowstat, double* stats, const hrf_bn_fin_t* tf_fin, float* ln_rowstat, float ln_eps,
                        const float* wp, void* stream);
int hrf_conv_bwd_data_packed(const float* dy, int ldD, int doff, const float* yraw,
                             const float* cA, const float* cB, const float* cC, const hrf_bn_bfin_t* bfin,
                             const float* w, int KH, int stride, int Cout,
                             int B, int H, int W, int Cin,
                             float* dx, int sB, int sY, int sX, int sC, int accumulate,
                             int epi, const float* xraw, int ldXr, const float* tf_scale,
                             const float* tf_shift, int act, double* stats, const float* wp, void* stream);

long hrf_conv_bwd_weight_scratch(int sB, int sY, int sX, int sC, int B, int H, int W, int Cin, int KH, int stride, int Cout,
                                 int tf_mode, int has_bias);
int hrf_conv_bwd_weight_s(const float* dy, int ldD, int doff, const float* yraw,
                          const float* cA, const float* cB, const float* cC,
                          const float* x, int sB, int sY, int sX, int sC,
                          int B, int H, int W, int Cin, int KH, int stride, int Cout,
                          int tf_mode, const float* tf_scale, const float* tf_shift,
                          const float* tf_rowstat, float* dw, float* dbias, float* scratch, void* stream);

int hrf_dwconv_fwd(const float* x, int B, int H, int W, int C, const float* w, const float* bias,
                   int stride, int tf_mode, const float* tf_scale, const float* tf_shift, float* y,
                   double* stats, const hrf_bn_fin_t* tf_fin, void* stream);
int hrf_dwconv_bwd_data(const float* dy, const float* yraw, const float* cA, const float* cB,
                        const float* cC, const hrf_bn_bfin_t* bfin, const float* w, int stride, int B, int H, int W, int C,
                        float* dx, int accumulate, int epi, const float* xraw, const float* tf_scale,
                        const float* tf_shift, int act, double* stats, void* stream);
int hrf_dwconv_bwd_data_weight(const float* dy, const float* yraw, const float* cA, const float* cB,
                               const float* cC, const hrf_bn_bfin_t* bfin, const float* w, int B, int H, int W, int C,
                               float* dx, const float* xraw, const float* tf_scale, const float* tf_shift, int act,
                               double* stats, float* dw, float* dbias, long copy_stride, void* stream);
int hrf_dwconv_bwd_weight(const float* dy, const float* yraw, const float* cA, const float* cB,
                          const float* cC, const float* x, int B, int H, int W, int C, int stride,
                          int tf_mode, const float* tf_scale, const float* tf_shift, float* dw,
                          float* dbias, long copy_stride, void* stream);

int hrf_window_attn_fwd(const float* q, int ldq, int qoff, const float* k, int ldk, int koff,
                        const float* v, int ldv, int voff, const float* kpad, const float* vpad,
                        const float* rpb, float* o, int ldo, int B, int H, int W, int C, int heads,
                        void* stream);
int hrf_window_attn_bwd(const float* q, int ldq, int qoff, const float* k, int ldk, int koff,
                        const float* v, int ldv, int voff, const float* kpad, const float* vpad,
                        const float* rpb, const float* dout, int lddo,
                        float* dq, int lddq, int dqoff, float* dk, int lddk, int dkoff,
                        float* dv, int lddv, int dvoff, float* dkpad, float* dvpad, float* drpb, long copy_stride,
                        int B, int H, int W, int C, int heads, void* stream);

typedef struct hrf_attn_proj {
  int B, H, W, C, heads;
  const float* xq; const float* xkv;
  const float* lnq_g; const float* lnq_b; const float* lnkv_g; const float* lnkv_b;
  const float* rowstat_q; const float* rowstat_kv;
  const float* wq; const float* bq; const float* wk; const float* bk; const float* wv; const float* bv;
  const float* rpb;
  float* o; int ldo;
  float* q_out; int ldq, qoff;
  float* k_out; int ldk, koff;
  float* v_out; int ldv, voff;
} hrf_attn_proj_t;
int hrf_window_attn_proj_supported(int C, int heads);
int hrf_window_attn_proj_fwd(const hrf_attn_proj_t* p, void* stream);

typedef struct hrf_attn_block {
  int B, H, W, C, heads;
  const float* xq; const float* xkv;
  const float* lnq_g; const float* lnq_b; const float* lnkv_g; const float* lnkv_b; float ln_eps;
// ... 192 lines not shown
```

Baseline: 189.2 images/sec.

## Fuse residual add, ReLU mask and BN backward stats into bottleneck conv1x1 dgrad

Adds a relu-tail variant of the 1x1 conv backward-data kernels (lin and lin2 engines). It adds the residual gradient, applies the ReLU mask of the previous block's output, and accumulates the BN backward moments in the same epilogue. The residual gradient is now borrowed instead of cloned, and the runtime tracks expected and arrived gradient contributions so the last consumer can run the fused path. This removes a separate clone, add, ReLU-backward and stats pass per inner bottleneck. In exchange it adds bookkeeping state in Python and larger kernel template variants.

```diff
diff --git a/hrfuser_amd/_lib.py b/hrfuser_amd/_lib.py
--- a/hrfuser_amd/_lib.py
+++ b/hrfuser_amd/_lib.py
@@ -60,7 +60,7 @@
     return None if t is None else t.data_ptr()
 
 
-_RAW_RETURN = ('hrf_conv3_wgrad_wide_scratch', 'hrf_conv_bwd_weight_scratch', 'hrf_conv3x_pack_size', 'hrf_conv3x_supported', 'hrf_conv_bwd_data_weight_supported', 'hrf_conv_fwd_split_scratch', 'hrf_wgrad_group_report', 'hrf_attn_block_supported', 'hrf_attn_block_bwd_supported', 'hrf_window_attn_proj_supported', 'hrf_group_count',
+_RAW_RETURN = ('hrf_conv3_wgrad_wide_scratch', 'hrf_conv_bwd_weight_scratch', 'hrf_conv3x_pack_size', 'hrf_conv3x_supported', 'hrf_conv_bwd_data_weight_supported', 'hrf_conv_bwd_data_relu_tail_supported', 'hrf_conv_fwd_split_scratch', 'hrf_wgrad_group_report', 'hrf_attn_block_supported', 'hrf_attn_block_bwd_supported', 'hrf_window_attn_proj_supported', 'hrf_group_count',
                'hrf_ffn_eval_supported', 'hrf_bottleneck_eval_supported', 'hrf_roi_align_supported', 'hrf_get_deterministic', 'hrf_det_bins_bytes', 'hrf_conv3_bf16x3_supported', 'hrf_grad_sumsq_parts')
 _ERR = {1: 'HRF_ERR_ARG (bad argument)', 2: 'HRF_ERR_LAUNCH (kernel launch failed)'}
 
diff --git a/hrfuser_amd/backbone.py b/hrfuser_amd/backbone.py
--- a/hrfuser_amd/backbone.py
+++ b/hrfuser_amd/backbone.py
@@ -531,7 +531,7 @@
         self.add_module(self._nn[2], build_bn(norm_cfg, planes * 4))
         self.downsample = downsample
 
-    def run(self, ctx, x):
+    def run(self, ctx, x, sole_uses=0):
         if R.bottleneck_eval_ok(ctx, self, x):
             return R.bottleneck_eval(ctx, x, self)
         n1, n2, n3 = (getattr(self, k) for k in self._nn)
@@ -540,8 +540,8 @@
         y = R.conv_bn(ctx, y, self.conv3, n3, R.TF_AFFINE)
         if self.downsample is not None:
             idt = R.conv_bn(ctx, x, self.downsample[0], self.downsample[1], R.TF_AFFINE)
-            return R.materialize(ctx, y, R.ACT_RELU, lazy2=idt)
-        return R.materialize(ctx, y, R.ACT_RELU, res=x)
+            return R.materialize(ctx, y, R.ACT_RELU, lazy2=idt, sole_uses=sole_uses)
+        return R.materialize(ctx, y, R.ACT_RELU, res=x, sole_uses=sole_uses)
 
 
 class BasicBlock(nn.Module):
@@ -1018,6 +1018,14 @@
     return nn.Sequential(*layers)
 
 
+def _run_res_layer(ctx, layer, x):
+    blocks = list(layer)
+    for i, blk in enumerate(blocks):
+        inner = i + 1 < len(blocks) and isinstance(blk, Bottleneck) and isinstance(blocks[i + 1], Bottleneck)
+        x = blk.run(ctx, x, sole_uses=2) if inner else blk.run(ctx, x)
+    return x
+
+
 def resolve_init_cfg(pretrained, init_cfg):
     assert not (init_cfg and pretrained), 'init_cfg and pretrained cannot be specified at the same time'
     if isinstance(pretrained, str):
@@ -1498,9 +1506,7 @@
         y = R.conv_bn(ctx, src, c1, b1, R.TF_RELU)
         y = R.conv_bn(ctx, y, c2, b2, R.TF_RELU)
         x = R.materialize(ctx, y, R.ACT_RELU)
-        for blk in layer:
-            x = blk.run(ctx, x)
-        return x
+        return _run_res_layer(ctx, layer, x)
 
     def _fuse_stage(self, ctx, cam_in, trans_cam, trans_mod, fusion, nb, mods, first, tag=''):
         M = self.num_fused_modalities
diff --git a/hrfuser_amd/csrc/conv_engine.hip b/hrfuser_amd/csrc/conv_engine.hip
--- a/hrfuser_amd/csrc/conv_engine.hip
+++ b/hrfuser_amd/csrc/conv_engine.hip
@@ -996,6 +996,48 @@
   l.tf_scale = tf_scale; l.tf_shift = tf_shift; l.act = act; l.stats = hrf_det_tag(stats);
   l.M = (int)rows; l.K = Cout; l.N = Cin;
   l.x = x; l.ldX = ldX; l.dw = dw; l.dbias = dbias; l.copy_stride = copy_stride;
+  const int rc = hrf_lin_bwd_data_launch(l, stream);
+  return rc >= 0 ? rc : HRF_ERR_ARG;
+}
+
+extern "C" int hrf_conv_bwd_data_relu_tail_supported(int Cin, int Cout, long rows, int bnb, int two_norms) {
+  (void)bnb; (void)two_norms;
+  if (Cin <= 0 || Cout <= 0 || rows <= 0 || g_knob[4] != 0) return 0;
+  if (hrf_lin2_bwd_data_wide(rows, Cout, Cin) && !hrf_lin2_bwd_data_tail_built(Cin)) return 0;
+  return hrf_lin_bwd_data_tail_ok(rows, Cout, Cin) ? 1 : 0;
+}
+
+extern "C" int hrf_conv_bwd_data_relu_tail(const float* dy, int ldD, int doff, const float* yraw,
+                                           const float* cA, const float* cB, const float* cC, const hrf_bn_bfin_t* bfin,
+                                           const float* w, int KH, int stride, int Cout,
+                                           int B, int H, int W, int Cin,
+                                           float* dx, int sB, int sY, int sX, int sC, int accumulate,
+                                           int epi, const float* xraw, int ldXr, const float* tf_scale,
+                                           const float* tf_shift, int act, double* stats,
+                                           const float* addend, int ldAdd, const float* mask_out, const float* y1, const float* y2,
+                                           int ldT, double* stats1, double* stats2, void* stream) {
+  HRF_GROUP_CALL();
+  (void)xraw; (void)ldXr; (void)tf_scale; (void)tf_shift; (void)act;
+  if (KH != 1 || stride != 1 || !(sC == 1 && sX == Cin && sY == W * sX && sB == H * sY)) return HRF_ERR_ARG;
+  if (accumulate != 0 || epi != 0 || stats != nullptr) return HRF_ERR_ARG;
+  if (bfin != nullptr && (cA == nullptr || bfin->C != Cout || Cout > HRF_FIN_MAXC || bfin->gstats == nullptr)) return HRF_ERR_ARG;
+  if (dy == nullptr || w == nullptr || dx == nullptr || mask_out == nullptr || y1 == nullptr || ldT < Cin) return HRF_ERR_ARG;
+  if ((cA != nullptr && (yraw == nullptr || cB == nullptr || cC == nullptr)) || (addend != nullptr && (ldAdd < Cin || addend == dx)))
+    return HRF_ERR_ARG;
+  if ((y2 == nullptr) != (stats2 == nullptr)) return HRF_ERR_ARG;
+  const long rows = (long)B * H * W;
+  if (B <= 0 || H <= 0 || W <= 0 || !hrf_conv_bwd_data_relu_tail_supported(Cin, Cout, rows, cA != nullptr, y2 != nullptr)) return HRF_ERR_ARG;
+  if (!hrf_det_fin_ok(bfin)) return HRF_ERR_ARG;
+  LinBwdDataArgs l;
+  l.bfin = hrf_bn_bfin_t{};
+  if (bfin != nullptr) l.bfin = *bfin;
+  l.dy = dy; l.ldD = ldD; l.doff = doff; l.yraw = yraw; l.cA = cA; l.cB = cB; l.cC = cC; l.w = w;
+  l.dx = dx; l.ldDx = sX; l.accumulate = 0; l.epi = 2; l.xraw = nullptr; l.ldXr = 0;
+  l.tf_scale = nullptr; l.tf_shift = nullptr; l.act = 0; l.stats = hrf_det_tag(stats1);
+  l.M = (int)rows; l.K = Cout; l.N = Cin;
+  l.addend = addend; l.ldAdd = ldAdd; l.mask_out = mask_out; l.y1 = y1; l.y2 = y2; l.ldT = ldT; l.stats2 = hrf_det_tag(stats2);
+  const int rc2 = hrf_lin2_bwd_data_launch(l, stream);
+  if (rc2 >= 0) return rc2;
   const int rc = hrf_lin_bwd_data_launch(l, stream);
   return rc >= 0 ? rc : HRF_ERR_ARG;
 }
diff --git a/hrfuser_amd/csrc/hrf_lin.h b/hrfuser_amd/csrc/hrf_lin.h
--- a/hrfuser_amd/csrc/hrf_lin.h
+++ b/hrfuser_amd/csrc/hrf_lin.h
@@ -24,6 +24,9 @@
   int M, K, N;
   const float* x = nullptr; int ldX = 0;
   float* dw = nullptr; float* dbias = nullptr; long copy_stride = 0;
+  const float* addend = nullptr; int ldAdd = 0;
+  const float* mask_out = nullptr; const float* y1 = nullptr; const float* y2 = nullptr; int ldT = 0;
+  double* stats2 = nullptr;
 };
 
 int hrf_lin_fwd_launch(const LinFwdArgs& a, void* stream);
@@ -34,6 +37,8 @@
 bool hrf_lin2_fwd_emits_ln(const LinFwdArgs& a);
 int hrf_lin2_bwd_data_launch(const LinBwdDataArgs& a, void* stream);
 bool hrf_lin2_bwd_data_wide(long M, int K, int N);
+bool hrf_lin_bwd_data_tail_ok(long M, int K, int N);
+bool hrf_lin2_bwd_data_tail_built(int N);
 
 struct Conv3Args {
   const float* in; int ldIn;
diff --git a/hrfuser_amd/csrc/lin2_engine.hip b/hrfuser_amd/csrc/lin2_engine.hip
--- a/hrfuser_amd/csrc/lin2_engine.hip
+++ b/hrfuser_amd/csrc/lin2_engine.hip
@@ -83,7 +83,7 @@
 #pragma unroll
     for (int tt = 0; tt < T::CT; ++tt) l2_st4(sE + ((rg * T::RT + rr) * 16 + i) * T::PE + tt * 16 + 4 * q, acc[rr][tt]);
 }
-template <class T>
+template <class T, bool F64 = false>
 __device__ __forceinline__ void moments_out(float* sRed, double* stats, int N, int chbase, int c4, int rgp, bool active,
                                             const float* s1, const float* s2) {
   constexpr int CW = T::CT * 16;
@@ -98,10 +98,94 @@
   for (int e = threadIdx.x; e < 2 * CW; e += NTHR) {
     const int which = e / CW, c = e - which * CW;
     if (chbase + c < N) {
-      float s = 0.f;
+      typename std::conditional<F64, double, float>::type s = 0;
 #pragma unroll
       for (int g = 0; g < T::NRG; ++g) s += sRed[(g * 2 + which) * CW + c];
       hrf_stat_add(stats, 2 * N, which * N + chbase + c, (double)s);
+    }
+  }
+}
+
+template <class T>
+__device__ __forceinline__ void tail_epilogue(const LinBwdDataArgs& a, float* sE, float* sRed, const hrf_f4 (*acc)[T::CT],
+                                              long m0, int n0, int chg, int rg, int lane, int tid) {
+  constexpr int CG = T::CG, CT = T::CT, Q = T::Q, PE = T::PE, NRG = T::NRG, NR = T::NR;
+  const int c4 = tid % Q, rgp = tid / Q;
+  const bool active = rgp < NRG;
+  const bool two = a.y2 != nullptr;
+#pragma unroll 1
+  for (int pass = 0; pass < CG; ++pass) {
+    const int chbase = n0 + pass * CT * 16, ch = chbase + 4 * c4;
+    const int nval = active ? a.N - ch : 0;
+    hrf_f4 u0[NR], u1[NR];
+#pragma unroll
+    for (int j = 0; j < NR; ++j) {
+      const long m = m0 + rgp + j * NRG;
+      const bool rv = rgp + j * NRG < GROWS && m < a.M;
+      u0[j] = hrf_f4{0.f, 0.f, 0.f, 0.f};
+      u1[j] = gl_ld4(a.mask_out + (rv ? m : 0) * a.ldT + ch, rv ? nval : 0);
+    }
+    if (a.addend != nullptr) {
+#pragma unroll
+      for (int j = 0; j < NR; ++j) {
+        const long m = m0 + rgp + j * NRG;
+        const bool rv = rgp + j * NRG < GROWS && m < a.M;
+        u0[j] = gl_ld4(a.addend + (rv ? m : 0) * a.ldAdd + ch, rv ? nval : 0);
+      }
+    }
+    if (pass > 0) __syncthreads();
+    if (chg == pass) acc_to_lds<T>(sE, acc, rg, lane);
+    __syncthreads();
+#pragma unroll
+    for (int j = 0; j < NR; ++j) {
+      const int row = rgp + j * NRG;
+      const long m = m0 + row;
+      if (row < GROWS && m < a.M && nval > 0) {
+        hrf_f4 v = l2_ld4(sE + row * PE + 4 * c4);
+#pragma unroll
+        for (int r = 0; r < 4; ++r) {
+          const float t = v[r] + u0[j][r];
+          v[r] = (u1[j][r] > 0.f && r < nval) ? t : 0.f;
+        }
+        l2_st4(sE + row * PE + 4 * c4, v);
+        float* o = a.dx + m * a.ldDx + ch;
+        if (nval >= 4) hrf_st4(o, v);
+        else {
+#pragma unroll
+          for (int r = 0; r < 4; ++r)
+            if (r < nval) o[r] = v[r];
+        }
+      }
+    }
+#pragma unroll
+    for (int j = 0; j < NR; ++j) {
+      const long m = m0 + rgp + j * NRG;
+      const bool rv = rgp + j * NRG < GROWS && m < a.M;
+      u0[j] = gl_ld4(a.y1 + (rv ? m : 0) * a.ldT + ch, rv ? nval : 0);
+      u1[j] = hrf_f4{0.f, 0.f, 0.f, 0.f};
+    }
+    if (two) {
+#pragma unroll
+      for (int j = 0; j < NR; ++j) {
+        const long m = m0 + rgp + j * NRG;
+        const bool rv = rgp + j * NRG < GROWS && m < a.M;
+        u1[j] = gl_ld4(a.y2 + (rv ? m : 0) * a.ldT + ch, rv ? nval : 0);
+      }
+    }
+    float s1[4] = {0.f, 0.f, 0.f, 0.f}, s2[4] = {0.f, 0.f, 0.f, 0.f}, s3[4] = {0.f, 0.f, 0.f, 0.f};
+#pragma unroll
+    for (int j = 0; j < NR; ++j) {
+      const int row = rgp + j * NRG;
+      if (row < GROWS && m0 + row < a.M && nval > 0) {
+        const hrf_f4 v = l2_ld4(sE + row * PE + 4 * c4);
+#pragma unroll
+        for (int r = 0; r < 4; ++r) { s1[r] += v[r]; s2[r] = fmaf(v[r], u0[j][r], s2[r]); s3[r] = fmaf(v[r], u1[j][r], s3[r]); }
+      }
+    }
+    if (a.stats != nullptr) moments_out<T, true>(sRed, a.stats, a.N, chbase, c4, rgp, active, s1, s2);
+    if (two && a.stats2 != nullptr) {
+      __syncthreads();
+      moments_out<T, true>(sRed, a.stats2, a.N, chbase, c4, rgp, active, s1, s3);
     }
   }
 }
@@ -318,7 +402,7 @@
   }
 }
 
-template <class T, bool BNB>
+template <class T, bool BNB, bool TAIL = false>
 __global__ __launch_bounds__(NTHR, 2) void lin2_bwd_data_kernel(HrfGroup<LinBwdDataArgs> grp) {
   const LinBwdDataArgs& a = grp.sel();
   constexpr int CG = T::CG, CT = T::CT, PD = T::PD, NB = T::NB, RT = T::RT, SLOT = T::SLOT, NWV = T::NWV;
@@ -460,6 +544,10 @@
   };
   if (all_on) kloop(std::true_type{}); else kloop(std::false_type{});
 
+  if (TAIL) {
+    tail_epilogue<T>(a, smem, sRed, acc, m0, n0, chg, rg, lane, tid);
+    return;
+  }
   {
     constexpr int Q = T::Q, PE = T::PE, NRG = T::NRG, NR = T::NR;
     float* sE = smem;
@@ -582,18 +670,22 @@
     default: return -1;
   }
 }
-template <class T, bool BNB>
+template <class T, bool BNB, bool TAIL>
 int launch_bwd(const LinBwdDataArgs& a, int id, void* stream) {
   const size_t smem = smem_bytes(id, BNB ? 3 : 0, a.K, T::RED);
   if (smem > SMEM_MAX) return -1;
   static size_t granted = 0;
-  if (smem > granted) { if (set_smem(&lin2_bwd_data_kernel<T, BNB>, smem) != HRF_OK) return HRF_ERR_LAUNCH; granted = smem; }
+  if (smem > granted) { if (set_smem(&lin2_bwd_data_kernel<T, BNB, TAIL>, smem) != HRF_OK) return HRF_ERR_LAUNCH; granted = smem; }
   const dim3 grid(hrf_cdiv(a.M, GROWS), hrf_cdiv(a.N, T::NB));
-  return HRF_LAUNCH_G((lin2_bwd_data_kernel<T, BNB>), grid, dim3(NTHR), (unsigned)smem, stream, a);
+  return HRF_LAUNCH_G((lin2_bwd_data_kernel<T, BNB, TAIL>), grid, dim3(NTHR), (unsigned)smem, stream, a);
 }
 template <class T>
 int launch_bwd_b(const LinBwdDataArgs& a, int id, void* stream) {
-  return a.cA != nullptr ? launch_bwd<T, true>(a, id, stream) : launch_bwd<T, false>(a, id, stream);
+  if (a.epi == 2) {
+    if constexpr (T::CT < 10) return a.cA != nullptr ? launch_bwd<T, true, true>(a, id, stream) : launch_bwd<T, false, true>(a, id, stream);
+    else return -1;
+  }
+  return a.cA != nullptr ? launch_bwd<T, true, false>(a, id, stream) : launch_bwd<T, false, false>(a, id, stream);
 }
 
 }
@@ -613,6 +705,7 @@
 }
 bool hrf_lin2_fwd_emits_ln(const LinFwdArgs&) { return false; }
 bool hrf_lin2_bwd_data_wide(long M, int K, int N) { return wide_enough(M, K, N); }
+bool hrf_lin2_bwd_data_tail_built(int N) { return pick_tile(N) != 4; }
 int hrf_lin2_bwd_data_launch(const LinBwdDataArgs& a, void* stream) {
   if (!wide_enough(a.M, a.K, a.N)) return -1;
   if (a.cA != nullptr && a.bfin.gstats != nullptr && a.K > HRF_FIN_MAXC) return -1;
diff --git a/hrfuser_amd/csrc/lin_engine.hip b/hrfuser_amd/csrc/lin_engine.hip
--- a/hrfuser_amd/csrc/lin_engine.hip
+++ b/hrfuser_amd/csrc/lin_engine.hip
@@ -65,14 +65,15 @@
   }
 }
 
-template <int NT>
+template <int NT, bool F64 = false>
 __device__ __forceinline__ void flush_moments(const float* sStat, double* stats, int n0w, int N) {
   for (int i = threadIdx.x; i < 2 * NT * 16; i += 256) {
     const int which = i / (NT * 16), cidx = i - which * (NT * 16);
     const int ch = n0w + cidx;
     if (ch < N) {
-      const float s = sStat[(0 * 2 + which) * (NT * 16) + cidx] + sStat[(1 * 2 + which) * (NT * 16) + cidx] +
-                      sStat[(2 * 2 + which) * (NT * 16) + cidx] + sStat[(3 * 2 + which) * (NT * 16) + cidx];
+      typedef typename std::conditional<F64, double, float>::type acc_t;
+      const acc_t s = (acc_t)sStat[(0 * 2 + which) * (NT * 16) + cidx] + (acc_t)sStat[(1 * 2 + which) * (NT * 16) + cidx] +
+                      (acc_t)sStat[(2 * 2 + which) * (NT * 16) + cidx] + (acc_t)sStat[(3 * 2 + which) * (NT * 16) + cidx];
       hrf_stat_add(stats, 2 * N, which * N + ch, (double)s);
     }
   }
@@ -196,7 +197,7 @@
 }
 
 constexpr int LIN_WG_LD = 20;
-template <int NT, bool BNB, int SB, bool SK, bool ONE = false, bool WG = false>
+template <int NT, bool BNB, int SB, bool SK, bool ONE = false, bool WG = false, bool TAIL = false>
 __global__ __launch_bounds__(256) void lin_bwd_data_kernel(HrfGroup<LinBwdDataArgs> grp) {
   const LinBwdDataArgs& a = grp.sel();
   __shared__ float sStat[4 * 2 * NT * 16];
@@ -228,7 +229,8 @@
     const int chb = n0w + 16 * t + 4 * q, nval = a.N - chb;
     const bool nfull = n0w + 16 * (t + 1) <= a.N;
     xr[t] = ld_sel(nfull, a.xraw, pc * a.ldXr + chb, a.epi == 1 ? nval : 0);
-    acc[t] = ld_sel(nfull, a.dx, pc * a.ldDx + chb, (a.epi != 1 && a.accumulate && (!SK || wave == 0)) ? nval : 0);
+    if (TAIL) acc[t] = ld_sel(nfull, a.addend, pc * a.ldAdd + chb, a.addend != nullptr ? nval : 0);
+    else acc[t] = ld_sel(nfull, a.dx, pc * a.ldDx + chb, (a.epi != 1 && a.accumulate && (!SK || wave == 0)) ? nval : 0);
   }
 
   hrf_f4 xb[WG ? NT : 1];
@@ -386,6 +388,40 @@
     }
   }
 
+  if (TAIL) {
+    const bool two = a.y2 != nullptr;
+    hrf_f4 ov[NT], y1v[NT], y2v[NT];
+#pragma unroll
+    for (int t = 0; t < NT; ++t) {
+      const int chb = n0w + 16 * t + 4 * q, nval = a.N - chb;
+      const bool nfull = n0w + 16 * (t + 1) <= a.N;
+      ov[t] = ld_sel(nfull, a.mask_out, pc * a.ldT + chb, nval);
+      y1v[t] = ld_sel(nfull, a.y1, pc * a.ldT + chb, nval);
+      y2v[t] = ld_sel(nfull, a.y2, pc * a.ldT + chb, two ? nval : 0);
+    }
+#pragma unroll
+    for (int t = 0; t < NT; ++t)
+#pragma unroll
+      for (int r = 0; r < 4; ++r) acc[t][r] = ov[t][r] > 0.f ? acc[t][r] : 0.f;
+#pragma unroll
+    for (int t = 0; t < NT; ++t) {
+      const int chb = n0w + 16 * t + 4 * q;
+      if (n0w + 16 * (t + 1) <= a.N) st_group<true>(a.dx + (long)pc * a.ldDx + chb, acc[t], pixv ? a.N - chb : 0);
+      else st_group<false>(a.dx + (long)pc * a.ldDx + chb, acc[t], pixv ? a.N - chb : 0);
+    }
+    if (a.stats != nullptr) {
+      wave_moments<NT>(sStat, wave, j, q, pixv, n0w, a.N, acc, y1v);
+      __syncthreads();
+      flush_moments<NT, true>(sStat, a.stats, n0w, a.N);
+    }
+    if (two && a.stats2 != nullptr) {
+      __syncthreads();
+      wave_moments<NT>(sStat, wave, j, q, pixv, n0w, a.N, acc, y2v);
+      __syncthreads();
+      flush_moments<NT, true>(sStat, a.stats2, n0w, a.N);
+    }
+    return;
+  }
   if (a.epi == 1) {
     hrf_f4 esc[NT], esh[NT];
 #pragma unroll
@@ -553,15 +589,33 @@
   return hrf_check_launch();
 }
 
+#define HRF_LBT(NT_, BNB_, SB_) HRF_LAUNCH_G((lin_bwd_data_kernel<NT_, BNB_, SB_, false, false, false, true>), grid, dim3(256), 0, stream, a)
+#define HRF_LBT_NT(BNB_)                                   \
+  switch (ntw) {                                           \
+    case 1: HRF_LBT(1, BNB_, LIN_SB); break;               \
+    case 2: HRF_LBT(2, BNB_, LIN_SB); break;               \
+    case 3: HRF_LBT(3, BNB_, LIN_SB); break;               \
+    default: if (a.K <= LIN_SB_WIDE_K) { HRF_LBT(5, BNB_, LIN_SB); } else { HRF_LBT(5, BNB_, LIN_SB_WIDE); } break; \
+  }
+bool hrf_lin_bwd_data_tail_ok(long M, int K, int N) {
+  if (K <= 48 || N < 4 || M <= 0 || M > (1L << 30)) return false;
+  return !((N + 15) / 16 <= 9 && lin_use_sk((int)M, K));
+}
+
 int hrf_lin_bwd_data_launch(const LinBwdDataArgs& a, void* stream) {
   if (a.K < 4 || a.N < 4 || a.M <= 0) return -1;
   if (a.dw != nullptr && !hrf_lin_bwd_data_wg_ok(a.M, a.K, a.N, a.cA != nullptr)) return -1;
+  if (a.epi == 2 && (a.dw != nullptr || a.accumulate || !hrf_lin_bwd_data_tail_ok(a.M, a.K, a.N))) return -1;
   const int T = (a.N + 15) / 16;
   const bool sk = T <= 9 && lin_use_sk(a.M, a.K);
   int ntw = pick_ntw(sk ? 4 * a.M : a.M, T);
   if (ntw > LIN_BWD_EPI_MAX_NT) ntw = LIN_BWD_EPI_MAX_NT;
   const dim3 grid(hrf_cdiv(a.M, sk ? 16 : 64), hrf_cdiv(T, ntw));
   if (a.dw != nullptr) return lin_bwd_data_wg_launch(a, ntw, sk, grid, stream);
+  if (a.epi == 2) {
+    if (a.cA != nullptr) { HRF_LBT_NT(true) } else { HRF_LBT_NT(false) }
+    return hrf_check_launch();
+  }
   if (a.cA != nullptr) { HRF_LB_V4(true) } else { HRF_LB_V4(false) }
   return hrf_check_launch();
 }
diff --git a/hrfuser_amd/profiling.py b/hrfuser_amd/profiling.py
--- a/hrfuser_amd/profiling.py
+++ b/hrfuser_amd/profiling.py
@@ -51,6 +51,11 @@
         by = f4 * (M * a['Cout'] * (2 if a['cA'] is not None else 1) + 2 * a['Cin'] * a['Cout']
                    + M * a['Cin'] * (2 if a['epi'] else 2 + bool(a['accumulate'])))
         return 'lin_bwd_data_kernel', 4.0 * M * a['Cin'] * a['Cout'], by
+    if name == 'hrf_conv_bwd_data_relu_tail':
+        M = a['B'] * a['H'] * a['W']
+        maps = 3 + (a['addend'] is not None) + (a['y2'] is not None)
+        by = f4 * (M * a['Cout'] * (2 if a['cA'] is not None else 1) + a['Cin'] * a['Cout'] + M * a['Cin'] * maps)
+        return 'lin_bwd_data_kernel', 2.0 * M * a['Cin'] * a['Cout'], by
     if name == 'hrf_conv_bwd_weight_s':
         Ho, Wo = _out_hw(a['H'], a['W'], a['KH'], a['stride'])
         Mp, Np = a['B'] * Ho * Wo, a['KH'] ** 2 * a['Cin']
diff --git a/hrfuser_amd/runtime.py b/hrfuser_amd/runtime.py
--- a/hrfuser_amd/runtime.py
+++ b/hrfuser_amd/runtime.py
@@ -87,28 +87,50 @@
 
 
 class Act:
-    __slots__ = ('t', 'grad', 'needs_grad', 'rowstat')
+    __slots__ = ('t', 'grad', 'needs_grad', 'rowstat', 'tail', 'expect', 'arrived', 'borrowed', 'masked')
 
     def __init__(self, t, needs_grad=True):
         self.t = t
         self.grad = None
         self.needs_grad = needs_grad
         self.rowstat = None
+        self.tail = None
+        self.expect = 0
+        self.arrived = 0
+        self.borrowed = False
+        self.masked = False
 
     @property
     def shape(self):
         return self.t.shape
 
+    def own_grad(self):
+        if self.borrowed:
+            self.grad = gpu_clone(self.grad)
+            self.borrowed = False
+
     def grad_target(self):
+        self.arrived += 1
         if self.grad is None:
             self.grad = _new_like(self.t)
             return self.grad, 0
+        self.own_grad()
         return self.grad, 1
 
     def add_grad(self, g):
+        self.arrived += 1
         if self.grad is None:
             self.grad = g
         else:
+            self.own_grad()
+            gpu_add_(self.grad, g)
+
+    def add_grad_kept(self, g, may_borrow=False):
+        self.arrived += 1
+        if self.grad is None:
+            self.grad, self.borrowed = (g, True) if may_borrow else (gpu_clone(g), False)
+        else:
+            self.own_grad()
             gpu_add_(self.grad, g)
 
 
@@ -275,7 +297,7 @@
 
 _GROUPABLE = frozenset((
     'hrf_conv_fwd', 'hrf_conv_bwd_data', 'hrf_conv_fwd_packed', 'hrf_conv_bwd_data_packed', 'hrf_dwconv_fwd', 'hrf_dwconv_bwd_data',
-    'hrf_dwconv_bwd_data_weight', 'hrf_conv_bwd_data_weight',
+    'hrf_dwconv_bwd_data_weight', 'hrf_conv_bwd_data_weight', 'hrf_conv_bwd_data_relu_tail',
     'hrf_attn_block_fwd', 'hrf_attn_block_bwd', 'hrf_affine_act_res', 'hrf_act_bwd', 'hrf_scale_add', 'hrf_ln_stats',
     'hrf_ln_bwd', 'hrf_window_attn_fwd', 'hrf_window_attn_bwd', 'hrf_window_attn_proj_fwd', 'hrf_fuse_sum', 'hrf_bilinear_up_bwd'))
 _NO_PARK = frozenset(_lib._RAW_RETURN) | frozenset((
@@ -793,6 +815,7 @@
         if self.det:
             eng.det_begin()
         self.lin_fused = lin_fused_sites()
+        self.relu_tail = relu_tail_fused()
         use_keep_list(self.owner._engine().keep)
         self.owner._engine().fs_prepare()
         self._flush_n = int(os.environ.get('HRF_WGRAD_FLUSH', '48')) if (self.multi and os.environ.get('HRF_WGRAD', 'defer') == 'flush') else 0
@@ -1145,6 +1168,37 @@
     return bool(ctx.L.hrf_conv_bwd_data_weight_supported(Cin, Cout, rows, epi, 1 if bnb else 0))
 
 
+_RELU_TAIL_FUSED_DEFAULT = '1'
+
+
+def relu_tail_fused(value=None):
+    v = (os.environ.get('HRF_RELU_TAIL_FUSED', _RELU_TAIL_FUSED_DEFAULT) if value is None else value).strip()
+    if v not in ('0', '1'):
+        raise ValueError(f"HRF_RELU_TAIL_FUSED={v!r}: one of 0, 1")
+    return v == '1'
+
+
+def _relu_tail_candidate(ctx, act):
+    on = ctx.__dict__.get('relu_tail')
+    if on is None:
+        on = relu_tail_fused()
+    return bool(on and isinstance(act, Act) and act.tail is not None and act.expect == 2 and act.arrived == 0
+                and hasattr(ctx.L, 'hrf_conv_bwd_data_relu_tail'))
+
+
+def _relu_tail_now(ctx, src, KH, stride, strides, B, H, W, Cin, Cout, bnb):
+    on = ctx.__dict__.get('relu_tail')
+    if on is None:
+        on = relu_tail_fused()
+    if not on or src.tail is None or src.masked or src.expect <= 0 or src.arrived != src.expect - 1:
+        return False
+    if not (src.grad is None or src.borrowed) or not hasattr(ctx.L, 'hrf_conv_bwd_data_relu_tail'):
+        return False
+    if KH != 1 or stride != 1 or tuple(strides) != _nhwc_strides(B, H, W, Cin):
+        return False
+    return bool(ctx.L.hrf_conv_bwd_data_relu_tail_supported(Cin, Cout, B * H * W, 1 if bnb else 0, 1 if src.tail[1] is not None else 0))
+
+
 _S2F_MINPIX = int(os.environ.get('HRF_C3X_S2F_MINPIX', '4096'))
 _IM2COL = os.environ.get('HRF_IM2COL', '1') != '0'
 
@@ -1203,6 +1257,15 @@
         gacc, cs = eng.grad_acc(src.ln.weight)
         bacc, _ = eng.grad_acc(src.ln.bias)
         L.hrf_ln_bwd(da, src.act.t, src.rowstat, src.ln.weight, B * H * W, Cin, g, acc, gacc, bacc, cs, s)
+    elif isinstance(src, Act) and _relu_tail_now(ctx, src, KH, stride, strides, B, H, W, Cin, Cout, cA is not None):
+        tst, tst2 = src.tail
+        g = _new_like(src.t)
+        L.hrf_conv_bwd_data_relu_tail(dy, ldD, doff, yraw, cA, cB, cC, bfin, weight, KH, stride, Cout, B, H, W, Cin,
+                                      g, *strides, 0, 0, None, 0, None, None, 0, None,
+                                      src.grad, Cin, src.t, tst.raw, tst2.raw if tst2 is not None else None, Cin,
+                                      tst.gstats, tst2.gstats if tst2 is not None else None, s)
+        src.grad, src.borrowed, src.masked = g, False, True
+        src.arrived += 1
     elif isinstance(src, Act):
         g, acc = src.grad_target()
         bwd_data(dy, ldD, doff, yraw, cA, cB, cC, bfin, weight, KH, stride, Cout, B, H, W, Cin,
@@ -1826,7 +1889,7 @@
     return out
 
 
-def materialize(ctx, lazy, act, res=None, lazy2=None, act_first=False, rowscale=None):
+def materialize(ctx, lazy, act, res=None, lazy2=None, act_first=False, rowscale=None, sole_uses=0):
     L, s = ctx.L, ctx.stream
     if not act_first and act not in (ACT_NONE, ACT_RELU):
         raise _lib.HRFuserHipError('materialize: an activation applied last must be ReLU or none (its backward uses the output mask)')
@@ -1844,8 +1907,19 @@
                          act, 1 if act_first else 0, out.t, rows, C, rs_out, LN_EPS, take_fin(ctx, st), take_fin(ctx, st2), s)
     if ctx.probe is not None and act == ACT_RELU and not act_first:
         ctx.probe.append(('out', out.t))
+    if act == ACT_RELU and not act_first:
+        out.tail = (st, st2)
+        out.expect = sole_uses
 
     def bwd():
+        if out.masked:
+            g = out.grad
+            st.du = g
+            if st2 is not None:
+                st2.du = g
+            if res is not None and res.needs_grad:
+                res.add_grad_kept(g, may_borrow=_relu_tail_candidate(ctx, res))
+            return
         g = _new_like(out.t)
         if act_first:
             assert act == ACT_GELU and st2 is None
@@ -1862,10 +1936,7 @@
             if st2 is not None:
                 st2.du = g
             if res is not None and res.needs_grad:
-                if res.grad is None:
-                    res.grad = gpu_clone(g)
-                else:
-                    gpu_add_(res.grad, g)
+                res.add_grad_kept(g, may_borrow=_relu_tail_candidate(ctx, res))
     ctx.push(bwd)
     return out
 
@@ -1912,6 +1983,7 @@
                         t.grad = g if can_alias else gpu_clone(g)
                         can_alias = False
                     else:
+                        t.own_grad()
                         gpu_add_(t.grad, g)
             elif kind == 'same':
                 t.st.du = g
diff --git a/include/hrfuser_hip.h b/include/hrfuser_hip.h
--- a/include/hrfuser_hip.h
+++ b/include/hrfuser_hip.h
@@ -59,6 +59,16 @@
                              int epi, const float* xraw, int ldXr, const float* tf_scale,
                              const float* tf_shift, int act, double* stats,
                              const float* x, int ldX, float* dw, float* dbias, long copy_stride, void* stream);
+int hrf_conv_bwd_data_relu_tail_supported(int Cin, int Cout, long rows, int bnb, int two_norms);
+int hrf_conv_bwd_data_relu_tail(const float* dy, int ldD, int doff, const float* yraw,
+                                const float* cA, const float* cB, const float* cC, const hrf_bn_bfin_t* bfin,
+                                const float* w, int KH, int stride, int Cout,
+                                int B, int H, int W, int Cin,
+                                float* dx, int sB, int sY, int sX, int sC, int accumulate,
+                                int epi, const float* xraw, int ldXr, const float* tf_scale,
+                                const float* tf_shift, int act, double* stats,
+                                const float* addend, int ldAdd, const float* mask_out, const float* y1, const float* y2,
+                                int ldT, double* stats1, double* stats2, void* stream);
 int hrf_conv_bwd_weight(const float* dy, int ldD, int doff, const float* yraw,
                         const float* cA, const float* cB, const float* cC,
                         const float* x, int sB, int sY, int sX, int sC,
```

Result: no change. 190.4 images/sec, median of 5 (+0.7%).
